# kzhai/PyLDA

Hardware: AMD Instinct MI355X
Metric: documents/sec per VB iteration (higher is better)
Workload: dtype f64

## Files before the change

### include/pylda_hip.h

```cpp
#ifndef PYLDA_HIP_H
#define PYLDA_HIP_H

#include <stdint.h>

#ifdef __cplusplus
extern "C" {
#endif

typedef struct pylda_ctx pylda_ctx;
typedef struct pylda_corpus pylda_corpus;

typedef enum pylda_status {
    PYLDA_OK = 0,
    PYLDA_ERR_INVALID = -1,
    PYLDA_ERR_HIP = -2,
    PYLDA_ERR_OOM = -3,
    PYLDA_ERR_STATE = -4
} pylda_status;

#define PYLDA_ABI_VERSION 10
int pylda_abi_version(void);

const char* pylda_version(void);

// ... 72 lines not shown
int pylda_elapsed_ms(pylda_ctx* ctx, int slot_from, int slot_to, double* ms);

int pylda_set_profiling(pylda_ctx* ctx, int enabled);
int pylda_kernel_time(pylda_ctx* ctx, double* doc_kernel_ms, double* sstats_kernel_ms,
                      int64_t* estep_calls);
int pylda_work_counters(pylda_ctx* ctx, double* inner_iterations, double* inner_iteration_terms);
int pylda_executed_work(pylda_ctx* ctx, double* tile_entries, double* handed_over);
int pylda_clock_counters(pylda_ctx* ctx, double* shader_ticks, double* wall_ticks, double* wall_hz);

int pylda_corpus_plan(pylda_corpus* corpus, int32_t capacity, int32_t* variant, int32_t* geometry,
                      int64_t* documents, int64_t* terms, double* kernel_ms);

int64_t pylda_corpus_layout(pylda_corpus* corpus, const char* name);

int pylda_set_option(pylda_ctx* ctx, const char* name, int64_t value);

int pylda_test_special(pylda_ctx* ctx, int64_t n, const double* x, double* digamma_out,
                       double* lgamma_out);

int pylda_parse_corpus(const char* text, int64_t text_bytes, int doc_separator, const char* vocab,
                       int64_t vocab_bytes, int lowercase, int64_t* n_docs, int64_t* nnz,
                       int64_t* doc_ptr, int32_t* term_id, int32_t* term_ct, int64_t* dropped_docs);

int pylda_test_alpha_update(pylda_ctx* ctx, const double* alpha_k, const double* alpha_ss_k, double number_of_documents,
                            int hyper_parameter_iteration, double hyper_parameter_decay_factor,
                            int hyper_parameter_maximum_decay, double hyper_parameter_converge_threshold,
                            double* alpha_out_k);

int pylda_hybrid_estep(pylda_ctx* ctx, pylda_corpus* corpus, int number_of_samples, int burn_in_samples, uint64_t seed,
                       uint64_t stream, int64_t first_document, int heldout);
int pylda_hybrid_scale_sstats(pylda_ctx* ctx, double divisor);

int pylda_test_philox(pylda_ctx* ctx, int64_t n, const uint32_t* counter_key, uint32_t* out);

int pylda_gibbs_init(pylda_ctx* ctx, pylda_corpus* corpus, uint64_t seed, int64_t first_document);
int pylda_gibbs_sweep(pylda_ctx* ctx, pylda_corpus* corpus, const double* alpha_k, const double* beta_v, double beta_sum,
                      int64_t blocks, uint64_t seed, uint64_t stream, int64_t first_document);
int pylda_gibbs_log_posterior(pylda_ctx* ctx, pylda_corpus* corpus, const double* alpha_k, const double* beta_v, double* out);
int pylda_gibbs_get_counts(pylda_ctx* ctx, pylda_corpus* corpus, int32_t* n_kv, int32_t* n_k, int32_t* topics);
int pylda_gibbs_set_state(pylda_ctx* ctx, pylda_corpus* corpus, const int32_t* n_kv, const int32_t* n_k, const int32_t* topics);

int pylda_gibbs_round_tokens(pylda_ctx* ctx, pylda_corpus* corpus, int64_t blocks, int64_t first_document, int64_t* tokens);
int pylda_gibbs_exchange_prepare(pylda_ctx* ctx, pylda_corpus* corpus, int64_t blocks, int64_t first_document, int world, int rank,
                                 const int64_t* capacity, void** send, void** recv);
int pylda_gibbs_round_sample(pylda_ctx* ctx, pylda_corpus* corpus, const double* alpha_k, const double* beta_v, double beta_sum,
                             int64_t blocks, int64_t round, uint64_t seed, uint64_t stream, int64_t first_document);
int pylda_gibbs_round_apply(pylda_ctx* ctx, pylda_corpus* corpus, int64_t round);
int pylda_gibbs_table_device(pylda_ctx* ctx, pylda_corpus* corpus, void** table, int64_t* table_elements, void** n_k);
int pylda_gibbs_log_posterior_parts(pylda_ctx* ctx, pylda_corpus* corpus, const double* alpha_k, const double* beta_v, double* out);

int pylda_foldin_set_model(pylda_ctx* ctx, pylda_corpus* trained, const int32_t* n_kv, const int32_t* n_k,
                           const double* beta_v, double beta_sum);
int pylda_foldin(pylda_ctx* ctx, pylda_corpus* heldout, const double* alpha_k, int number_of_samples, int burn_in_samples,
                 uint64_t seed, uint64_t stream, int64_t first_document, double* words_log_likelihood);

int pylda_completion_set_model(pylda_ctx* ctx);
int pylda_completion_score(pylda_ctx* ctx, pylda_corpus* observed, pylda_corpus* held, const double* gamma_dk,
                           double* held_log_likelihood, int64_t* held_tokens);

int pylda_left_to_right(pylda_ctx* ctx, pylda_corpus* heldout, const double* alpha_k, int particles, int resample,
                        uint64_t seed, uint64_t stream, int64_t first_document, int64_t step_budget,
                        double* log_likelihood, int64_t* tokens);
int pylda_test_left_to_right_state(pylda_ctx* ctx, pylda_corpus* heldout, int particles, uint16_t* z_out, double* p_out);

int pylda_top_words(pylda_ctx* ctx, const double* table_kv ,
                    int M, int32_t* ids_km, double* values_km);
int pylda_codocument_counts(pylda_ctx* ctx, pylda_corpus* reference, int M, const int32_t* ids_km ,
                            int64_t* doc_freq_km, int64_t* co_kmm);

int pylda_similarity_set_base(pylda_ctx* ctx, int64_t D, const double* rows_dk , int transform);
int pylda_similar_documents(pylda_ctx* ctx, int64_t Q, const double* rows_qk , int transform, int N,
                            const int32_t* self_ids , int32_t* ids_qn, double* scores_qn);

int pylda_topic_distances(pylda_ctx* ctx, const double* a_kv , int Ka,
                          const double* b_kv , int Kb, int metric, double* out_ab);

int pylda_test_expdigamma(pylda_ctx* ctx, int64_t n, const double* x, double c, double* out);

int pylda_test_special_forms(pylda_ctx* ctx, int64_t n, const double* x, double c, int form, double* out);

int pylda_test_tables(pylda_ctx* ctx, double* psi_rowsum_k, double* elog_vldk, double* expElog_vldk,
                      double* expElog_elog_vldk, double* shift_v, double* topic_lse_k, double* alpha_sgn_k, int* path_out);

int pylda_test_statistics(pylda_ctx* ctx, pylda_corpus* corpus, const double* t_dldk, const double* r_nnz,
                          const int32_t* live_n_d, const uint16_t* live_topic_d60, const double* live_t_d60,
                          double* entropy_out);

int pylda_test_gibbs_posterior_terms(pylda_ctx* ctx, pylda_corpus* corpus, const double* alpha_k, const double* beta_v,
                                     double* doc_terms, double* word_terms, double* sums);

#ifdef __cplusplus
}
#endif
#endif
```

### pylda_amd/_capi.py

```python
import collections
import ctypes
import os
import threading

import numpy as np

ABI_VERSION = 10
_LIB_PATH = os.path.join(os.path.dirname(os.path.abspath(__file__)), "lib", "libpylda_hip.so")
_lib = None

_c_double_p = ctypes.POINTER(ctypes.c_double)
_c_int32_p = ctypes.POINTER(ctypes.c_int32)
_c_int64_p = ctypes.POINTER(ctypes.c_int64)
_vp = ctypes.c_void_p

SIGNATURES = {
    "pylda_version": (ctypes.c_char_p, []),
    "pylda_abi_version": (ctypes.c_int, []),
    "pylda_device_count": (ctypes.c_int, [ctypes.POINTER(ctypes.c_int)]),
    "pylda_create": (ctypes.c_int, [ctypes.c_int, ctypes.c_int, ctypes.c_int, ctypes.POINTER(_vp)]),
    "pylda_destroy": (None, [_vp]),
    "pylda_last_error": (ctypes.c_char_p, [_vp]),
    "pylda_set_stream": (ctypes.c_int, [_vp, _vp]),
    "pylda_use_own_stream": (ctypes.c_int, [_vp]),
    "pylda_synchronize": (ctypes.c_int, [_vp]),
    "pylda_corpus_create": (ctypes.c_int, [_vp, ctypes.c_int64, _c_int64_p, _c_int32_p, _c_int32_p,
                                           ctypes.POINTER(_vp)]),
    "pylda_corpus_destroy": (None, [_vp]),
    "pylda_corpus_info": (ctypes.c_int, [_vp, _c_int64_p, _c_int64_p, _c_int64_p, _c_int32_p]),
    "pylda_set_eta": (ctypes.c_int, [_vp, _c_double_p]),
    "pylda_get_eta": (ctypes.c_int, [_vp, _c_double_p]),
    "pylda_set_alpha": (ctypes.c_int, [_vp, _c_double_p]),
    "pylda_estep": (ctypes.c_int, [_vp, _vp, ctypes.c_int, ctypes.c_double, ctypes.c_int]),
    "pylda_estep_results": (ctypes.c_int, [_vp, _vp, _c_double_p, _c_double_p, _c_int64_p]),
    "pylda_get_sstats": (ctypes.c_int, [_vp, _c_double_p]),
    "pylda_set_sstats": (ctypes.c_int, [_vp, _c_double_p]),
    "pylda_get_gamma": (ctypes.c_int, [_vp, _vp, _c_double_p]),
    "pylda_get_doc_values": (ctypes.c_int, [_vp, _vp, _c_double_p, _c_double_p, _c_int32_p]),
    "pylda_estep_host": (ctypes.c_int, [_vp, _vp, _c_double_p, _c_double_p, ctypes.c_int,
                                        ctypes.c_double, ctypes.c_int, _c_double_p, _c_double_p,
                                        _c_double_p, _c_double_p, _c_int32_p, _c_double_p]),
    "pylda_table_stride": (ctypes.c_int, [_vp]),
    "pylda_compute_units": (ctypes.c_int, [_vp]),
    "pylda_sstats_device": (_vp, [_vp]),
    "pylda_eta_device": (_vp, [_vp]),
    "pylda_gamma_device": (_vp, [_vp]),
    "pylda_mark_device_state": (ctypes.c_int, [_vp, ctypes.c_int, ctypes.c_int]),
    "pylda_comm_unique_id": (ctypes.c_int, [_vp]),
    "pylda_comm_init": (ctypes.c_int, [_vp, _vp, ctypes.c_int, ctypes.c_int]),
    "pylda_comm_destroy": (ctypes.c_int, [_vp]),
    "pylda_allreduce_sstats": (ctypes.c_int, [_vp]),
    "pylda_allreduce_doubles": (ctypes.c_int, [_vp, _c_double_p, ctypes.c_int64]),
    "pylda_mstep": (ctypes.c_int, [_vp, _vp, _c_double_p, _c_double_p, _c_double_p]),
    "pylda_mstep_enqueue": (ctypes.c_int, [_vp, _vp, _c_double_p, ctypes.c_int, ctypes.c_double, ctypes.c_int,
                                           ctypes.c_double]),
    "pylda_mstep_online": (ctypes.c_int, [_vp, _vp, _c_double_p, ctypes.c_double, ctypes.c_double, _c_double_p, _c_double_p]),
    "pylda_mstep_online_enqueue": (ctypes.c_int, [_vp, _vp, _c_double_p, ctypes.c_double, ctypes.c_double]),
    "pylda_outer_device": (_vp, [_vp, _c_int64_p]),
    "pylda_allreduce_outer": (ctypes.c_int, [_vp]),
    "pylda_outer_fetch": (ctypes.c_int, [_vp, _c_double_p, _c_double_p, _c_int64_p, _c_double_p, _c_double_p,
                                         _c_double_p]),
    "pylda_host_alloc": (ctypes.c_int, [ctypes.c_int64, ctypes.POINTER(_vp)]),
    "pylda_host_free": (ctypes.c_int, [_vp]),
    "pylda_model_checkpoint": (ctypes.c_int, [_vp, ctypes.c_int]),
    "pylda_mark_time": (ctypes.c_int, [_vp, ctypes.c_int]),
    "pylda_elapsed_ms": (ctypes.c_int, [_vp, ctypes.c_int, ctypes.c_int, _c_double_p]),
    "pylda_work_counters": (ctypes.c_int, [_vp, _c_double_p, _c_double_p]),
    "pylda_executed_work": (ctypes.c_int, [_vp, _c_double_p, _c_double_p]),
    "pylda_clock_counters": (ctypes.c_int, [_vp, _c_double_p, _c_double_p, _c_double_p]),
    "pylda_set_profiling": (ctypes.c_int, [_vp, ctypes.c_int]),
    "pylda_kernel_time": (ctypes.c_int, [_vp, _c_double_p, _c_double_p, _c_int64_p]),
    "pylda_corpus_layout": (ctypes.c_int64, [_vp, ctypes.c_char_p]),
    "pylda_corpus_plan": (ctypes.c_int, [_vp, ctypes.c_int32, _c_int32_p, _c_int32_p, _c_int64_p, _c_int64_p,
                                         _c_double_p]),
    "pylda_set_option": (ctypes.c_int, [_vp, ctypes.c_char_p, ctypes.c_int64]),
    "pylda_parse_corpus": (ctypes.c_int, [ctypes.c_char_p, ctypes.c_int64, ctypes.c_int, ctypes.c_char_p,
                                          ctypes.c_int64, ctypes.c_int, _c_int64_p, _c_int64_p, _c_int64_p,
                                          _c_int32_p, _c_int32_p, _c_int64_p]),
    "pylda_test_alpha_update": (ctypes.c_int, [_vp, _c_double_p, _c_double_p, ctypes.c_double, ctypes.c_int, ctypes.c_double,
                                               ctypes.c_int, ctypes.c_double, _c_double_p]),
    "pylda_test_expdigamma": (ctypes.c_int, [_vp, ctypes.c_int64, _c_double_p, ctypes.c_double, _c_double_p]),
    "pylda_test_special_forms": (ctypes.c_int, [_vp, ctypes.c_int64, _c_double_p, ctypes.c_double, ctypes.c_int, _c_double_p]),
    "pylda_test_tables": (ctypes.c_int, [_vp, _c_double_p, _c_double_p, _c_double_p, _c_double_p, _c_double_p, _c_double_p,
                                         _c_double_p, ctypes.POINTER(ctypes.c_int)]),
    "pylda_test_statistics": (ctypes.c_int, [_vp, _vp, _c_double_p, _c_double_p, _c_int32_p, ctypes.POINTER(ctypes.c_uint16),
                                             _c_double_p, _c_double_p]),
    "pylda_test_special": (ctypes.c_int, [_vp, ctypes.c_int64, _c_double_p, _c_double_p, _c_double_p]),
    "pylda_test_gibbs_posterior_terms": (ctypes.c_int, [_vp, _vp, _c_double_p, _c_double_p, _c_double_p, _c_double_p, _c_double_p]),
    "pylda_hybrid_estep": (ctypes.c_int, [_vp, _vp, ctypes.c_int, ctypes.c_int, ctypes.c_uint64, ctypes.c_uint64,
                                          ctypes.c_int64, ctypes.c_int]),
    "pylda_hybrid_scale_sstats": (ctypes.c_int, [_vp, ctypes.c_double]),
    "pylda_test_philox": (ctypes.c_int, [_vp, ctypes.c_int64, ctypes.POINTER(ctypes.c_uint32),
                                         ctypes.POINTER(ctypes.c_uint32)]),
    "pylda_gibbs_init": (ctypes.c_int, [_vp, _vp, ctypes.c_uint64, ctypes.c_int64]),
    "pylda_gibbs_sweep": (ctypes.c_int, [_vp, _vp, _c_double_p, _c_double_p, ctypes.c_double, ctypes.c_int64, ctypes.c_uint64,
                                         ctypes.c_uint64, ctypes.c_int64]),
    "pylda_gibbs_log_posterior": (ctypes.c_int, [_vp, _vp, _c_double_p, _c_double_p, _c_double_p]),
    "pylda_gibbs_get_counts": (ctypes.c_int, [_vp, _vp, _c_int32_p, _c_int32_p, _c_int32_p]),
    "pylda_gibbs_set_state": (ctypes.c_int, [_vp, _vp, _c_int32_p, _c_int32_p, _c_int32_p]),
    "pylda_gibbs_round_tokens": (ctypes.c_int, [_vp, _vp, ctypes.c_int64, ctypes.c_int64, _c_int64_p]),
    "pylda_gibbs_exchange_prepare": (ctypes.c_int, [_vp, _vp, ctypes.c_int64, ctypes.c_int64, ctypes.c_int, ctypes.c_int, _c_int64_p,
                                                    ctypes.POINTER(_vp), ctypes.POINTER(_vp)]),
    "pylda_gibbs_round_sample": (ctypes.c_int, [_vp, _vp, _c_double_p, _c_double_p, ctypes.c_double, ctypes.c_int64, ctypes.c_int64,
                                                ctypes.c_uint64, ctypes.c_uint64, ctypes.c_int64]),
    "pylda_gibbs_round_apply": (ctypes.c_int, [_vp, _vp, ctypes.c_int64]),
    "pylda_gibbs_table_device": (ctypes.c_int, [_vp, _vp, ctypes.POINTER(_vp), _c_int64_p, ctypes.POINTER(_vp)]),
    "pylda_gibbs_log_posterior_parts": (ctypes.c_int, [_vp, _vp, _c_double_p, _c_double_p, _c_double_p]),
    "pylda_foldin_set_model": (ctypes.c_int, [_vp, _vp, _c_int32_p, _c_int32_p, _c_double_p, ctypes.c_double]),
    "pylda_foldin": (ctypes.c_int, [_vp, _vp, _c_double_p, ctypes.c_int, ctypes.c_int, ctypes.c_uint64, ctypes.c_uint64,
                                    ctypes.c_int64, _c_double_p]),
    "pylda_completion_set_model": (ctypes.c_int, [_vp]),
    "pylda_completion_score": (ctypes.c_int, [_vp, _vp, _vp, _c_double_p, _c_double_p, _c_int64_p]),
    "pylda_left_to_right": (ctypes.c_int, [_vp, _vp, _c_double_p, ctypes.c_int, ctypes.c_int, ctypes.c_uint64, ctypes.c_uint64,
                                           ctypes.c_int64, ctypes.c_int64, _c_double_p, _c_int64_p]),
    "pylda_test_left_to_right_state": (ctypes.c_int, [_vp, _vp, ctypes.c_int, ctypes.POINTER(ctypes.c_uint16), _c_double_p]),
    "pylda_top_words": (ctypes.c_int, [_vp, _c_double_p, ctypes.c_int, _c_int32_p, _c_double_p]),
    "pylda_codocument_counts": (ctypes.c_int, [_vp, _vp, ctypes.c_int, _c_int32_p, _c_int64_p, _c_int64_p]),
    "pylda_similarity_set_base": (ctypes.c_int, [_vp, ctypes.c_int64, _c_double_p, ctypes.c_int]),
    "pylda_similar_documents": (ctypes.c_int, [_vp, ctypes.c_int64, _c_double_p, ctypes.c_int, ctypes.c_int, _c_int32_p, _c_int32_p,
                                               _c_double_p]),
    "pylda_topic_distances": (ctypes.c_int, [_vp, _c_double_p, ctypes.c_int, _c_double_p, ctypes.c_int, ctypes.c_int, _c_double_p]),
}


def library_path():
    return _LIB_PATH


def _preload_torch_hip_runtime():
    if os.environ.get("PYLDA_HIP_RUNTIME", "") == "system":
        return
    try:
        import importlib.util
        spec = importlib.util.find_spec("torch")
        if spec is None or not spec.submodule_search_locations:
            return
        bundled = os.path.join(list(spec.submodule_search_locations)[0], "lib", "libamdhip64.so")
        if os.path.exists(bundled):
            ctypes.CDLL(bundled, mode=ctypes.RTLD_GLOBAL)
    except Exception:
        pass


def _bind(lib, path=_LIB_PATH):
    for name, (restype, argtypes) in SIGNATURES.items():
        try:
            fn = getattr(lib, name)
        except AttributeError:
            raise RuntimeError("pylda_amd: %s does not export %s, which this binding declares: it was built from older "
                               "sources - rebuild it (python -m pylda_amd.build --force)" % (path, name))
        fn.restype = restype
        fn.argtypes = argtypes
    return lib


def load():
    global _lib
    if _lib is not None:
        return _lib
    if not os.path.exists(_LIB_PATH):
        raise RuntimeError(
            "pylda_amd: %s is missing - build it with `python -m pylda_amd.build` "
            "(or __graft_entry__.build()).  pylda_amd has no CPU fallback." % _LIB_PATH)
    _preload_torch_hip_runtime()
    lib = _bind(ctypes.CDLL(_LIB_PATH))
    if lib.pylda_abi_version() != ABI_VERSION:
        raise RuntimeError("pylda_amd: %s implements ABI %d, this binding was written for ABI %d - rebuild it "
# ... 470 lines not shown
        self._check(self._lib.pylda_elapsed_ms(self._h, int(slot_from), int(slot_to), ctypes.byref(ms)))
        return ms.value

    def work_counters(self):
        a, b = ctypes.c_double(0), ctypes.c_double(0)
        self._check(self._lib.pylda_work_counters(self._h, ctypes.byref(a), ctypes.byref(b)))
        return a.value, b.value

    def executed_work(self):
        a, b = ctypes.c_double(0), ctypes.c_double(0)
        self._check(self._lib.pylda_executed_work(self._h, ctypes.byref(a), ctypes.byref(b)))
        return a.value, b.value

    def shader_clock_mhz(self):
        a, b, hz = ctypes.c_double(0), ctypes.c_double(0), ctypes.c_double(0)
        self._check(self._lib.pylda_clock_counters(self._h, ctypes.byref(a), ctypes.byref(b), ctypes.byref(hz)))
        return a.value / b.value * hz.value / 1e6 if b.value > 0 else None

    def sstats_elements(self):
        return self.V * int(self._lib.pylda_table_stride(self._h))

    def compute_units(self):
        return int(self._lib.pylda_compute_units(self._h))

    def sstats_device_ptr(self):
        return int(self._lib.pylda_sstats_device(self._h) or 0)

    def eta_device_ptr(self):
        return int(self._lib.pylda_eta_device(self._h) or 0)

    def mark_device_state(self, have_eta=-1, have_sstats=-1):
        self._check(self._lib.pylda_mark_device_state(self._h, int(have_eta), int(have_sstats)))

    def comm_init(self, unique_id, rank, world_size):
        buf = ctypes.create_string_buffer(bytes(unique_id), 128)
        self._check(self._lib.pylda_comm_init(self._h, ctypes.cast(buf, _vp), int(rank), int(world_size)))

    def comm_destroy(self):
        self._check(self._lib.pylda_comm_destroy(self._h))

    def allreduce_sstats(self):
        self._check(self._lib.pylda_allreduce_sstats(self._h))

    def allreduce_doubles(self, values):
        values = np.ascontiguousarray(values, dtype=np.float64).copy()
        self._check(self._lib.pylda_allreduce_doubles(self._h, _dp(values), values.size))
        return values

    def set_profiling(self, enabled):
        self._check(self._lib.pylda_set_profiling(self._h, 1 if enabled else 0))

    def kernel_time(self):
        ms, ss, calls = ctypes.c_double(0), ctypes.c_double(0), ctypes.c_int64(0)
        self._check(self._lib.pylda_kernel_time(self._h, ctypes.byref(ms), ctypes.byref(ss), ctypes.byref(calls)))
        return ms.value, ss.value, calls.value

    def test_alpha_update(self, alpha, alpha_ss, number_of_documents, iterations=100, decay_factor=0.9, maximum_decay=10,
                          threshold=1e-6):
        alpha, alpha_ss = _f64(alpha, (self.K,), "alpha"), _f64(alpha_ss, (self.K,), "alpha_ss")
        out = np.empty(self.K, dtype=np.float64)
        self._check(self._lib.pylda_test_alpha_update(self._h, _dp(alpha), _dp(alpha_ss), float(number_of_documents),
                                                      int(iterations), float(decay_factor), int(maximum_decay),
                                                      float(threshold), _dp(out)))
        return out

    def test_expdigamma(self, x, c):
        x = _f64(x)
        out = np.empty_like(x)
        self._check(self._lib.pylda_test_expdigamma(self._h, x.size, _dp(x), float(c), _dp(out)))
        return out

    def test_special_forms(self, x, form, c=0.0):
        x = _f64(x)
        out = np.empty_like(x)
        self._check(self._lib.pylda_test_special_forms(self._h, x.size, _dp(x), float(c), int(form), _dp(out)))
        return out

    def test_special(self, x):
        x = _f64(x)
        dg, lg = np.empty_like(x), np.empty_like(x)
        self._check(self._lib.pylda_test_special(self._h, x.size, _dp(x), _dp(dg), _dp(lg)))
        return dg, lg

    def test_tables(self, alpha_sgn=False, tables=True, only=None):
        ldk = int(self._lib.pylda_table_stride(self._h))
        out = {}
        if tables:
            out = {"psi_rowsum": (self.K,), "elog": (self.V, ldk), "expElog": (self.V, ldk),
                   "expElog_elog": (self.V, ldk), "shift": (self.V,), "topic_lse": (self.K,)}
            out = {name: np.empty(shape) for name, shape in out.items() if only is None or name in only}
        if alpha_sgn:
            out["alpha_sgn"] = np.empty(self.K)
        path = ctypes.c_int(0)
        self._check(self._lib.pylda_test_tables(self._h, *[_dp(out.get(name)) for name in (
            "psi_rowsum", "elog", "expElog", "expElog_elog", "shift", "topic_lse", "alpha_sgn")], ctypes.byref(path)))
        out["path"] = path.value
        return out

    def test_statistics(self, corpus, t, r, live_n=None, live_topic=None, live_t=None):
        ldk = int(self._lib.pylda_table_stride(self._h))
        t, r = _f64(t, (corpus.D, ldk), "t"), _f64(r, (corpus.nnz,), "r")
        topic_p = None
        if live_n is not None:
            live_n = np.ascontiguousarray(live_n, dtype=np.int32)
            live_topic = np.ascontiguousarray(live_topic, dtype=np.uint16)
            live_t = _f64(live_t, (corpus.D, 60), "live_t")
            if live_n.shape != (corpus.D,) or live_topic.shape != (corpus.D, 60):
                raise ValueError("live_n, live_topic have shapes %s, %s, expected %s, %s"
                                 % (live_n.shape, live_topic.shape, (corpus.D,), (corpus.D, 60)))
            topic_p = live_topic.ctypes.data_as(ctypes.POINTER(ctypes.c_uint16))
        entropy = ctypes.c_double(0)
        self._check(self._lib.pylda_test_statistics(self._h, corpus._h, _dp(t), _dp(r), _ip(live_n), topic_p, _dp(live_t),
                                                    ctypes.byref(entropy)))
        return entropy.value

    def test_gibbs_posterior_terms(self, corpus, alpha, beta):
        alpha, beta = _f64(alpha, (self.K,), "alpha"), _f64(beta, (self.V,), "beta")
        docs, words, sums = np.zeros(corpus.D), np.zeros(self.V), np.zeros(3)
        self._check(self._lib.pylda_test_gibbs_posterior_terms(self._h, corpus._h, _dp(alpha), _dp(beta), _dp(docs), _dp(words),
                                                               _dp(sums)))
        return docs, words, sums


class Corpus(object):

    def __init__(self, ctx, doc_ptr, term_id, term_ct):
        doc_ptr = np.ascontiguousarray(doc_ptr, dtype=np.int64)
        term_id = np.ascontiguousarray(term_id, dtype=np.int32)
        term_ct = np.ascontiguousarray(term_ct, dtype=np.int32)
        if doc_ptr.ndim != 1 or doc_ptr.size < 1:
            raise ValueError("doc_ptr must hold D+1 offsets")
        if term_id.shape != term_ct.shape or term_id.ndim != 1 or term_id.size != doc_ptr[-1]:
            raise ValueError("term_id/term_ct must be 1-D of length doc_ptr[-1]")
        handle = _vp()
        rc = ctx._lib.pylda_corpus_create(
            ctx._h, doc_ptr.size - 1, doc_ptr.ctypes.data_as(_c_int64_p),
            term_id.ctypes.data_as(_c_int32_p), term_ct.ctypes.data_as(_c_int32_p),
            ctypes.byref(handle))
        ctx._check(rc)
        self._ctx = ctx
        self._h = handle
        self.D = int(doc_ptr.size - 1)
        self.nnz = int(term_id.size)
        tokens = ctypes.c_int64(0)
        ctx._lib.pylda_corpus_info(handle, None, None, ctypes.byref(tokens), None)
        self.tokens = int(tokens.value)

    def gamma_device_ptr(self):
        return int(self._ctx._lib.pylda_gamma_device(self._h) or 0)

    VARIANT_NAMES = {0: "generic64", 1: "generic256", 2: "generic512", 3: "generic_global", 4: "slab",
                     6: "quilt", 9: "qgroup", 10: "quad", 11: "qfuse", 12: "generic_huge", 13: "qfusek"}

    def plan(self):
        lib = self._ctx._lib
        n = lib.pylda_corpus_plan(self._h, 0, None, None, None, None, None)
        if n < 0:
            self._ctx._check(n)
        variant, geometry = np.zeros(n, np.int32), np.zeros(n, np.int32)
        documents, terms, ms = np.zeros(n, np.int64), np.zeros(n, np.int64), np.zeros(n, np.float64)
        rc = lib.pylda_corpus_plan(self._h, n, _ip(variant), _ip(geometry), documents.ctypes.data_as(_c_int64_p),
                                   terms.ctypes.data_as(_c_int64_p), _dp(ms))
        if rc < 0:
            self._ctx._check(rc)
        return [{"kernel": self.VARIANT_NAMES.get(int(variant[i]), str(int(variant[i]))), "geometry": int(geometry[i]),
                 "documents": int(documents[i]), "terms": int(terms[i]), "kernel_ms": float(ms[i])}
# ... 19 lines not shown
```

### pylda_amd/csrc/context.hip

```cpp
#include "host_internal.h"
#include "transpose_kernel.h"
#include "special_device.h"

namespace pylda_host {

std::string g_create_error;

int fail(pylda_ctx* ctx, int code, const char* fmt, ...)
{
    char buf[512];
    va_list ap;
    va_start(ap, fmt);
    vsnprintf(buf, sizeof buf, fmt, ap);
    va_end(ap);
    if (ctx) ctx->err = buf; else g_create_error = buf;
    return code;
}

static hipEvent_t take_event(pylda_ctx* ctx)
{
    if (!ctx->event_pool.empty()) {
        hipEvent_t e = ctx->event_pool.back();
        ctx->event_pool.pop_back();
        return e;
// ... 76 lines not shown
const char* pylda_version(void) { return "pylda_hip 0.9 (gfx950, abi 10)"; }
int pylda_abi_version(void) { return PYLDA_ABI_VERSION; }

int pylda_device_count(int* count)
{
    if (!count) return PYLDA_ERR_INVALID;
    int n = 0;
    if (hipGetDeviceCount(&n) != hipSuccess) n = 0;
    *count = n;
    return PYLDA_OK;
}

const char* pylda_last_error(const pylda_ctx* ctx)
{
    return ctx ? ctx->err.c_str() : g_create_error.c_str();
}

int pylda_create(int device, int K, int V, pylda_ctx** out)
{
    if (!out) return fail(nullptr, PYLDA_ERR_INVALID, "pylda_create: out is NULL");
    *out = nullptr;
    if (K < 1 || V < 1) return fail(nullptr, PYLDA_ERR_INVALID, "pylda_create: K=%d V=%d", K, V);
    if ((int64_t)K * V > ((int64_t)1 << 40))
        return fail(nullptr, PYLDA_ERR_INVALID, "pylda_create: K*V too large");
    int ndev = 0;
    if (hipGetDeviceCount(&ndev) != hipSuccess || ndev == 0)
        return fail(nullptr, PYLDA_ERR_HIP,
                    "pylda_create: no HIP device visible; this library has no CPU fallback");
    if (device < 0 || device >= ndev)
        return fail(nullptr, PYLDA_ERR_INVALID, "pylda_create: device %d of %d", device, ndev);
    pylda_ctx* ctx = new (std::nothrow) pylda_ctx;
    if (!ctx) return fail(nullptr, PYLDA_ERR_OOM, "pylda_create: host allocation failed");
    ctx->device = device;
    ctx->K = K;
    ctx->V = V;
    ctx->ldk = table_stride_for(K);
    auto bail = [&](int code) {
        g_create_error = ctx->err;
        pylda_destroy(ctx);
        return code;
    };
#define CREATE_TRY(expr)                     \
    do {                                     \
        int rc_ = (expr);                    \
        if (rc_ != PYLDA_OK) return bail(rc_); \
    } while (0)
    auto hip_ok = [&](hipError_t e, const char* what) {
        if (e == hipSuccess) return (int)PYLDA_OK;
        return fail(ctx, e == hipErrorOutOfMemory ? PYLDA_ERR_OOM : PYLDA_ERR_HIP, "%s: %s", what,
                    hipGetErrorString(e));
    };
    CREATE_TRY(hip_ok(hipSetDevice(device), "hipSetDevice"));
    hipDeviceProp_t prop;
    CREATE_TRY(hip_ok(hipGetDeviceProperties(&prop, device), "hipGetDeviceProperties"));
    ctx->num_cu = prop.multiProcessorCount > 0 ? prop.multiProcessorCount : 256;
    size_t lds = prop.maxSharedMemoryPerMultiProcessor;
    if (lds < 64 * 1024) lds = 64 * 1024;
    if (lds > 160 * 1024) lds = 160 * 1024;
    ctx->lds_limit = lds;
    CREATE_TRY(hip_ok(hipStreamCreateWithFlags(&ctx->own_stream, hipStreamNonBlocking),
                      "hipStreamCreate"));
    ctx->stream = ctx->own_stream;
    for (int i = 0; i < pylda_ctx::kAux; ++i) {
        CREATE_TRY(hip_ok(hipStreamCreateWithFlags(&ctx->aux_stream[i], hipStreamNonBlocking), "hipStreamCreate"));
        CREATE_TRY(hip_ok(hipEventCreateWithFlags(&ctx->join_event[i], hipEventDisableTiming), "hipEventCreate"));
    }
    CREATE_TRY(hip_ok(hipEventCreateWithFlags(&ctx->fork_event, hipEventDisableTiming), "hipEventCreate"));
    const size_t kv = (size_t)K * V, wk = (size_t)V * ctx->ldk;
    CREATE_TRY(dev_alloc(ctx, &ctx->d_eta, kv));
    CREATE_TRY(dev_alloc(ctx, &ctx->d_elog, wk));
    CREATE_TRY(dev_alloc(ctx, &ctx->d_expElog, wk));
    CREATE_TRY(dev_alloc(ctx, &ctx->d_expElog_elog, wk));
    CREATE_TRY(dev_alloc(ctx, &ctx->d_sstats, wk));
    CREATE_TRY(dev_alloc(ctx, &ctx->d_kv_scratch, kv));
    CREATE_TRY(dev_alloc(ctx, &ctx->d_shift, (size_t)V));
    CREATE_TRY(dev_alloc(ctx, &ctx->d_beta, (size_t)V));
    CREATE_TRY(dev_alloc(ctx, &ctx->d_psi_rowsum, (size_t)K));
    CREATE_TRY(dev_alloc(ctx, &ctx->d_topic_lse, (size_t)K));
    CREATE_TRY(dev_alloc(ctx, &ctx->d_alpha, (size_t)K));
    CREATE_TRY(dev_alloc(ctx, &ctx->d_alpha_sgn, (size_t)K));
    CREATE_TRY(dev_alloc(ctx, &ctx->d_alpha_wsum, (size_t)1));
    CREATE_TRY(dev_alloc(ctx, &ctx->d_small, (size_t)(4 * K + 16)));
    CREATE_TRY(dev_alloc(ctx, &ctx->d_partial, (size_t)1024 * K));
    CREATE_TRY(dev_alloc(ctx, &ctx->d_outer, (size_t)(3 * K + 8)));
    CREATE_TRY(dev_alloc(ctx, &ctx->d_newton_work, (size_t)4 * K));
    CREATE_TRY(dev_alloc(ctx, &ctx->d_work, (size_t)6));
    CREATE_TRY(hip_ok(hipMemsetAsync(ctx->d_work, 0, 6 * sizeof(double), ctx->stream), "hipMemsetAsync"));
    CREATE_TRY(hip_ok(hipHostMalloc(reinterpret_cast<void**>(&ctx->h_pin), (size_t)(5 * K + 8) * sizeof(double), hipHostMallocDefault),
                      "hipHostMalloc"));
    for (int i = 0; i < 2; ++i)
        CREATE_TRY(hip_ok(hipEventCreateWithFlags(&ctx->alpha_event[i], hipEventDisableTiming), "hipEventCreate"));
    CREATE_TRY(hip_ok(hipMemsetAsync(ctx->d_sstats, 0, wk * sizeof(double), ctx->stream),
                      "hipMemsetAsync"));
#undef CREATE_TRY
    *out = ctx;
    return PYLDA_OK;
}

void pylda_destroy(pylda_ctx* ctx)
{
    if (!ctx) return;
    (void)hipSetDevice(ctx->device);
    if (ctx->own_stream) (void)hipStreamSynchronize(ctx->own_stream);
    if (ctx->comm) pylda::comm_destroy(ctx->comm);
    dev_free(ctx->d_comm_small);
    dev_free(ctx->d_foldin_table); dev_free(ctx->d_foldin_alpha); dev_free(ctx->d_completion_rowsum);
    dev_free(ctx->d_similarity_base);
    dev_free(ctx->d_ltr_z); dev_free(ctx->d_ltr_p);
    drain_events(ctx);
    for (hipEvent_t e : ctx->event_pool) (void)hipEventDestroy(e);
    dev_free(ctx->d_eta); dev_free(ctx->d_elog); dev_free(ctx->d_expElog); dev_free(ctx->d_expElog_elog); dev_free(ctx->d_sstats);
    dev_free(ctx->d_kv_scratch); dev_free(ctx->d_shift); dev_free(ctx->d_beta);
    dev_free(ctx->d_psi_rowsum); dev_free(ctx->d_topic_lse); dev_free(ctx->d_alpha); dev_free(ctx->d_alpha_sgn); dev_free(ctx->d_alpha_wsum);
    dev_free(ctx->d_small); dev_free(ctx->d_partial); dev_free(ctx->d_outer); dev_free(ctx->d_newton_work); dev_free(ctx->d_work); dev_free(ctx->d_eta_ckpt);
    if (ctx->h_pin) (void)hipHostFree(ctx->h_pin);
    for (int i = 0; i < 2; ++i)
        if (ctx->alpha_event[i]) (void)hipEventDestroy(ctx->alpha_event[i]);
    for (hipEvent_t e : ctx->mark_event)
        if (e) (void)hipEventDestroy(e);
    for (int i = 0; i < pylda_ctx::kAux; ++i) {
        if (ctx->aux_stream[i]) { (void)hipStreamSynchronize(ctx->aux_stream[i]); (void)hipStreamDestroy(ctx->aux_stream[i]); }
        if (ctx->join_event[i]) (void)hipEventDestroy(ctx->join_event[i]);
    }
    if (ctx->fork_event) (void)hipEventDestroy(ctx->fork_event);
    if (ctx->own_stream) (void)hipStreamDestroy(ctx->own_stream);
    delete ctx;
}

int pylda_set_stream(pylda_ctx* ctx, void* hip_stream)
{
    if (!ctx) return PYLDA_ERR_INVALID;
    HIP_TRY(ctx, hipSetDevice(ctx->device));
    HIP_TRY(ctx, hipStreamSynchronize(ctx->stream));
    ctx->stream = reinterpret_cast<hipStream_t>(hip_stream);
    return PYLDA_OK;
}

int pylda_use_own_stream(pylda_ctx* ctx)
{
    if (!ctx) return PYLDA_ERR_INVALID;
    HIP_TRY(ctx, hipSetDevice(ctx->device));
    HIP_TRY(ctx, hipStreamSynchronize(ctx->stream));
    ctx->stream = ctx->own_stream;
    return PYLDA_OK;
}

int pylda_synchronize(pylda_ctx* ctx)
{
    if (!ctx) return PYLDA_ERR_INVALID;
    HIP_TRY(ctx, hipSetDevice(ctx->device));
    HIP_TRY(ctx, hipStreamSynchronize(ctx->stream));
    return PYLDA_OK;
}

int pylda_set_option(pylda_ctx* ctx, const char* name, int64_t value)
{
    if (!ctx || !name) return PYLDA_ERR_INVALID;
    if (!strcmp(name, "force_logspace")) ctx->force_logspace = value != 0;
    else if (!strcmp(name, "force_variant")) {
        if (value < -1 || value > kVariantLast || value == kRetired5 || value == kRetired7 || value == kRetired8)
            return fail(ctx, PYLDA_ERR_INVALID, "force_variant %lld is not a kernel variant", (long long)value);
        ctx->force_variant = (int)value;
        ctx->plan_epoch += 1;
    } else if (!strcmp(name, "gather_rows")) {
        ctx->gather_rows = (int)value;
    } else if (!strcmp(name, "gather_blocks")) {
        if (value > 1 && value % 8) return fail(ctx, PYLDA_ERR_INVALID, "gather_blocks=%lld: a multiple of 8, or -1 / 0 / 1", (long long)value);
        ctx->gather_blocks = (int)value;
    } else if (!strcmp(name, "quilt_odd")) {
        ctx->quilt_odd = value != 0;
        ctx->plan_epoch += 1;
    } else if (!strcmp(name, "sweep_xcd")) {
        ctx->sweep_xcd = value != 0;
    } else if (!strcmp(name, "sweep_sub")) {
        ctx->sweep_sub = (int)std::min<int64_t>(64, std::max<int64_t>(1, value));
    } else if (!strcmp(name, "sweep_spin")) {
        ctx->sweep_spin = (int)std::max<int64_t>(0, value);
    } else if (!strcmp(name, "gather_sweep")) {
        ctx->gather_sweep = (int)std::min<int64_t>(2, std::max<int64_t>(0, value));
    } else if (!strcmp(name, "gather_round_mb")) {
        ctx->gather_round_mb = (int)std::max<int64_t>(0, value);
    } else if (!strcmp(name, "launch_order")) {
        ctx->launch_order = (int)value;
    } else if (!strcmp(name, "terms_overlap")) {
        ctx->terms_overlap = value != 0;
    } else if (!strcmp(name, "slab_uber")) {
        ctx->slab_uber = value != 0;
    } else if (!strcmp(name, "wide_postings")) {
        ctx->wide_postings = value != 0;
    } else if (!strcmp(name, "lds_pad")) {
        ctx->lds_pad = (int)value;
    } else if (!strcmp(name, "quad")) {
        ctx->quad = value != 0;
        ctx->plan_epoch += 1;
    } else if (!strcmp(name, "quad_stream")) {
        ctx->quad_stream = value != 0;
        ctx->plan_epoch += 1;
    } else if (!strcmp(name, "quad_packed")) {
        ctx->quad_packed = value != 0;
    } else if (!strcmp(name, "prepare_path")) {
        if (value < 0 || value > 2 || (value == 1 && ctx->K > 64))
            return fail(ctx, PYLDA_ERR_INVALID, "prepare_path=%lld at K=%d: 0 (by size), 1 (one kernel, K <= 64) or 2 (two passes)",
                        (long long)value, ctx->K);
        ctx->prepare_path = (int)value;
    } else if (!strcmp(name, "quilt12")) {
        ctx->quilt12 = value != 0;
        ctx->plan_epoch += 1;
    } else if (!strcmp(name, "doc_values")) {
        ctx->doc_values = value != 0;
    } else if (!strcmp(name, "gather_live")) {
        ctx->gather_live = value != 0;
    } else if (!strcmp(name, "compact")) {
        ctx->compact = value != 0;
    } else if (!strcmp(name, "compact_pair")) {
        ctx->compact_pair = value < 0 ? -1 : value != 0;
    } else if (!strcmp(name, "compact_stream")) {
        ctx->compact_stream = value != 0;
    } else if (!strcmp(name, "compact_phase")) {
        ctx->compact_phase = value != 0;
    } else if (!strcmp(name, "compact_cap")) {
        if (value < 0 || value > kLiveStride) return fail(ctx, PYLDA_ERR_INVALID, "compact_cap=%lld: 0 .. %d", (long long)value, kLiveStride);
        ctx->compact_cap = (int)value;
    } else if (!strcmp(name, "compact_guard_fail")) {
        ctx->compact_guard_fail = value != 0;
    } else if (!strcmp(name, "coherence_chunk_docs")) {
        if (value < 0 || value % 64) return fail(ctx, PYLDA_ERR_INVALID, "coherence_chunk_docs=%lld: a multiple of 64, or 0", (long long)value);
        ctx->coherence_chunk_docs = value;
    } else if (!strcmp(name, "similarity_doc_slices")) {
        if (value < 0 || value > 1024) return fail(ctx, PYLDA_ERR_INVALID, "similarity_doc_slices=%lld: 1 .. 1024, or 0", (long long)value);
        ctx->similarity_doc_slices = (int)value;
    } else if (!strcmp(name, "topic_distance_segment_groups")) {
        if (value < 0 || value > 65535)
            return fail(ctx, PYLDA_ERR_INVALID, "topic_distance_segment_groups=%lld: 1 .. 65535, or 0", (long long)value);
        ctx->topic_distance_segment_groups = (int)value;
    } else if (!strcmp(name, "ltr_chunk_tokens")) {
        if (value < 0) return fail(ctx, PYLDA_ERR_INVALID, "ltr_chunk_tokens=%lld: a number of tokens, or 0", (long long)value);
        ctx->ltr_chunk_tokens = value;
    } else
        return fail(ctx, PYLDA_ERR_INVALID, "unknown option '%s'", name);
    return PYLDA_OK;
}

int pylda_set_eta(pylda_ctx* ctx, const double* eta_kv)
{
    if (!ctx) return PYLDA_ERR_INVALID;
    if (!eta_kv) return fail(ctx, PYLDA_ERR_INVALID, "set_eta: NULL");
    HIP_TRY(ctx, hipSetDevice(ctx->device));
    HIP_TRY(ctx, hipMemcpyAsync(ctx->d_eta, eta_kv, (size_t)ctx->K * ctx->V * sizeof(double),
                                hipMemcpyHostToDevice, ctx->stream));
    HIP_TRY(ctx, hipStreamSynchronize(ctx->stream));
    ctx->have_eta = true;
    return PYLDA_OK;
}

int pylda_get_eta(pylda_ctx* ctx, double* eta_kv)
{
    if (!ctx) return PYLDA_ERR_INVALID;
    if (!eta_kv) return fail(ctx, PYLDA_ERR_INVALID, "get_eta: NULL");
    if (!ctx->have_eta) return fail(ctx, PYLDA_ERR_STATE, "get_eta: eta was never set");
    HIP_TRY(ctx, hipSetDevice(ctx->device));
    HIP_TRY(ctx, hipMemcpyAsync(eta_kv, ctx->d_eta, (size_t)ctx->K * ctx->V * sizeof(double),
                                hipMemcpyDeviceToHost, ctx->stream));
    HIP_TRY(ctx, hipStreamSynchronize(ctx->stream));
    return PYLDA_OK;
}

int pylda_set_alpha(pylda_ctx* ctx, const double* alpha_k)
{
    if (!ctx) return PYLDA_ERR_INVALID;
    if (!alpha_k) return fail(ctx, PYLDA_ERR_INVALID, "set_alpha: NULL");
    for (int k = 0; k < ctx->K; ++k)
        if (!(alpha_k[k] > 0.0) || !std::isfinite(alpha_k[k]))
            return fail(ctx, PYLDA_ERR_INVALID, "set_alpha: alpha[%d]=%g is not positive", k, alpha_k[k]);
    if (ctx->have_alpha && ctx->h_alpha.size() == (size_t)ctx->K &&
        memcmp(ctx->h_alpha.data(), alpha_k, (size_t)ctx->K * sizeof(double)) == 0)
        return PYLDA_OK;
    ctx->h_alpha.assign(alpha_k, alpha_k + ctx->K);
    HIP_TRY(ctx, hipSetDevice(ctx->device));
    const int slot = ctx->alpha_slot;
    ctx->alpha_slot ^= 1;
    if (ctx->alpha_event_used[slot]) HIP_TRY(ctx, hipEventSynchronize(ctx->alpha_event[slot]));
    double* pin = ctx->h_pin + (size_t)slot * ctx->K;
    memcpy(pin, alpha_k, (size_t)ctx->K * sizeof(double));
    HIP_TRY(ctx, hipMemcpyAsync(ctx->d_alpha, pin, (size_t)ctx->K * sizeof(double), hipMemcpyHostToDevice, ctx->stream));
    HIP_TRY(ctx, hipEventRecord(ctx->alpha_event[slot], ctx->stream));
    ctx->alpha_event_used[slot] = true;
    ctx->have_alpha = true;
    return PYLDA_OK;
}

int pylda_get_sstats(pylda_ctx* ctx, double* sstats_kv)
{
    if (!ctx) return PYLDA_ERR_INVALID;
    if (!sstats_kv) return fail(ctx, PYLDA_ERR_INVALID, "get_sstats: NULL");
    if (!ctx->have_sstats) return fail(ctx, PYLDA_ERR_STATE, "get_sstats: no training-mode E-step has run");
    HIP_TRY(ctx, hipSetDevice(ctx->device));
    const int K = ctx->K, V = ctx->V;
    hipLaunchKernelGGL(transpose_kernel, dim3((K + 31) / 32, (V + 31) / 32), dim3(256), 0, ctx->stream,
                       ctx->d_sstats, V, K, ctx->ldk, V, ctx->d_kv_scratch);
    HIP_TRY(ctx, hipGetLastError());
    HIP_TRY(ctx, hipMemcpyAsync(sstats_kv, ctx->d_kv_scratch, (size_t)K * V * sizeof(double),
                                hipMemcpyDeviceToHost, ctx->stream));
    HIP_TRY(ctx, hipStreamSynchronize(ctx->stream));
    return PYLDA_OK;
}

int pylda_set_sstats(pylda_ctx* ctx, const double* sstats_kv)
{
    if (!ctx) return PYLDA_ERR_INVALID;
    if (!sstats_kv) return fail(ctx, PYLDA_ERR_INVALID, "set_sstats: NULL");
    HIP_TRY(ctx, hipSetDevice(ctx->device));
    const int K = ctx->K, V = ctx->V;
    HIP_TRY(ctx, hipMemcpyAsync(ctx->d_kv_scratch, sstats_kv, (size_t)K * V * sizeof(double),
                                hipMemcpyHostToDevice, ctx->stream));
    HIP_TRY(ctx, hipMemsetAsync(ctx->d_sstats, 0, (size_t)V * ctx->ldk * sizeof(double), ctx->stream));
    hipLaunchKernelGGL(transpose_kernel, dim3((V + 31) / 32, (K + 31) / 32), dim3(256), 0, ctx->stream,
                       ctx->d_kv_scratch, K, V, V, ctx->ldk, ctx->d_sstats);
    HIP_TRY(ctx, hipGetLastError());
    HIP_TRY(ctx, hipStreamSynchronize(ctx->stream));
    ctx->have_sstats = true;
    return PYLDA_OK;
}

int pylda_table_stride(const pylda_ctx* ctx) { return ctx ? ctx->ldk : 0; }
int pylda_compute_units(const pylda_ctx* ctx) { return ctx ? ctx->num_cu : 0; }
void* pylda_sstats_device(pylda_ctx* ctx) { return ctx ? ctx->d_sstats : nullptr; }
void* pylda_eta_device(pylda_ctx* ctx) { return ctx ? ctx->d_eta : nullptr; }
void* pylda_gamma_device(pylda_corpus* c) { return c ? c->d_gamma : nullptr; }

int pylda_mark_device_state(pylda_ctx* ctx, int have_eta, int have_sstats)
{
    if (!ctx) return PYLDA_ERR_INVALID;
    if (have_eta >= 0) ctx->have_eta = have_eta != 0;
    if (have_sstats >= 0) ctx->have_sstats = have_sstats != 0;
    return PYLDA_OK;
}

int pylda_host_alloc(int64_t bytes, void** out)
{
    if (!out || bytes < 0) return PYLDA_ERR_INVALID;
    *out = nullptr;
    const hipError_t e = hipHostMalloc(out, (size_t)std::max<int64_t>(bytes, 1), hipHostMallocDefault);
    if (e != hipSuccess) {
        *out = nullptr;
        return fail(nullptr, e == hipErrorOutOfMemory ? PYLDA_ERR_OOM : PYLDA_ERR_HIP, "host_alloc: %s", hipGetErrorString(e));
    }
    return PYLDA_OK;
}

int pylda_host_free(void* p)
{
    if (p && hipHostFree(p) != hipSuccess) return fail(nullptr, PYLDA_ERR_HIP, "host_free: not a pylda_host_alloc pointer");
    return PYLDA_OK;
}

int pylda_model_checkpoint(pylda_ctx* ctx, int restore)
{
    if (!ctx) return PYLDA_ERR_INVALID;
    HIP_TRY(ctx, hipSetDevice(ctx->device));
    const size_t bytes = (size_t)ctx->K * ctx->V * sizeof(double);
    if (!restore) {
        if (!ctx->have_eta) return fail(ctx, PYLDA_ERR_STATE, "model_checkpoint: eta was never set");
        if (!ctx->d_eta_ckpt) {
            const int rc = dev_alloc(ctx, &ctx->d_eta_ckpt, (size_t)ctx->K * ctx->V);
            if (rc != PYLDA_OK) return rc;
        }
        HIP_TRY(ctx, hipMemcpyAsync(ctx->d_eta_ckpt, ctx->d_eta, bytes, hipMemcpyDeviceToDevice, ctx->stream));
    } else {
        if (!ctx->d_eta_ckpt) return fail(ctx, PYLDA_ERR_STATE, "model_checkpoint: nothing was saved");
        HIP_TRY(ctx, hipMemcpyAsync(ctx->d_eta, ctx->d_eta_ckpt, bytes, hipMemcpyDeviceToDevice, ctx->stream));
        ctx->have_eta = true;
    }
    return PYLDA_OK;
}

int pylda_mark_time(pylda_ctx* ctx, int slot)
{
    if (!ctx) return PYLDA_ERR_INVALID;
    if (slot < 0 || slot >= 4) return fail(ctx, PYLDA_ERR_INVALID, "mark_time: slot %d", slot);
    HIP_TRY(ctx, hipSetDevice(ctx->device));
    if (!ctx->mark_event[slot]) HIP_TRY(ctx, hipEventCreate(&ctx->mark_event[slot]));
    HIP_TRY(ctx, hipEventRecord(ctx->mark_event[slot], ctx->stream));
    return PYLDA_OK;
}

int pylda_elapsed_ms(pylda_ctx* ctx, int slot_from, int slot_to, double* ms)
{
    if (!ctx) return PYLDA_ERR_INVALID;
    if (slot_from < 0 || slot_from >= 4 || slot_to < 0 || slot_to >= 4 || !ms || !ctx->mark_event[slot_from] || !ctx->mark_event[slot_to])
        return fail(ctx, PYLDA_ERR_INVALID, "elapsed_ms: slots %d, %d", slot_from, slot_to);
    HIP_TRY(ctx, hipSetDevice(ctx->device));
    HIP_TRY(ctx, hipEventSynchronize(ctx->mark_event[slot_to]));
    float f = 0.f;
    HIP_TRY(ctx, hipEventElapsedTime(&f, ctx->mark_event[slot_from], ctx->mark_event[slot_to]));
    *ms = f;
    return PYLDA_OK;
}

int pylda_work_counters(pylda_ctx* ctx, double* inner_iterations, double* inner_iteration_terms)
{
    if (!ctx) return PYLDA_ERR_INVALID;
    HIP_TRY(ctx, hipSetDevice(ctx->device));
    HIP_TRY(ctx, hipMemcpyAsync(ctx->work_cache, ctx->d_work, sizeof ctx->work_cache, hipMemcpyDeviceToHost, ctx->stream));
    HIP_TRY(ctx, hipMemsetAsync(ctx->d_work, 0, sizeof ctx->work_cache, ctx->stream));
    HIP_TRY(ctx, hipStreamSynchronize(ctx->stream));
    if (inner_iterations) *inner_iterations = ctx->work_cache[0];
    if (inner_iteration_terms) *inner_iteration_terms = ctx->work_cache[1];
    return PYLDA_OK;
}

int pylda_executed_work(pylda_ctx* ctx, double* tile_entries, double* handed_over)
// ... 206 lines not shown
```

### pylda_amd/csrc/estep_api.hip

```cpp
#include "host_internal.h"
#include "estep_logspace.h"
#include "doc_terms.h"
#include "prepare_kernels.h"

namespace pylda_host {

int prepare_path_of(const pylda_ctx* ctx)
{
    if (ctx->prepare_path) return ctx->prepare_path;
    return ctx->K <= 64 && (int64_t)ctx->K * ctx->V <= (1 << 21) ? 1 : 2;
}

int enqueue_prepare(pylda_ctx* ctx, bool heldout)
{
    const int K = ctx->K, V = ctx->V;
    hipLaunchKernelGGL(eta_rowsum_psi_kernel, dim3(K), dim3(256), 0, ctx->stream, ctx->d_eta, K, V,
                       ctx->d_psi_rowsum);
    if (prepare_path_of(ctx) == 1) {
        hipLaunchKernelGGL(elog_rows_small_kernel, dim3((V + 3) / 4), dim3(256), 0, ctx->stream, ctx->d_eta, ctx->d_psi_rowsum,
                           K, V, ctx->ldk, ctx->d_elog, ctx->d_expElog, ctx->d_expElog_elog, ctx->d_shift);
    } else {
        hipLaunchKernelGGL(elog_transpose_kernel, dim3((V + 31) / 32, (K + 31) / 32), dim3(256), 0,
                           ctx->stream, ctx->d_eta, ctx->d_psi_rowsum, K, V, ctx->ldk, ctx->d_elog);
        hipLaunchKernelGGL(row_shift_exp_kernel, dim3((V + 3) / 4), dim3(256), 0, ctx->stream,
// ... 43 lines not shown
        const int64_t n = doc_ptr[d + 1] - doc_ptr[d];
        if (n < 0) return fail(ctx, PYLDA_ERR_INVALID, "corpus_create: doc_ptr not monotone at %lld", (long long)d);
        *max_terms = std::max(*max_terms, n);
    }
    const int64_t nnz = doc_ptr[D];
    const size_t need = generic_lds_layout(ctx->K, 0, tile_stride_for(ctx->K), 256, true).total;
    const size_t net = logspace_launch_lds_bytes(ctx->K) + kLdsMargin;
    if (need > ctx->lds_limit || net > ctx->lds_limit)
        return fail(ctx, PYLDA_ERR_INVALID, "corpus_create: K=%d needs %zu bytes of LDS per document (limit %zu)", ctx->K,
                    std::max(need, net), ctx->lds_limit);
    if (*max_terms > INT32_MAX)
        return fail(ctx, PYLDA_ERR_INVALID, "corpus_create: a document has %lld distinct terms", (long long)*max_terms);
    if (nnz > ((int64_t)1 << 36))
        return fail(ctx, PYLDA_ERR_INVALID, "corpus_create: %lld distinct (doc, term) pairs; shard the corpus", (long long)nnz);
    if (nnz > 0 && (!term_id || !term_ct))
        return fail(ctx, PYLDA_ERR_INVALID, "corpus_create: NULL term arrays");
    const int nthreads = (int)std::max<int64_t>(1, std::min<int64_t>({(int64_t)std::thread::hardware_concurrency(), 16, nnz / 4000000 + 1}));
    std::vector<int64_t> bad_at((size_t)nthreads, -1), part((size_t)nthreads, 0);
    auto check = [&](int t) {
        const int64_t from = nnz * t / nthreads, to = nnz * (t + 1) / nthreads;
        const int V = ctx->V;
        int64_t sum = 0;
        for (int64_t i = from; i < to; ++i) {
            if ((unsigned)term_id[i] >= (unsigned)V || term_ct[i] < 1) {
                bad_at[(size_t)t] = i;
                return;
            }
            sum += term_ct[i];
        }
        part[(size_t)t] = sum;
    };
    std::vector<std::thread> workers;
    for (int t = 1; t < nthreads; ++t) workers.emplace_back(check, t);
    check(0);
    for (auto& w : workers) w.join();
    *tokens = 0;
    for (int t = 0; t < nthreads; ++t) {
        const int64_t i = bad_at[(size_t)t];
        if (i >= 0) {
            if (term_id[i] < 0 || term_id[i] >= ctx->V)
                return fail(ctx, PYLDA_ERR_INVALID, "corpus_create: term id %d at %lld outside [0,%d)",
                            term_id[i], (long long)i, ctx->V);
            return fail(ctx, PYLDA_ERR_INVALID, "corpus_create: count %d at %lld", term_ct[i], (long long)i);
        }
        *tokens += part[(size_t)t];
    }
    return PYLDA_OK;
}

void schedule_corpus(pylda_corpus* c, const int64_t* doc_ptr)
{
    const int64_t D = c->D, max_terms = c->max_terms;
    std::vector<int32_t>& order = c->h_order;
    order.resize((size_t)D);
    if (max_terms <= (int64_t)4 << 20) {
        std::vector<int64_t> at((size_t)max_terms + 2, 0);
        for (int64_t d = 0; d < D; ++d) at[(size_t)(max_terms - (doc_ptr[d + 1] - doc_ptr[d])) + 1] += 1;
        for (int64_t n = 0; n <= max_terms; ++n) at[(size_t)n + 1] += at[(size_t)n];
        for (int64_t d = 0; d < D; ++d) order[(size_t)at[(size_t)(max_terms - (doc_ptr[d + 1] - doc_ptr[d]))]++] = (int32_t)d;
    } else {
        std::iota(order.begin(), order.end(), 0);
        std::stable_sort(order.begin(), order.end(), [&](int32_t a, int32_t b) {
            return doc_ptr[a + 1] - doc_ptr[a] > doc_ptr[b + 1] - doc_ptr[b];
        });
    }
    c->h_terms_sorted.resize((size_t)D);
    for (int64_t i = 0; i < D; ++i)
        c->h_terms_sorted[i] = (int32_t)(doc_ptr[order[i] + 1] - doc_ptr[order[i]]);
    build_plan(c);
}

int upload_corpus(pylda_ctx* ctx, pylda_corpus* c, const int64_t* doc_ptr, const int32_t* term_id, const int32_t* term_ct)
{
    const size_t D = (size_t)c->D, nnz = (size_t)c->nnz;
    FirstError A{ctx, "corpus_create"};
    A(dev_alloc(ctx, &c->d_doc_ptr, D + 1));
    A(dev_alloc(ctx, &c->d_term_id, nnz));
    A(dev_alloc(ctx, &c->d_term_ct, nnz));
    A(dev_alloc(ctx, &c->d_order, D));
    A(dev_alloc(ctx, &c->d_gamma, D * ctx->K));
    A(dev_alloc(ctx, &c->d_doc_ll, D));
    A(dev_alloc(ctx, &c->d_doc_wll, D));
    A(dev_alloc(ctx, &c->d_iters, D));
    A(dev_alloc(ctx, &c->d_status, D));
    A(dev_alloc(ctx, &c->d_scalars, (size_t)4));
    c->d_flag_count = c->d_scalars ? reinterpret_cast<int32_t*>(c->d_scalars + 3) : nullptr;
    A(dev_alloc(ctx, &c->d_entropy_partial, (size_t)(((int64_t)ctx->V * ctx->ldk + 255) / 256)));
    A(dev_alloc(ctx, &c->d_tfinal, D * ctx->ldk));
    A(dev_alloc(ctx, &c->d_rfinal, nnz));
    if (A.rc != PYLDA_OK) return A.rc;
    A.h2d(c->d_doc_ptr, doc_ptr, (D + 1) * sizeof(int64_t));
    A.h2d(c->d_term_id, term_id, nnz * sizeof(int32_t));
    A.h2d(c->d_term_ct, term_ct, nnz * sizeof(int32_t));
    A.h2d(c->d_order, c->h_order.data(), D * sizeof(int32_t));
    return A.rc;
}

int pack_quad_slots(pylda_ctx* ctx, pylda_corpus* c)
{
    if (c->quad_slots_serial == c->plan_serial) return PYLDA_OK;
    c->quad_slots_serial = c->plan_serial;
    HIP_TRY(ctx, hipStreamSynchronize(ctx->stream));
    dev_free(c->d_quad_rec);
    dev_free(c->d_quad_ids);
    c->quad_slots = quad_slot_layout(c->plan);
    if (c->quad_slots.records == 0) return PYLDA_OK;
    if (hipMalloc(reinterpret_cast<void**>(&c->d_quad_rec), (size_t)c->quad_slots.records * sizeof(QuadSlot)) != hipSuccess ||
        hipMalloc(reinterpret_cast<void**>(&c->d_quad_ids), (size_t)c->quad_slots.ids * sizeof(int32_t)) != hipSuccess) {
        (void)hipGetLastError();
        dev_free(c->d_quad_rec);
        dev_free(c->d_quad_ids);
        return PYLDA_OK;
    }
    for (size_t j = 0; j < c->plan.size(); ++j) {
        const Launch& L = c->plan[j];
        if (c->quad_slots.rec_first[j] < 0 || L.count <= 0) continue;
        hipLaunchKernelGGL(quad_pack_kernel, dim3((unsigned)L.count), dim3(256), 0, ctx->stream, c->d_doc_ptr, c->d_term_id, c->d_term_ct,
                           c->d_order + L.first, quad_wpr_of(L.rn), quad_wpg_of(L.rn), c->quad_slots.ids_stride[j],
                           c->d_quad_rec + c->quad_slots.rec_first[j], c->d_quad_ids + c->quad_slots.ids_first[j]);
    }
    HIP_TRY(ctx, hipGetLastError());
    return PYLDA_OK;
}

int plan_handover(pylda_ctx* ctx, pylda_corpus* c)
{
    if (c->plan_epoch != ctx->plan_epoch || c->plan_exact != ctx->exact_stop) build_plan(c);
    const bool off = !alpha_allows_live(ctx, c->live_off_by_alpha);
    if (off != c->live_off_by_alpha) {
        c->live_off_by_alpha = off;
        if (c->have_postings && (c->live_stats || !off)) release_postings(c);
    }
    const int rc = pack_quad_slots(ctx, c);
    return rc == PYLDA_OK ? prepare_compact(ctx, c) : rc;
}

int estep_plan(pylda_ctx* ctx, pylda_corpus* c, double tol, bool heldout)
{
    const double span = tol * ctx->K;
    ctx->exact_stop = !(span >= 3.725290298461914e-09  && span < 1024.0);
    int rc = plan_handover(ctx, c);
    if (rc == PYLDA_OK && !heldout) rc = build_postings(c);
    if (rc != PYLDA_OK || c->d_term_scratch) return rc;
    for (const Launch& L : c->plan)
        if (L.variant == kGenericHuge) return dev_alloc(ctx, &c->d_term_scratch, (size_t)c->nnz);
    return PYLDA_OK;
}

EstepParams estep_params(const pylda_ctx* ctx, const pylda_corpus* c, int max_iter, double tol, int heldout)
{
    EstepParams p{};
    p.K = ctx->K;
    p.V = ctx->V;
    p.ldk = ctx->ldk;
    p.expElog = ctx->d_expElog;
    p.expElog_elog = ctx->d_expElog_elog;
    p.shift = ctx->d_shift;
    p.topic_lse = ctx->d_topic_lse;
    p.alpha = ctx->d_alpha;
    p.alpha_sgn = ctx->d_alpha;
    p.alpha_wsum = ctx->d_alpha_wsum;
    const AlphaSums a = alpha_sums(ctx);
    p.alpha_term = a.term;
    p.alpha_sum = a.sum;
    p.alpha_lgamma_sum = a.lgamma_sum;
    p.doc_ptr = c->d_doc_ptr;
// ... 85 lines not shown
    }
    if (debug_sync)
        fprintf(stderr, "[pylda debug] class %d variant %d geometry %d documents %lld handoff %d: %s\n", slot, L.variant, L.rn,
                (long long)L.count, p.handoff_on, hipGetErrorString(hipStreamSynchronize(st)));
    if (compact_behind)
        for (const pylda_corpus::CompactRange& r : c->compact_ranges)
            if (rc == PYLDA_OK && r.plan_index == slot) rc = launch_compact(ctx, st, c, p, r.slots, r.from_table, r.first, r.count);
    if (debug_sync && compact_behind)
        fprintf(stderr, "[pylda debug] class %d live-topic kernel: %s\n", slot, hipGetErrorString(hipStreamSynchronize(st)));
    close_bracket(ctx, class_bracket, st);
    return rc;
}

int enqueue_dense_classes(pylda_ctx* ctx, const pylda_corpus* c, EstepParams& p)
{
    const int uber_from = slab_uber_from(ctx, c);
    const size_t separate = uber_from >= 0 ? (size_t)uber_from : c->plan.size();
    const bool fan_out = separate > (uber_from >= 0 ? 0u : 1u);
    AuxFork aux{ctx};
    int rc = fan_out ? aux.fork((int)std::min<size_t>(pylda_ctx::kAux, separate)) : PYLDA_OK;
    if (rc != PYLDA_OK) return rc;
    std::vector<size_t> launch_seq(separate);
    std::iota(launch_seq.begin(), launch_seq.end(), (size_t)0);
    if (ctx->launch_order == 1)
        std::stable_sort(launch_seq.begin(), launch_seq.end(), [&](size_t a, size_t b) { return c->plan[a].count < c->plan[b].count; });
    for (size_t i = 0; i < separate; ++i) {
        hipStream_t st = fan_out ? ctx->aux_stream[i % pylda_ctx::kAux] : ctx->stream;
        if ((rc = launch_class(ctx, st, c, p, (int)launch_seq[i])) != PYLDA_OK) return rc;
    }
    p.handoff_on = 0;
    p.handoff_live = 0;
    if (uber_from < 0) return PYLDA_OK;
    const Launch& L = c->plan[(size_t)uber_from];
    p.order = c->d_order + L.first;
    p.n_cap = L.n_cap;
    p.tile_stride = L.tile_stride;
    const int class_bracket = open_bracket(ctx, uber_from, ctx->stream);
    rc = launch_slab_uber_any(ctx, ctx->stream, p, c, uber_from);
    close_bracket(ctx, class_bracket, ctx->stream);
    return rc;
}

int enqueue_live_phase(pylda_ctx* ctx, const pylda_corpus* c, const EstepParams& p)
{
    if (!c->compact_ready || !ctx->compact_phase) return PYLDA_OK;
    for (size_t a = 0; a < c->compact_ranges.size();) {
        const pylda_corpus::CompactRange& r = c->compact_ranges[a];
        int64_t count = r.count;
        size_t b = a + 1;
        while (b < c->compact_ranges.size() && c->compact_ranges[b].slots == r.slots && c->compact_ranges[b].from_table == r.from_table &&
               c->compact_ranges[b].first == r.first + count) {
            count += c->compact_ranges[b].count;
            ++b;
        }
        const int rc = launch_compact(ctx, ctx->stream, c, p, r.slots, r.from_table, r.first, count);
        if (rc != PYLDA_OK) return rc;
        a = b;
    }
    return PYLDA_OK;
}

bool plan_leaves_terms(const pylda_corpus* c)
{
    for (const Launch& L : c->plan)
        if (L.variant == kQuad || L.variant == kQuilt || L.variant == kQgroup || L.variant == kQfuse || L.variant == kQfusek) return true;
    return false;
}

bool enqueue_doc_terms(pylda_ctx* ctx, const pylda_corpus* c, EstepParams& p)
{
    if (p.heldout || p.want_doc_ll || c->D <= 0 || ctx->force_logspace || !plan_leaves_terms(c)) return false;
    p.order = nullptr;
    hipStream_t st = ctx->stream;
    if (c->have_postings && !c->sweep && ctx->terms_overlap && hipEventRecord(ctx->fork_event, ctx->stream) == hipSuccess &&
        hipStreamWaitEvent(ctx->aux_stream[0], ctx->fork_event, 0) == hipSuccess)
        st = ctx->aux_stream[0];
    hipLaunchKernelGGL(doc_terms_kernel, dim3((unsigned)((c->D + 3) / 4)), dim3(256), 0, st, p, c->D);
    if (st == ctx->stream) return false;
    if (hipEventRecord(ctx->join_event[0], st) == hipSuccess) return true;
    (void)hipStreamSynchronize(st);
    return false;
}

int enqueue_statistics(pylda_ctx* ctx, pylda_corpus* c, bool terms_forked)
{
    if (ctx->force_logspace) {
        HIP_TRY(ctx, hipMemsetAsync(c->d_rfinal, 0, (size_t)c->nnz * sizeof(double), ctx->stream));
        HIP_TRY(ctx, hipMemsetAsync(c->d_tfinal, 0, (size_t)c->D * ctx->ldk * sizeof(double), ctx->stream));
    }
    const int ss_bracket = open_bracket(ctx, -2, ctx->stream);
    const int rc = enqueue_sstats_gather(ctx, c);
    if (terms_forked) (void)hipStreamWaitEvent(ctx->stream, ctx->join_event[0], 0);
    close_bracket(ctx, ss_bracket, ctx->stream);
    return rc;
}

int enqueue_logspace_net(pylda_ctx* ctx, const pylda_corpus* c, EstepParams& p)
{
    if (c->D <= 0) return PYLDA_OK;
    p.order = nullptr;
    const int64_t slots = 4 * (int64_t)ctx->num_cu;
    const int chunk = (int)std::min<int64_t>(256, std::max<int64_t>(1, (c->D + slots - 1) / slots));
    const unsigned grid = (unsigned)std::min<int64_t>((c->D + chunk - 1) / chunk, slots);
    const size_t list_offset = logspace_list_offset(ctx->K), lds = logspace_launch_lds_bytes(ctx->K);
    HIP_TRY(ctx, launch_kernel(estep_logspace_kernel, dim3(grid), dim3(256), lds, ctx->stream, p, ctx->d_elog, ctx->d_sstats, c->d_status,
                               c->D, list_offset, chunk));
    return PYLDA_OK;
}


}

}

extern "C" {

int pylda_corpus_create(pylda_ctx* ctx, int64_t D, const int64_t* doc_ptr, const int32_t* term_id,
                        const int32_t* term_ct, pylda_corpus** out)
{
    if (!ctx) return PYLDA_ERR_INVALID;
    if (!out) return fail(ctx, PYLDA_ERR_INVALID, "corpus_create: out is NULL");
    *out = nullptr;
    PhaseTimer timer;
    int64_t max_terms = 0, tokens = 0;
    int rc = check_corpus(ctx, D, doc_ptr, term_id, term_ct, &max_terms, &tokens);
    if (rc != PYLDA_OK) return rc;
    timer.lap("corpus validation");
    HIP_TRY(ctx, hipSetDevice(ctx->device));
    pylda_corpus* c = new (std::nothrow) pylda_corpus;
    if (!c) return fail(ctx, PYLDA_ERR_OOM, "corpus_create: host allocation failed");
    c->ctx = ctx;
    c->D = D;
    c->nnz = doc_ptr[D];
    c->tokens = tokens;
    c->max_terms = (int32_t)max_terms;
    schedule_corpus(c, doc_ptr);
    timer.lap("schedule (sort + launch plan)");
    if ((rc = upload_corpus(ctx, c, doc_ptr, term_id, term_ct)) != PYLDA_OK) {
        pylda_corpus_destroy(c);
        return rc;
    }
    timer.lap("allocations + corpus H2D");
    if ((rc = pack_quad_slots(ctx, c)) != PYLDA_OK) {
        pylda_corpus_destroy(c);
        return rc;
    }
    timer.lap("packed quad launch slots");
    *out = c;
    return PYLDA_OK;
}

void pylda_corpus_destroy(pylda_corpus* c)
{
    if (!c) return;
    if (c->ctx) {
        (void)hipSetDevice(c->ctx->device);
        (void)hipStreamSynchronize(c->ctx->stream);
    }
    dev_free(c->d_doc_ptr); dev_free(c->d_term_id); dev_free(c->d_term_ct); dev_free(c->d_order);
    dev_free(c->d_gamma); dev_free(c->d_doc_ll); dev_free(c->d_doc_wll); dev_free(c->d_iters);
    dev_free(c->d_status); c->d_flag_count = nullptr; dev_free(c->d_scalars); dev_free(c->d_entropy_partial);
    dev_free(c->d_tfinal); dev_free(c->d_rfinal); dev_free(c->d_term_scratch); dev_free(c->d_post_doc);
    if (c->d_post_pos) (void)hipFree(c->d_post_pos);
    c->d_post_pos = nullptr;
    dev_free(c->d_seg_begin); dev_free(c->d_seg_end); dev_free(c->d_word_seg_ptr); dev_free(c->d_partial); dev_free(c->d_exec_order);
    dev_free(c->d_seg_block); dev_free(c->d_term_of); dev_free(c->d_rendezvous);
    dev_free(c->d_live_n); dev_free(c->d_live_list); dev_free(c->d_tile_ptr); dev_free(c->d_live_tile);
    dev_free(c->d_handoff_it); dev_free(c->d_col_iters); dev_free(c->d_quad_rec); dev_free(c->d_quad_ids);
    dev_free(c->d_tok_off); dev_free(c->d_hyb_state); dev_free(c->d_hyb_col_ptr); dev_free(c->d_hyb_post_pos);
    dev_free(c->d_gibbs_table); dev_free(c->d_gibbs_nk); dev_free(c->d_gibbs_alpha); dev_free(c->d_gibbs_beta); dev_free(c->d_gibbs_words);
    dev_free(c->d_gibbs_send); dev_free(c->d_gibbs_recv); dev_free(c->d_gibbs_rec_off);
    dev_free(c->d_ltr_tok_off);
    if (c->ctx && c->ctx->ltr_last_corpus == c) c->ctx->ltr_last_corpus = nullptr;
    delete c;
}

int pylda_corpus_info(const pylda_corpus* c, int64_t* D, int64_t* nnz, int64_t* tokens,
                      int32_t* max_terms)
{
    if (!c) return PYLDA_ERR_INVALID;
    if (D) *D = c->D;
    if (nnz) *nnz = c->nnz;
    if (tokens) *tokens = c->tokens;
    if (max_terms) *max_terms = c->max_terms;
    return PYLDA_OK;
}

int pylda_estep(pylda_ctx* ctx, pylda_corpus* c, int max_iter, double tol, int heldout)
{
    if (!ctx) return PYLDA_ERR_INVALID;
    if (!c || c->ctx != ctx) return fail(ctx, PYLDA_ERR_INVALID, "estep: corpus does not belong to this context");
    if (max_iter < 1) return fail(ctx, PYLDA_ERR_INVALID, "estep: local_parameter_iteration=%d (must be >= 1)", max_iter);
    if (!(tol >= 0.0) && !(tol < 0.0)) return fail(ctx, PYLDA_ERR_INVALID, "estep: threshold is NaN");
    if (!ctx->have_eta || !ctx->have_alpha)
        return fail(ctx, PYLDA_ERR_STATE, "estep: set_eta and set_alpha must be called first");
    HIP_TRY(ctx, hipSetDevice(ctx->device));
    heldout = heldout ? 1 : 0;
    int rc = enqueue_prepare(ctx, heldout != 0);
    if (rc != PYLDA_OK) return rc;
    if ((rc = estep_plan(ctx, c, tol, heldout != 0)) != PYLDA_OK) return rc;
    EstepParams p = estep_params(ctx, c, max_iter, tol, heldout);
    if ((rc = reset_handoff(ctx, c, p)) != PYLDA_OK) return rc;
    if (ctx->profiling && ctx->class_ms.size() != c->plan.size()) ctx->class_ms.assign(c->plan.size(), 0.0);
    const int doc_bracket = open_bracket(ctx, -1, ctx->stream);
    if (ctx->force_logspace) {
        HIP_TRY(ctx, hipMemsetD32Async(reinterpret_cast<hipDeviceptr_t>(c->d_status), 1, (size_t)c->D, ctx->stream));
    } else {
        if ((rc = enqueue_dense_classes(ctx, c, p)) != PYLDA_OK) return rc;
        if ((rc = enqueue_live_phase(ctx, c, p)) != PYLDA_OK) return rc;
    }
    const bool terms_forked = enqueue_doc_terms(ctx, c, p);
    close_bracket(ctx, doc_bracket, ctx->stream);
    if (ctx->profiling) ctx->estep_calls += 1;
    if (!heldout && (rc = enqueue_statistics(ctx, c, terms_forked)) != PYLDA_OK) return rc;
    if ((rc = enqueue_logspace_net(ctx, c, p)) != PYLDA_OK) return rc;
    if (ctx->profiling && c->D > 0)
        hipLaunchKernelGGL(work_count_kernel, dim3(1), dim3(1024), 0, ctx->stream, c->d_iters, c->d_doc_ptr, c->D, ctx->d_work,
                           c->compact_ready ? c->d_handoff_it : nullptr, c->d_col_iters, ctx->K);
    return finish_estep(ctx, c, heldout, !heldout, p.want_doc_ll != 0);
}

int pylda_estep_results(pylda_ctx* ctx, pylda_corpus* c, double* document_log_likelihood,
                        double* words_log_likelihood, int64_t* logspace_documents)
{
    if (!ctx) return PYLDA_ERR_INVALID;
    if (!c || c->ctx != ctx) return fail(ctx, PYLDA_ERR_INVALID, "estep_results: bad corpus");
    if (!c->estep_done) return fail(ctx, PYLDA_ERR_STATE, "estep_results: no E-step has run on this corpus");
    HIP_TRY(ctx, hipSetDevice(ctx->device));
    double* sc = ctx->h_pin + (size_t)5 * ctx->K + 4;
    int32_t* nflag_pin = reinterpret_cast<int32_t*>(sc + 3);
    HIP_TRY(ctx, hipMemcpyAsync(sc, c->d_scalars, 4 * sizeof(double), hipMemcpyDeviceToHost, ctx->stream));
    HIP_TRY(ctx, hipStreamSynchronize(ctx->stream));
    const int32_t nflag = *nflag_pin;
    if (!c->last_doc_values) sc[0] -= sc[2];
    if (document_log_likelihood) *document_log_likelihood = sc[0];
    if (words_log_likelihood) *words_log_likelihood = sc[1];
    if (logspace_documents) *logspace_documents = nflag;
    return PYLDA_OK;
}

int pylda_get_gamma(pylda_ctx* ctx, pylda_corpus* c, double* gamma_dk)
{
    if (!ctx) return PYLDA_ERR_INVALID;
    if (!c || c->ctx != ctx || !gamma_dk) return fail(ctx, PYLDA_ERR_INVALID, "get_gamma: bad argument");
    if (!c->estep_done) return fail(ctx, PYLDA_ERR_STATE, "get_gamma: no E-step has run on this corpus");
    HIP_TRY(ctx, hipSetDevice(ctx->device));
    HIP_TRY(ctx, hipMemcpyAsync(gamma_dk, c->d_gamma, (size_t)c->D * ctx->K * sizeof(double),
                                hipMemcpyDeviceToHost, ctx->stream));
    HIP_TRY(ctx, hipStreamSynchronize(ctx->stream));
    return PYLDA_OK;
}

int pylda_get_doc_values(pylda_ctx* ctx, pylda_corpus* c, double* doc_ll, double* doc_words_ll,
                         int32_t* iters)
{
    if (!ctx) return PYLDA_ERR_INVALID;
    if (!c || c->ctx != ctx) return fail(ctx, PYLDA_ERR_INVALID, "get_doc_values: bad corpus");
    if (!c->estep_done) return fail(ctx, PYLDA_ERR_STATE, "get_doc_values: no E-step has run on this corpus");
    if (doc_ll && !c->last_doc_values)
        return fail(ctx, PYLDA_ERR_STATE, "get_doc_values: the last E-step ran with option doc_values=0 (corpus-level likelihood only)");
    HIP_TRY(ctx, hipSetDevice(ctx->device));
    if (doc_ll)
        HIP_TRY(ctx, hipMemcpyAsync(doc_ll, c->d_doc_ll, (size_t)c->D * sizeof(double), hipMemcpyDeviceToHost, ctx->stream));
    if (doc_words_ll)
        HIP_TRY(ctx, hipMemcpyAsync(doc_words_ll, c->d_doc_wll, (size_t)c->D * sizeof(double), hipMemcpyDeviceToHost, ctx->stream));
    if (iters)
        HIP_TRY(ctx, hipMemcpyAsync(iters, c->d_iters, (size_t)c->D * sizeof(int32_t), hipMemcpyDeviceToHost, ctx->stream));
    HIP_TRY(ctx, hipStreamSynchronize(ctx->stream));
    return PYLDA_OK;
}

int pylda_test_tables(pylda_ctx* ctx, double* psi_rowsum_k, double* elog_vldk, double* expElog_vldk, double* expElog_elog_vldk,
                      double* shift_v, double* topic_lse_k, double* alpha_sgn_k, int* path_out)
{
    if (!ctx) return PYLDA_ERR_INVALID;
    if (!ctx->have_eta) return fail(ctx, PYLDA_ERR_STATE, "test_tables: set_eta must be called first");
    if (alpha_sgn_k && !ctx->have_alpha) return fail(ctx, PYLDA_ERR_STATE, "test_tables: alpha_sgn needs set_alpha first");
    HIP_TRY(ctx, hipSetDevice(ctx->device));
    const int rc = enqueue_prepare(ctx, true);
    if (rc != PYLDA_OK) return rc;
    if (alpha_sgn_k) {
        hipLaunchKernelGGL(alpha_mortality_kernel, dim3(1), dim3(256), 0, ctx->stream, ctx->d_alpha, ctx->K, ctx->d_alpha_sgn);
        HIP_TRY(ctx, hipGetLastError());
    }
    const size_t K = (size_t)ctx->K, V = (size_t)ctx->V, wk = V * (size_t)ctx->ldk;
    const struct { double* host; const double* dev; size_t n; } out[] = {
        {psi_rowsum_k, ctx->d_psi_rowsum, K}, {elog_vldk, ctx->d_elog, wk},   {expElog_vldk, ctx->d_expElog, wk},
        {expElog_elog_vldk, ctx->d_expElog_elog, wk}, {shift_v, ctx->d_shift, V}, {topic_lse_k, ctx->d_topic_lse, K},
        {alpha_sgn_k, ctx->d_alpha_sgn, K}};
    for (const auto& o : out)
        if (o.host) HIP_TRY(ctx, hipMemcpyAsync(o.host, o.dev, o.n * sizeof(double), hipMemcpyDeviceToHost, ctx->stream));
    HIP_TRY(ctx, hipStreamSynchronize(ctx->stream));
    if (path_out) *path_out = prepare_path_of(ctx);
    return PYLDA_OK;
}

int pylda_test_statistics(pylda_ctx* ctx, pylda_corpus* c, const double* t_dldk, const double* r_nnz, const int32_t* live_n_d,
                          const uint16_t* live_topic_d60, const double* live_t_d60, double* entropy_out)
{
    if (!ctx) return PYLDA_ERR_INVALID;
    if (!c || c->ctx != ctx) return fail(ctx, PYLDA_ERR_INVALID, "test_statistics: corpus does not belong to this context");
    if (!t_dldk || (c->nnz > 0 && !r_nnz)) return fail(ctx, PYLDA_ERR_INVALID, "test_statistics: t or r is NULL");
    if (live_n_d && (!live_topic_d60 || !live_t_d60)) return fail(ctx, PYLDA_ERR_INVALID, "test_statistics: live_n without the lists");
    if (!ctx->have_eta) return fail(ctx, PYLDA_ERR_STATE, "test_statistics: set_eta must be called first");
    HIP_TRY(ctx, hipSetDevice(ctx->device));
    const size_t D = (size_t)c->D;
    std::vector<char> lists;
    bool any_listed = false;
    if (live_n_d) {
        lists.assign(D * kLiveListBytes, 0);
        for (size_t d = 0; d < D; ++d) {
            const int n = live_n_d[d];
            if (n < -1 || n > kLiveStride) return fail(ctx, PYLDA_ERR_INVALID, "test_statistics: live_n[%zu]=%d outside -1 .. %d", d, n, kLiveStride);
            any_listed = any_listed || n >= 0;
            for (int j = 0; j < n; ++j) {
                const uint16_t topic = live_topic_d60[d * kLiveStride + j];
                if (topic >= ctx->K) return fail(ctx, PYLDA_ERR_INVALID, "test_statistics: document %zu lists topic %d of %d", d, (int)topic, ctx->K);
                char* line = lists.data() + d * kLiveListBytes + 128 * (j / kLiveHead);
                memcpy(line + 8 * (j % kLiveHead), &live_t_d60[d * kLiveStride + j], sizeof(double));
                memcpy(line + 96 + 2 * (j % kLiveHead), &topic, sizeof(uint16_t));
            }
        }
    }
    int rc = enqueue_prepare(ctx, false);
    if (rc != PYLDA_OK) return rc;
    if ((rc = plan_handover(ctx, c)) != PYLDA_OK) return rc;
    const bool forced = live_n_d && !c->compact_ready && !c->have_postings;
    if (forced && !c->d_live_n) {
        FirstError A{ctx, "test_statistics"};
        A(dev_alloc(ctx, &c->d_live_n, D));
        A(dev_alloc(ctx, &c->d_live_list, D * kLiveListBytes));
        A(dev_alloc(ctx, &c->d_tile_ptr, D));
        A(dev_alloc(ctx, &c->d_handoff_it, D));
        A(dev_alloc(ctx, &c->d_col_iters, D));
        if (A.rc != PYLDA_OK) return A.rc;
    }
    if (forced) c->compact_ready = true;
    rc = build_postings(c);
    if (forced) c->compact_ready = false;
    if (rc != PYLDA_OK) return rc;
    if (any_listed && !c->live_stats)
        return fail(ctx, PYLDA_ERR_STATE, "test_statistics: documents are listed, but the statistics pass of this corpus reads rows (layout gather_live = 0)");
    HIP_TRY(ctx, hipMemcpyAsync(c->d_tfinal, t_dldk, D * ctx->ldk * sizeof(double), hipMemcpyHostToDevice, ctx->stream));
    if (c->nnz > 0) HIP_TRY(ctx, hipMemcpyAsync(c->d_rfinal, r_nnz, (size_t)c->nnz * sizeof(double), hipMemcpyHostToDevice, ctx->stream));
    if (c->live_stats && live_n_d) {
        HIP_TRY(ctx, hipMemcpyAsync(c->d_live_n, live_n_d, D * sizeof(int32_t), hipMemcpyHostToDevice, ctx->stream));
        HIP_TRY(ctx, hipMemcpyAsync(c->d_live_list, lists.data(), lists.size(), hipMemcpyHostToDevice, ctx->stream));
    } else if (c->live_stats) {
        HIP_TRY(ctx, hipMemsetAsync(c->d_live_n, 0xff, D * sizeof(int32_t), ctx->stream));
    }
// ... 40 lines not shown
```

### pylda_amd/csrc/host_internal.h

```cpp
#pragma once
#include "../../include/pylda_hip.h"

#include <hip/hip_runtime.h>

#include <algorithm>
#include <chrono>
#include <cmath>
#include <cstdarg>
#include <cstdio>
#include <cstdlib>
#include <cstring>
#include <new>
#include <numeric>
#include <string>
#include <thread>
#include <vector>

#include "comm.h"
#include "estep_common.h"
#include "estep_limits.h"
#include "host_plan.h"
#include "postings.h"

using namespace pylda;

namespace pylda_host __attribute__((visibility("hidden"))) {
using namespace pylda_plan;
}

using namespace pylda_host;

struct pylda_corpus;

struct pylda_ctx {
    int device = 0;
    int K = 0, V = 0;
    int ldk = 0;
    hipStream_t own_stream = nullptr;
    static constexpr int kAux = 4;
    hipStream_t aux_stream[kAux] = {nullptr, nullptr, nullptr, nullptr};
    hipEvent_t fork_event = nullptr;
    hipEvent_t join_event[kAux] = {nullptr, nullptr, nullptr, nullptr};
    hipStream_t stream = nullptr;
    size_t lds_limit = 64 * 1024;
    int num_cu = 256;

    double* d_eta = nullptr;
    double* d_elog = nullptr;
    double* d_expElog = nullptr;
    double* d_expElog_elog = nullptr;
    double* d_shift = nullptr;
    double* d_psi_rowsum = nullptr;
    double* d_topic_lse = nullptr;
    double* d_alpha = nullptr;
    double* d_alpha_wsum = nullptr;
    double* d_alpha_sgn = nullptr;
    double* d_sstats = nullptr;
    double* d_kv_scratch = nullptr;
    double* d_beta = nullptr;
    double* d_small = nullptr;
    double* d_partial = nullptr;
    std::vector<double> h_beta;
    double beta_sum = 0.0, beta_lgamma_sum = 0.0;

    std::vector<double> h_alpha;
    double* h_pin = nullptr;
    hipEvent_t alpha_event[2] = {nullptr, nullptr};
    bool alpha_event_used[2] = {false, false};
    int alpha_slot = 0;
    double* d_outer = nullptr;
    bool outer_ready = false;
    bool newton_pending = false;
    NewtonParams newton;
    double* d_newton_work = nullptr;
    double* d_eta_ckpt = nullptr;
    double* d_work = nullptr;
    double work_cache[6] = {0.0, 0.0, 0.0, 0.0, 0.0, 0.0};
    hipEvent_t mark_event[4] = {nullptr, nullptr, nullptr, nullptr};
    void* comm = nullptr;
    int comm_world = 1;
    double* d_comm_small = nullptr;
    double* d_foldin_table = nullptr;
    double* d_foldin_alpha = nullptr;
    bool foldin_ready = false;
    double* d_completion_rowsum = nullptr;
    bool completion_ready = false;
    uint16_t* d_ltr_z = nullptr;
    double* d_ltr_p = nullptr;
    size_t ltr_capacity = 0;
    int64_t ltr_chunk_tokens = 0;
    const pylda_corpus* ltr_last_corpus = nullptr;
    int ltr_last_particles = 0, ltr_last_chunks = 0;
    size_t comm_small_cap = 0;
    bool have_eta = false, have_alpha = false, have_sstats = false;
    int force_logspace = 0;
    int force_variant = -1;
    int quilt12 = 0;
    int gather_rows = 2;
    int gather_blocks = -1;
    int sweep_xcd = 1;
    int sweep_sub = 4;
    int sweep_spin = 4000;
    int gather_sweep = 1;
    int gather_round_mb = 0;
    int launch_order = 1;
    int terms_overlap = 1;
    int slab_uber = 1;
    int wide_postings = 0;
    int lds_pad = 0;
    int quad = 1;
    int quad_stream = 1;
    int prepare_path = 0;
    int quad_packed = 1;
    int quilt_odd = 1;
    int doc_values = 1;
    int compact = 1;
    int gather_live = 1;
    int compact_phase = 1;
    int compact_stream = 1;
    int compact_pair = -1;
    int compact_cap = 0;
    int compact_guard_fail = 0;
    int64_t coherence_chunk_docs = 0;
    int similarity_doc_slices = 0;
    double* d_similarity_base = nullptr;
    int64_t similarity_D = 0;
    int topic_distance_segment_groups = 0;
    int plan_epoch = 0;
    bool exact_stop = false;

    struct Bracket { hipEvent_t a, b; int slot; };
    bool profiling = false;
    std::vector<Bracket> pending_events;
    std::vector<hipEvent_t> event_pool;
    double doc_kernel_ms = 0.0, sstats_kernel_ms = 0.0;
    std::vector<double> class_ms;
    int64_t estep_calls = 0;

    std::string err;
};

struct pylda_corpus {
    pylda_ctx* ctx = nullptr;
    int64_t D = 0, nnz = 0, tokens = 0;
    int32_t max_terms = 0;
    int64_t* d_doc_ptr = nullptr;
    int32_t* d_term_id = nullptr;
    int32_t* d_term_ct = nullptr;
    int32_t* d_order = nullptr;
    double* d_gamma = nullptr;
    double* d_doc_ll = nullptr;
    double* d_doc_wll = nullptr;
    int32_t* d_iters = nullptr;
    int32_t* d_status = nullptr;
    int32_t* d_flag_count = nullptr;
    double* d_scalars = nullptr;
    double* d_entropy_partial = nullptr;
    bool last_doc_values = true;
    double* d_tfinal = nullptr;
    double* d_rfinal = nullptr;
    double* d_term_scratch = nullptr;
    bool have_postings = false;
    int32_t* d_post_doc = nullptr;
    void* d_post_pos = nullptr;
    bool wide_pos = false;
    int64_t* d_seg_begin = nullptr;
    int64_t* d_seg_end = nullptr;
    int32_t* d_exec_order = nullptr;
    int64_t exec_slots = 0;
    using Round = pylda_plan::Round;
    std::vector<Round> rounds;
    int64_t partial_rows = 0, ent_blocks = 0;
    bool sweep = false;
    int sweep_passes = 0, sweep_terms = 0, sweep_wpb = 0;
    int32_t* d_seg_block = nullptr;
    int32_t* d_term_of = nullptr;
    unsigned* d_rendezvous = nullptr;
    int gather_blocks = 1;
    int gather_rows = 2;
    int64_t* d_word_seg_ptr = nullptr;
    double* d_partial = nullptr;
    int64_t nseg = 0;
    std::vector<int32_t> h_terms_sorted;
    std::vector<int32_t> h_order;
    int32_t* d_live_n = nullptr;
    char* d_live_list = nullptr;
    bool live_stats = false;
    int64_t* d_tile_ptr = nullptr;
    double* d_live_tile = nullptr;
    int32_t* d_handoff_it = nullptr;
    int32_t* d_col_iters = nullptr;
    bool compact_ready = false;
    bool compact_failed = false;
    bool live_off_by_alpha = false;
    int compact_plan_epoch = -1, compact_cap_used = -1, compact_stream_used = -1, compact_pair_used = -2;
    struct CompactRange { int plan_index, slots; bool from_table; int64_t first, count; };
    std::vector<CompactRange> compact_ranges;
    std::vector<Launch> plan;
    int plan_epoch = 0;
    int plan_serial = 0;
    pylda::QuadSlot* d_quad_rec = nullptr;
    int32_t* d_quad_ids = nullptr;
    pylda_plan::QuadSlotLayout quad_slots;
    int quad_slots_serial = -1;
    bool plan_exact = false;
    bool estep_done = false;
    int last_heldout = 0;
    int64_t* d_tok_off = nullptr;
    uint64_t* d_hyb_state = nullptr;
    int64_t* d_hyb_col_ptr = nullptr;
    int64_t* d_hyb_post_pos = nullptr;
    int32_t* d_gibbs_table = nullptr;
    int32_t* d_gibbs_nk = nullptr;
    double* d_gibbs_alpha = nullptr;
    double* d_gibbs_beta = nullptr;
    double* d_gibbs_words = nullptr;
    std::vector<double> h_gibbs_alpha, h_gibbs_beta;
    bool gibbs_ready = false;
    uint64_t* d_gibbs_send = nullptr;
    uint64_t* d_gibbs_recv = nullptr;
    int64_t* d_gibbs_rec_off = nullptr;
    std::vector<int64_t> h_gibbs_capacity, h_gibbs_round_tokens;
    int64_t gibbs_exchange_blocks = 0, gibbs_exchange_first = 0;
    int gibbs_exchange_world = 0;
    int64_t* d_ltr_tok_off = nullptr;
    std::vector<int64_t> h_ltr_doc_tok;
};

namespace pylda_host __attribute__((visibility("hidden"))) {

extern std::string g_create_error;
int fail(pylda_ctx* ctx, int code, const char* fmt, ...);

#define HIP_TRY(ctx, expr)                                                              \
    do {                                                                                \
        hipError_t e_ = (expr);                                                         \
        if (e_ != hipSuccess)                                                           \
            return fail((ctx), e_ == hipErrorOutOfMemory ? PYLDA_ERR_OOM : PYLDA_ERR_HIP, \
                        "%s failed: %s (%s:%d)", #expr, hipGetErrorString(e_), __FILE__,  \
                        __LINE__);                                                      \
    } while (0)

template <typename T>
int dev_alloc(pylda_ctx* ctx, T** p, size_t n)
{
    *p = nullptr;
    if (n == 0) n = 1;
    HIP_TRY(ctx, hipMalloc(reinterpret_cast<void**>(p), n * sizeof(T)));
    return PYLDA_OK;
}

template <typename T>
void dev_free(T*& p)
{
    if (p) (void)hipFree(p);
    p = nullptr;
}

struct FirstError {
    pylda_ctx* ctx;
    const char* what;
    int rc = PYLDA_OK;
    void operator()(int r) { if (rc == PYLDA_OK) rc = r; }
    void h2d(void* dst, const void* src, size_t bytes)
    {
        if (rc == PYLDA_OK && bytes && hipMemcpy(dst, src, bytes, hipMemcpyHostToDevice) != hipSuccess)
            rc = fail(ctx, PYLDA_ERR_HIP, "%s: H2D copy failed", what);
    }
};

template <typename... Params, typename... Args>
hipError_t launch_kernel(void (*kern)(Params...), dim3 grid, dim3 block, size_t lds, hipStream_t st, const Args&... args)
{
    if (lds > 64 * 1024) {
        const hipError_t e = hipFuncSetAttribute(reinterpret_cast<const void*>(kern), hipFuncAttributeMaxDynamicSharedMemorySize, (int)lds);
        if (e != hipSuccess) return e;
    }
    hipLaunchKernelGGL(kern, grid, block, lds, st, args...);
    return hipGetLastError();
}

struct PhaseTimer {
    bool on = getenv("PYLDA_TIMING") != nullptr;
    std::chrono::steady_clock::time_point t0 = std::chrono::steady_clock::now();
    void lap(const char* what)
    {
        if (!on) return;
        const auto now = std::chrono::steady_clock::now();
        fprintf(stderr, "[pylda timing] %-34s %8.1f ms\n", what, std::chrono::duration<double, std::milli>(now - t0).count());
        t0 = now;
    }
};

PlanConfig plan_config(const pylda_ctx* ctx);
void build_plan(pylda_corpus* c);
int slab_uber_from(const pylda_ctx* ctx, const pylda_corpus* c);

int launch_generic_any(pylda_ctx* ctx, hipStream_t st, const EstepParams& p, const Launch& L);
int launch_slab_any(pylda_ctx* ctx, hipStream_t st, const EstepParams& p, const Launch& L);
int launch_slab_uber_any(pylda_ctx* ctx, hipStream_t st, const EstepParams& p, const pylda_corpus* c, int from);
int launch_quilt_any(pylda_ctx* ctx, hipStream_t st, const EstepParams& p, const Launch& L);
int launch_quad_any(pylda_ctx* ctx, hipStream_t st, const EstepParams& p, const Launch& L);
int launch_quad_dense_any(pylda_ctx* ctx, hipStream_t st, const EstepParams& p, const Launch& L);
int launch_qfuse(pylda_ctx* ctx, hipStream_t st, const EstepParams& p, const Launch& L);
int launch_qfusek(pylda_ctx* ctx, hipStream_t st, const EstepParams& p, const Launch& L);
int launch_qgroup(pylda_ctx* ctx, hipStream_t st, const EstepParams& p, const Launch& L);

int compact_handoff_for(const pylda_ctx* ctx, const Launch& L);
void compact_caps(const pylda_ctx* ctx, int (&caps)[9]);
int prepare_compact(pylda_ctx* ctx, pylda_corpus* c);
int immortal_topics(const pylda_ctx* ctx);
bool alpha_allows_live(const pylda_ctx* ctx, bool was_off);
void release_postings(pylda_corpus* c);
int launch_compact(pylda_ctx* ctx, hipStream_t st, const pylda_corpus* c, EstepParams p, int slots, bool from_table, int64_t first, int64_t count);

int enqueue_prepare(pylda_ctx* ctx, bool heldout);
struct AlphaSums { double sum, lgamma_sum, term; };
AlphaSums alpha_sums(const pylda_ctx* ctx);
int finish_estep(pylda_ctx* ctx, pylda_corpus* c, int heldout, bool entropy, bool doc_values);

int build_postings(pylda_corpus* c);
int enqueue_sstats_gather(pylda_ctx* ctx, pylda_corpus* c);

int open_bracket(pylda_ctx* ctx, int slot, hipStream_t st);
void close_bracket(pylda_ctx* ctx, int at, hipStream_t st);
void drain_events(pylda_ctx* ctx);

}
```

### pylda_amd/csrc/launch_completion.hip

```cpp
#include "host_internal.h"
#include "completion_score.h"

namespace {

template <int S>
hipError_t launch_score(const CompletionParams& p, hipStream_t st)
{
    return launch_kernel(completion_score_kernel<S>, dim3((unsigned)((p.D + 3) / 4)), dim3(256), 0, st, p);
}

}

extern "C" {

int pylda_completion_set_model(pylda_ctx* ctx)
{
    if (!ctx) return PYLDA_ERR_INVALID;
    const int K = ctx->K, V = ctx->V, ldk = ctx->ldk;
    if (K > 64 * 16) return fail(ctx, PYLDA_ERR_INVALID, "completion_set_model: %d topics (at most 1024: 16 per lane)", K);
    if (!ctx->have_eta) return fail(ctx, PYLDA_ERR_STATE, "completion_set_model: eta was never set");
    HIP_TRY(ctx, hipSetDevice(ctx->device));
    const size_t cells = (size_t)V * ldk;
    if (!ctx->d_foldin_table) {
        const size_t need = cells * sizeof(double);
        size_t free_bytes = 0, total_bytes = 0;
        HIP_TRY(ctx, hipMemGetInfo(&free_bytes, &total_bytes));
        if (need + ((size_t)256 << 20) > free_bytes)
            return fail(ctx, PYLDA_ERR_OOM, "completion_set_model: the predictive table needs %zu MiB, %zu MiB of device memory are free",
                        need >> 20, free_bytes >> 20);
        FirstError A{ctx, "completion_set_model"};
        A(dev_alloc(ctx, &ctx->d_foldin_table, cells));
        A(dev_alloc(ctx, &ctx->d_foldin_alpha, (size_t)K));
        if (A.rc != PYLDA_OK) {
            dev_free(ctx->d_foldin_table); dev_free(ctx->d_foldin_alpha);
            return A.rc;
        }
    }
    if (!ctx->d_completion_rowsum) {
        const int rc = dev_alloc(ctx, &ctx->d_completion_rowsum, (size_t)K);
        if (rc != PYLDA_OK) return rc;
    }
    ctx->foldin_ready = false;
    ctx->completion_ready = false;
    HIP_TRY(ctx, launch_kernel(completion_rowsum_kernel, dim3((unsigned)K), dim3(256), 0, ctx->stream, ctx->d_eta, K, V,
                               ctx->d_completion_rowsum));
    HIP_TRY(ctx, launch_kernel(completion_table_kernel, dim3((unsigned)((V + 31) / 32), (unsigned)((ldk + 31) / 32)), dim3(256), 0,
                               ctx->stream, ctx->d_eta, ctx->d_completion_rowsum, K, V, ldk, ctx->d_foldin_table));
    ctx->completion_ready = true;
    return PYLDA_OK;
}

int pylda_completion_score(pylda_ctx* ctx, pylda_corpus* observed, pylda_corpus* held, const double* gamma_dk,
                           double* held_log_likelihood, int64_t* held_tokens)
{
    if (!ctx) return PYLDA_ERR_INVALID;
    if (!held || held->ctx != ctx) return fail(ctx, PYLDA_ERR_INVALID, "completion_score: the held corpus does not belong to this context");
    if (observed && observed->ctx != ctx)
        return fail(ctx, PYLDA_ERR_INVALID, "completion_score: the observed corpus does not belong to this context");
    if (ctx->K > 64 * 16) return fail(ctx, PYLDA_ERR_INVALID, "completion_score: %d topics (at most 1024: 16 per lane)", ctx->K);
    if ((observed != nullptr) == (gamma_dk != nullptr))
        return fail(ctx, PYLDA_ERR_INVALID, "completion_score: gamma comes from the observed corpus OR from gamma_dk (%s given)",
                    observed ? "both" : "neither");
    if (observed && observed->D != held->D)
        return fail(ctx, PYLDA_ERR_INVALID, "completion_score: the observed corpus has %lld documents, the held corpus %lld",
                    (long long)observed->D, (long long)held->D);
    if (!ctx->completion_ready && !ctx->foldin_ready)
        return fail(ctx, PYLDA_ERR_STATE, "completion_score: no predictive table (completion_set_model or foldin_set_model first)");
    if (held->gibbs_ready || (observed && observed->gibbs_ready))
        return fail(ctx, PYLDA_ERR_STATE, "completion_score: the %s corpus holds a Gibbs training state; score corpora of their own",
                    held->gibbs_ready ? "held" : "observed");
    if (observed && !observed->estep_done)
        return fail(ctx, PYLDA_ERR_STATE, "completion_score: no E-step or fold-in has run on the observed corpus");
    HIP_TRY(ctx, hipSetDevice(ctx->device));
    if (gamma_dk && held->D > 0)
        HIP_TRY(ctx, hipMemcpyAsync(held->d_gamma, gamma_dk, (size_t)held->D * ctx->K * sizeof(double), hipMemcpyHostToDevice, ctx->stream));

    CompletionParams p{};
    p.K = ctx->K;
    p.ldk = ctx->ldk;
    p.doc_ptr = held->d_doc_ptr;
    p.term_id = held->d_term_id;
    p.term_ct = held->d_term_ct;
    p.P = ctx->d_foldin_table;
    p.gamma = observed ? observed->d_gamma : held->d_gamma;
    p.doc_ll = held->d_doc_ll;
    p.doc_wll = held->d_doc_wll;
    p.iters = held->d_iters;
    p.status = held->d_status;
    p.D = held->D;

    const int bracket = open_bracket(ctx, -1, ctx->stream);
    if (held->D > 0) {
        hipError_t e;
        switch (gibbs_slots(ctx->K)) {
        case 1: e = launch_score<1>(p, ctx->stream); break;
        case 2: e = launch_score<2>(p, ctx->stream); break;
        case 4: e = launch_score<4>(p, ctx->stream); break;
        case 8: e = launch_score<8>(p, ctx->stream); break;
        default: e = launch_score<16>(p, ctx->stream); break;
        }
        HIP_TRY(ctx, e);
    }
    close_bracket(ctx, bracket, ctx->stream);
    HIP_TRY(ctx, launch_kernel(completion_sum_kernel, dim3(1), dim3(1024), 0, ctx->stream, held->d_doc_wll, held->d_status, held->D,
                               held->d_doc_ll, held->d_scalars, held->d_flag_count));
    double* sc = ctx->h_pin + (size_t)5 * ctx->K + 4;
    HIP_TRY(ctx, hipMemcpyAsync(sc, held->d_scalars, 4 * sizeof(double), hipMemcpyDeviceToHost, ctx->stream));
    HIP_TRY(ctx, hipStreamSynchronize(ctx->stream));
    const int32_t flagged = *reinterpret_cast<const int32_t*>(sc + 3);
    if (flagged) {
        held->estep_done = false;
        return fail(ctx, PYLDA_ERR_INVALID, "completion_score: %d gamma rows whose sum is not positive and finite", (int)flagged);
    }
    held->estep_done = true;
    held->last_heldout = 1;
    held->last_doc_values = true;
    if (held_log_likelihood) *held_log_likelihood = sc[1];
    if (held_tokens) *held_tokens = (int64_t)sc[2];
    return PYLDA_OK;
}

}
```

### pylda_amd/csrc/launch_foldin.hip

```cpp
#include "host_internal.h"
#include "estep_foldin.h"

namespace {

int prepare_tokens(pylda_ctx* ctx, pylda_corpus* c)
{
    if (c->d_tok_off) return PYLDA_OK;
    const int64_t nnz = c->nnz;
    const size_t need = ((size_t)nnz + 1 + (size_t)c->tokens) * sizeof(int64_t);
    size_t free_bytes = 0, total_bytes = 0;
    HIP_TRY(ctx, hipMemGetInfo(&free_bytes, &total_bytes));
    if (need + ((size_t)256 << 20) > free_bytes)
        return fail(ctx, PYLDA_ERR_OOM, "foldin: the token offsets and states need %zu MiB, %zu MiB of device memory are free",
                    need >> 20, free_bytes >> 20);
    std::vector<int32_t> cts((size_t)nnz);
    HIP_TRY(ctx, hipStreamSynchronize(ctx->stream));
    if (nnz) HIP_TRY(ctx, hipMemcpy(cts.data(), c->d_term_ct, (size_t)nnz * sizeof(int32_t), hipMemcpyDeviceToHost));
    std::vector<int64_t> tok_off((size_t)nnz + 1, 0);
    for (int64_t q = 0; q < nnz; ++q) tok_off[(size_t)q + 1] = tok_off[(size_t)q] + cts[(size_t)q];
    FirstError A{ctx, "foldin"};
    A(dev_alloc(ctx, &c->d_tok_off, (size_t)nnz + 1));
    A(dev_alloc(ctx, &c->d_hyb_state, (size_t)c->tokens));
    A.h2d(c->d_tok_off, tok_off.data(), tok_off.size() * sizeof(int64_t));
    if (A.rc != PYLDA_OK) {
// ... 7 lines not shown
{
    return launch_kernel(foldin_sample_kernel<S>, dim3((unsigned)((p.D + 3) / 4)), dim3(256), 0, st, p);
}

}

extern "C" {

int pylda_foldin_set_model(pylda_ctx* ctx, pylda_corpus* trained, const int32_t* n_kv, const int32_t* n_k, const double* beta_v,
                           double beta_sum)
{
    if (!ctx) return PYLDA_ERR_INVALID;
    const int K = ctx->K, V = ctx->V, ldk = ctx->ldk;
    if (K > 64 * 16) return fail(ctx, PYLDA_ERR_INVALID, "foldin_set_model: %d topics (at most 1024: 16 per lane)", K);
    if (!beta_v || !(beta_sum > 0.0)) return fail(ctx, PYLDA_ERR_INVALID, "foldin_set_model: beta or beta_sum missing");
    if (trained && trained->ctx != ctx) return fail(ctx, PYLDA_ERR_INVALID, "foldin_set_model: corpus does not belong to this context");
    if (trained && !trained->gibbs_ready) return fail(ctx, PYLDA_ERR_STATE, "foldin_set_model: the corpus holds no Gibbs state");
    if (!trained && (!n_kv || !n_k)) return fail(ctx, PYLDA_ERR_INVALID, "foldin_set_model: neither a trained corpus nor n_kv and n_k");
    HIP_TRY(ctx, hipSetDevice(ctx->device));
    const size_t cells = (size_t)V * ldk;
    if (!ctx->d_foldin_table) {
        const size_t need = cells * (sizeof(double) + sizeof(int32_t)) + (size_t)V * sizeof(double);
        size_t free_bytes = 0, total_bytes = 0;
        HIP_TRY(ctx, hipMemGetInfo(&free_bytes, &total_bytes));
        if (need + ((size_t)256 << 20) > free_bytes)
            return fail(ctx, PYLDA_ERR_OOM, "foldin_set_model: the predictive table needs %zu MiB, %zu MiB of device memory are free",
                        need >> 20, free_bytes >> 20);
        FirstError A{ctx, "foldin_set_model"};
        A(dev_alloc(ctx, &ctx->d_foldin_table, cells));
        A(dev_alloc(ctx, &ctx->d_foldin_alpha, (size_t)K));
        if (A.rc != PYLDA_OK) {
            dev_free(ctx->d_foldin_table); dev_free(ctx->d_foldin_alpha);
            return A.rc;
        }
    }
    ctx->foldin_ready = false;
    ctx->completion_ready = false;
    double* d_beta = nullptr;
    int32_t *d_counts = nullptr, *d_nk = nullptr;
    FirstError A{ctx, "foldin_set_model"};
    A(dev_alloc(ctx, &d_beta, (size_t)V));
    A.h2d(d_beta, beta_v, (size_t)V * sizeof(double));
    if (!trained) {
        std::vector<int32_t> table(cells, 0);
        for (int k = 0; k < K; ++k)
            for (int v = 0; v < V; ++v) table[(size_t)v * ldk + k] = n_kv[(size_t)k * V + v];
        A(dev_alloc(ctx, &d_counts, cells));
        A(dev_alloc(ctx, &d_nk, (size_t)K));
        A.h2d(d_counts, table.data(), cells * sizeof(int32_t));
        A.h2d(d_nk, n_k, (size_t)K * sizeof(int32_t));
    }
    hipError_t e = hipSuccess;
    if (A.rc == PYLDA_OK) {
        e = launch_kernel(foldin_table_kernel, dim3((unsigned)((cells + 255) / 256)), dim3(256), 0, ctx->stream,
                          trained ? trained->d_gibbs_table : d_counts, trained ? trained->d_gibbs_nk : d_nk, d_beta, beta_sum, K, V, ldk,
                          ctx->d_foldin_table);
        if (e == hipSuccess) e = hipStreamSynchronize(ctx->stream);
    }
    dev_free(d_beta); dev_free(d_counts); dev_free(d_nk);
    if (A.rc != PYLDA_OK) return A.rc;
    HIP_TRY(ctx, e);
    ctx->foldin_ready = true;
    return PYLDA_OK;
}

int pylda_foldin(pylda_ctx* ctx, pylda_corpus* c, const double* alpha_k, int number_of_samples, int burn_in_samples, uint64_t seed,
                 uint64_t stream, int64_t first_document, double* words_log_likelihood)
{
    if (!ctx) return PYLDA_ERR_INVALID;
    if (!c || c->ctx != ctx) return fail(ctx, PYLDA_ERR_INVALID, "foldin: corpus does not belong to this context");
    if (ctx->K > 64 * 16) return fail(ctx, PYLDA_ERR_INVALID, "foldin: %d topics (at most 1024: 16 per lane)", ctx->K);
    if (!alpha_k) return fail(ctx, PYLDA_ERR_INVALID, "foldin: alpha is NULL");
    if (number_of_samples < 1 || number_of_samples > 65534)
        return fail(ctx, PYLDA_ERR_INVALID, "foldin: number_of_samples=%d (1 to 65534: the sweep is 16 bits of a draw's name)", number_of_samples);
    if (burn_in_samples < 0 || burn_in_samples >= number_of_samples)
        return fail(ctx, PYLDA_ERR_INVALID, "foldin: number_of_samples=%d, burn_in_samples=%d (need 0 <= burn-in < samples)",
                    number_of_samples, burn_in_samples);
    if (stream > 0xffffffffull) return fail(ctx, PYLDA_ERR_INVALID, "foldin: stream %llu >= 2^32", (unsigned long long)stream);
    if (first_document < 0 || first_document + c->D > ((int64_t)1 << 32))
        return fail(ctx, PYLDA_ERR_INVALID, "foldin: first_document=%lld (global indices must stay below 2^32)", (long long)first_document);
    if (!ctx->foldin_ready) return fail(ctx, PYLDA_ERR_STATE, "foldin: foldin_set_model must be called first");
    if (c->gibbs_ready) return fail(ctx, PYLDA_ERR_STATE, "foldin: the corpus holds a Gibbs training state; fold in a corpus of its own");
    HIP_TRY(ctx, hipSetDevice(ctx->device));
    int rc = prepare_tokens(ctx, c);
    if (rc != PYLDA_OK) return rc;
    HIP_TRY(ctx, hipMemcpyAsync(ctx->d_foldin_alpha, alpha_k, (size_t)ctx->K * sizeof(double), hipMemcpyHostToDevice, ctx->stream));

    FoldinParams p{};
    p.K = ctx->K;
    p.V = ctx->V;
    p.ldk = ctx->ldk;
    p.doc_ptr = c->d_doc_ptr;
    p.term_id = c->d_term_id;
    p.term_ct = c->d_term_ct;
    p.tok_off = c->d_tok_off;
    p.state = c->d_hyb_state;
    p.P = ctx->d_foldin_table;
    p.alpha = ctx->d_foldin_alpha;
    p.gamma = c->d_gamma;
    p.doc_ll = c->d_doc_ll;
    p.doc_wll = c->d_doc_wll;
    p.iters = c->d_iters;
    p.D = c->D;
    p.samples = number_of_samples;
    p.burn_in = burn_in_samples;
    p.first_document = (uint32_t)first_document;
    p.stream = (uint32_t)stream;
    p.seed_lo = (uint32_t)seed;
    p.seed_hi = (uint32_t)(seed >> 32);

    const int bracket = open_bracket(ctx, -1, ctx->stream);
    if (c->D > 0) {
        hipError_t e;
        switch (gibbs_slots(ctx->K)) {
        case 1: e = launch_sampler<1>(p, ctx->stream); break;
        case 2: e = launch_sampler<2>(p, ctx->stream); break;
        case 4: e = launch_sampler<4>(p, ctx->stream); break;
        case 8: e = launch_sampler<8>(p, ctx->stream); break;
        default: e = launch_sampler<16>(p, ctx->stream); break;
        }
        HIP_TRY(ctx, e);
    }
    close_bracket(ctx, bracket, ctx->stream);
    HIP_TRY(ctx, launch_kernel(foldin_sum_kernel, dim3(1), dim3(256), 0, ctx->stream, c->d_doc_wll, c->D, c->d_scalars));
    c->estep_done = true;
    c->last_heldout = 1;
    c->last_doc_values = true;
    double* sc = ctx->h_pin + (size_t)5 * ctx->K + 4;
    HIP_TRY(ctx, hipMemcpyAsync(sc, c->d_scalars + 1, sizeof(double), hipMemcpyDeviceToHost, ctx->stream));
    HIP_TRY(ctx, hipStreamSynchronize(ctx->stream));
    if (words_log_likelihood) *words_log_likelihood = sc[0];
    return PYLDA_OK;
}

}
```

### pylda_amd/csrc/launch_gibbs.hip

```cpp
#include "host_internal.h"
#include "estep_gibbs.h"
#include "gibbs_exchange.h"

namespace {

int prepare_gibbs(pylda_ctx* ctx, pylda_corpus* c)
{
    if (c->d_gibbs_table) return PYLDA_OK;
    if (c->tokens >= ((int64_t)1 << 31))
        return fail(ctx, PYLDA_ERR_INVALID, "gibbs: %lld tokens (the count tables are int32: fewer than 2^31)", (long long)c->tokens);
    const int64_t nnz = c->nnz;
    const bool need_tokens = !c->d_tok_off;
    size_t need = (size_t)ctx->V * ctx->ldk * sizeof(int32_t) + (size_t)ctx->K * (sizeof(int32_t) + sizeof(double)) +
                  ((size_t)ctx->V * 2 + 2) * sizeof(double);
    if (need_tokens) need += ((size_t)nnz + 1 + (size_t)c->tokens) * sizeof(int64_t);
    size_t free_bytes = 0, total_bytes = 0;
    HIP_TRY(ctx, hipMemGetInfo(&free_bytes, &total_bytes));
    if (need + ((size_t)256 << 20) > free_bytes)
        return fail(ctx, PYLDA_ERR_OOM, "gibbs: the count table and the token states need %zu MiB, %zu MiB of device memory are free",
                    need >> 20, free_bytes >> 20);
    FirstError A{ctx, "gibbs"};
    if (need_tokens) {
        std::vector<int32_t> cts((size_t)nnz);
        HIP_TRY(ctx, hipStreamSynchronize(ctx->stream));
// ... 66 lines not shown

template <int S>
hipError_t launch_sampler(const GibbsParams& p, hipStream_t st)
{
    return launch_kernel(gibbs_sample_kernel<S>, dim3((unsigned)((p.count + 3) / 4)), dim3(256), 0, st, p);
}

hipError_t launch_sampler_for(const GibbsParams& p, hipStream_t st)
{
    switch (gibbs_slots(p.K)) {
    case 1: return launch_sampler<1>(p, st);
    case 2: return launch_sampler<2>(p, st);
    case 4: return launch_sampler<4>(p, st);
    case 8: return launch_sampler<8>(p, st);
    default: return launch_sampler<16>(p, st);
    }
}

hipError_t launch_round(const GibbsParams& p, hipStream_t st)
{
    const hipError_t e = launch_sampler_for(p, st);
    if (e != hipSuccess) return e;
    return launch_kernel(gibbs_apply_kernel, dim3((unsigned)((p.count + 3) / 4)), dim3(256), (size_t)p.K * sizeof(int), st, p);
}

void round_block(const pylda_corpus* c, int64_t blocks, int64_t first_document, int64_t g, int64_t* first, int64_t* count)
{
    *first = ((g - first_document) % blocks + blocks) % blocks;
    *count = *first < c->D ? (c->D - *first + blocks - 1) / blocks : 0;
}

int document_tokens(pylda_ctx* ctx, const pylda_corpus* c, std::vector<int64_t>* tokens)
{
    std::vector<int64_t> ptr((size_t)c->D + 1, 0);
    std::vector<int32_t> cts((size_t)c->nnz);
    HIP_TRY(ctx, hipMemcpy(ptr.data(), c->d_doc_ptr, ptr.size() * sizeof(int64_t), hipMemcpyDeviceToHost));
    if (c->nnz) HIP_TRY(ctx, hipMemcpy(cts.data(), c->d_term_ct, cts.size() * sizeof(int32_t), hipMemcpyDeviceToHost));
    tokens->assign((size_t)c->D, 0);
    for (int64_t d = 0; d < c->D; ++d)
        for (int64_t q = ptr[(size_t)d]; q < ptr[(size_t)d + 1]; ++q) (*tokens)[(size_t)d] += cts[(size_t)q];
    return PYLDA_OK;
}

int check_blocks(pylda_ctx* ctx, const char* what, int64_t blocks)
{
    if (blocks < 1) return fail(ctx, PYLDA_ERR_INVALID, "%s: blocks=%lld (at least 1)", what, (long long)blocks);
    if (blocks > ((int64_t)1 << 24))
        return fail(ctx, PYLDA_ERR_INVALID, "%s: blocks=%lld (at most 2^24; above the global document count pass that count)", what, (long long)blocks);
    return PYLDA_OK;
}

struct PosteriorScalars {
    double alpha_sum = 0.0, beta_sum = 0.0, alpha_lg = 0.0, beta_lg = 0.0;
};

int posterior_terms(pylda_ctx* ctx, pylda_corpus* c, const char* what, const double* alpha_k, const double* beta_v, bool has_out,
                    PosteriorScalars* h)
{
    int rc = check_call(ctx, c, what, 0);
    if (rc != PYLDA_OK) return rc;
    if (!c->gibbs_ready) return fail(ctx, PYLDA_ERR_STATE, "%s: gibbs_init or gibbs_set_state must be called first", what);
    if (!alpha_k || !beta_v || !has_out) return fail(ctx, PYLDA_ERR_INVALID, "%s: alpha, beta or out is NULL", what);
    HIP_TRY(ctx, hipSetDevice(ctx->device));
    if ((rc = upload_priors(ctx, c, alpha_k, beta_v)) != PYLDA_OK) return rc;
    for (int k = 0; k < ctx->K; ++k) { h->alpha_sum += alpha_k[k]; h->alpha_lg += std::lgamma(alpha_k[k]); }
    for (int v = 0; v < ctx->V; ++v) { h->beta_sum += beta_v[v]; h->beta_lg += std::lgamma(beta_v[v]); }
    if (c->D > 0)
        HIP_TRY(ctx, launch_kernel(gibbs_doc_posterior_kernel, dim3((unsigned)((c->D + 3) / 4)), dim3(256), 0, ctx->stream,
                                   c->d_gamma, c->d_gibbs_alpha, h->alpha_sum, ctx->K, c->D, c->d_doc_ll));
    HIP_TRY(ctx, launch_kernel(gibbs_word_posterior_kernel, dim3((unsigned)ctx->V), dim3(256), 0, ctx->stream, c->d_gibbs_table,
                               c->d_gibbs_beta, ctx->K, ctx->ldk, c->d_gibbs_words));
    return PYLDA_OK;
}

}

extern "C" {

int pylda_gibbs_init(pylda_ctx* ctx, pylda_corpus* c, uint64_t seed, int64_t first_document)
{
    if (!ctx) return PYLDA_ERR_INVALID;
    int rc = check_call(ctx, c, "gibbs_init", first_document);
    if (rc != PYLDA_OK) return rc;
    HIP_TRY(ctx, hipSetDevice(ctx->device));
    if ((rc = prepare_gibbs(ctx, c)) != PYLDA_OK) return rc;
    GibbsParams p = gibbs_params(ctx, c);
    p.first_document = (uint32_t)first_document;
    p.seed_lo = (uint32_t)seed;
    p.seed_hi = (uint32_t)(seed >> 32);
    HIP_TRY(ctx, hipMemsetAsync(c->d_gibbs_table, 0, (size_t)ctx->V * ctx->ldk * sizeof(int32_t), ctx->stream));
    HIP_TRY(ctx, hipMemsetAsync(c->d_gibbs_nk, 0, (size_t)ctx->K * sizeof(int32_t), ctx->stream));
    if (c->D > 0)
        HIP_TRY(ctx, launch_kernel(gibbs_init_kernel, dim3((unsigned)((c->D + 3) / 4)), dim3(256), (size_t)4 * ctx->K * sizeof(int),
                                   ctx->stream, p));
    c->gibbs_ready = true;
    c->estep_done = true;
    return PYLDA_OK;
}

int pylda_gibbs_sweep(pylda_ctx* ctx, pylda_corpus* c, const double* alpha_k, const double* beta_v, double beta_sum, int64_t blocks,
                      uint64_t seed, uint64_t stream, int64_t first_document)
{
    if (!ctx) return PYLDA_ERR_INVALID;
    int rc = check_call(ctx, c, "gibbs_sweep", first_document);
    if (rc != PYLDA_OK) return rc;
    if (!c->gibbs_ready) return fail(ctx, PYLDA_ERR_STATE, "gibbs_sweep: gibbs_init or gibbs_set_state must be called first");
    if (!alpha_k || !beta_v || !(beta_sum > 0.0)) return fail(ctx, PYLDA_ERR_INVALID, "gibbs_sweep: alpha, beta or beta_sum missing");
    if (blocks < 1) return fail(ctx, PYLDA_ERR_INVALID, "gibbs_sweep: blocks=%lld (at least 1)", (long long)blocks);
    if (stream > 0xffffffffull) return fail(ctx, PYLDA_ERR_INVALID, "gibbs_sweep: stream %llu >= 2^32", (unsigned long long)stream);
    HIP_TRY(ctx, hipSetDevice(ctx->device));
    if ((rc = upload_priors(ctx, c, alpha_k, beta_v)) != PYLDA_OK) return rc;
    GibbsParams p = gibbs_params(ctx, c);
    p.beta_sum = beta_sum;
    p.first_document = (uint32_t)first_document;
    p.stream = (uint32_t)stream;
    p.seed_lo = (uint32_t)seed;
    p.seed_hi = (uint32_t)(seed >> 32);
    p.step = blocks;
    const int bracket = open_bracket(ctx, -1, ctx->stream);
    const int64_t g_begin = blocks >= first_document + c->D ? first_document : 0;
    for (int64_t g = g_begin; g < std::min<int64_t>(blocks, first_document + c->D); ++g) {
        p.first = ((g - first_document) % blocks + blocks) % blocks;
        p.count = p.first < c->D ? (c->D - p.first + blocks - 1) / blocks : 0;
        if (p.count > 0) HIP_TRY(ctx, launch_round(p, ctx->stream));
    }
    close_bracket(ctx, bracket, ctx->stream);
    return PYLDA_OK;
}

int pylda_gibbs_log_posterior(pylda_ctx* ctx, pylda_corpus* c, const double* alpha_k, const double* beta_v, double* out)
{
    if (!ctx) return PYLDA_ERR_INVALID;
    PosteriorScalars h;
    const int rc = posterior_terms(ctx, c, "gibbs_log_posterior", alpha_k, beta_v, out != nullptr, &h);
    if (rc != PYLDA_OK) return rc;
    double* d_out = c->d_gibbs_words + ctx->V;
    HIP_TRY(ctx, launch_kernel(gibbs_posterior_sum_kernel, dim3(1), dim3(256), 0, ctx->stream, c->d_doc_ll, c->D, c->d_gibbs_words,
                               ctx->V, c->d_gibbs_nk, ctx->K, h.beta_sum, d_out));
    double device_sum = 0.0;
    HIP_TRY(ctx, hipMemcpyAsync(&device_sum, d_out, sizeof(double), hipMemcpyDeviceToHost, ctx->stream));
    HIP_TRY(ctx, hipStreamSynchronize(ctx->stream));
    *out = (std::lgamma(h.alpha_sum) - h.alpha_lg) * (double)c->D + (std::lgamma(h.beta_sum) - h.beta_lg) * (double)ctx->K + device_sum;
    return PYLDA_OK;
}

int pylda_gibbs_get_counts(pylda_ctx* ctx, pylda_corpus* c, int32_t* n_kv, int32_t* n_k, int32_t* topics)
{
    if (!ctx) return PYLDA_ERR_INVALID;
    int rc = check_call(ctx, c, "gibbs_get_counts", 0);
    if (rc != PYLDA_OK) return rc;
    if (!c->gibbs_ready) return fail(ctx, PYLDA_ERR_STATE, "gibbs_get_counts: gibbs_init or gibbs_set_state must be called first");
    HIP_TRY(ctx, hipSetDevice(ctx->device));
    HIP_TRY(ctx, hipStreamSynchronize(ctx->stream));
    const int K = ctx->K, V = ctx->V, ldk = ctx->ldk;
    if (n_kv) {
        std::vector<int32_t> table((size_t)V * ldk);
        HIP_TRY(ctx, hipMemcpy(table.data(), c->d_gibbs_table, table.size() * sizeof(int32_t), hipMemcpyDeviceToHost));
        for (int v = 0; v < V; ++v)
            for (int k = 0; k < K; ++k) n_kv[(size_t)k * V + v] = table[(size_t)v * ldk + k];
    }
    if (n_k) HIP_TRY(ctx, hipMemcpy(n_k, c->d_gibbs_nk, (size_t)K * sizeof(int32_t), hipMemcpyDeviceToHost));
    if (topics && c->tokens) {
        std::vector<uint64_t> state((size_t)c->tokens);
        HIP_TRY(ctx, hipMemcpy(state.data(), c->d_hyb_state, state.size() * sizeof(uint64_t), hipMemcpyDeviceToHost));
        const uint64_t mask = ((uint64_t)1 << gibbs_bits(K)) - 1;
        for (size_t t = 0; t < state.size(); ++t) topics[t] = (int32_t)(state[t] & mask);
    }
    return PYLDA_OK;
}

int pylda_gibbs_set_state(pylda_ctx* ctx, pylda_corpus* c, const int32_t* n_kv, const int32_t* n_k, const int32_t* topics)
{
    if (!ctx) return PYLDA_ERR_INVALID;
    int rc = check_call(ctx, c, "gibbs_set_state", 0);
    if (rc != PYLDA_OK) return rc;
    HIP_TRY(ctx, hipSetDevice(ctx->device));
    const bool fresh = !c->gibbs_ready;
    if (fresh && (!n_kv || !n_k || !topics))
        return fail(ctx, PYLDA_ERR_STATE, "gibbs_set_state: a corpus without a state needs the table, n_k and the topics");
    if ((rc = prepare_gibbs(ctx, c)) != PYLDA_OK) return rc;
    const int K = ctx->K, V = ctx->V, ldk = ctx->ldk, bits = gibbs_bits(K);
    HIP_TRY(ctx, hipStreamSynchronize(ctx->stream));
    if (n_kv) {
        std::vector<int32_t> table((size_t)V * ldk, 0);
        for (int k = 0; k < K; ++k)
            for (int v = 0; v < V; ++v) table[(size_t)v * ldk + k] = n_kv[(size_t)k * V + v];
        HIP_TRY(ctx, hipMemcpy(c->d_gibbs_table, table.data(), table.size() * sizeof(int32_t), hipMemcpyHostToDevice));
    }
    if (n_k) HIP_TRY(ctx, hipMemcpy(c->d_gibbs_nk, n_k, (size_t)K * sizeof(int32_t), hipMemcpyHostToDevice));
    if (topics) {
        std::vector<uint64_t> state((size_t)c->tokens);
        for (size_t t = 0; t < state.size(); ++t) {
            if (topics[t] < 0 || topics[t] >= K) return fail(ctx, PYLDA_ERR_INVALID, "gibbs_set_state: topic %d of token %zu", topics[t], t);
            state[t] = (uint64_t)topics[t] | ((uint64_t)topics[t] << bits);
        }
        if (c->tokens)
            HIP_TRY(ctx, hipMemcpy(c->d_hyb_state, state.data(), state.size() * sizeof(uint64_t), hipMemcpyHostToDevice));
        if (c->D > 0)
            HIP_TRY(ctx, launch_kernel(gibbs_recount_kernel, dim3((unsigned)((c->D + 3) / 4)), dim3(256), (size_t)4 * K * sizeof(int),
                                       ctx->stream, gibbs_params(ctx, c)));
    }
    c->gibbs_ready = true;
    c->estep_done = true;
    return PYLDA_OK;
}

int pylda_gibbs_round_tokens(pylda_ctx* ctx, pylda_corpus* c, int64_t blocks, int64_t first_document, int64_t* tokens)
{
    if (!ctx) return PYLDA_ERR_INVALID;
    int rc = check_call(ctx, c, "gibbs_round_tokens", first_document);
    if (rc != PYLDA_OK) return rc;
    if ((rc = check_blocks(ctx, "gibbs_round_tokens", blocks)) != PYLDA_OK) return rc;
    if (!tokens) return fail(ctx, PYLDA_ERR_INVALID, "gibbs_round_tokens: tokens is NULL");
    HIP_TRY(ctx, hipSetDevice(ctx->device));
    std::vector<int64_t> doc_tokens;
    if ((rc = document_tokens(ctx, c, &doc_tokens)) != PYLDA_OK) return rc;
    for (int64_t g = 0; g < blocks; ++g) tokens[g] = 0;
    for (int64_t d = 0; d < c->D; ++d) tokens[(first_document + d) % blocks] += doc_tokens[(size_t)d];
    return PYLDA_OK;
}

int pylda_gibbs_exchange_prepare(pylda_ctx* ctx, pylda_corpus* c, int64_t blocks, int64_t first_document, int world, int rank,
                                 const int64_t* capacity, void** send, void** recv)
{
    if (!ctx) return PYLDA_ERR_INVALID;
    int rc = check_call(ctx, c, "gibbs_exchange_prepare", first_document);
    if (rc != PYLDA_OK) return rc;
    if ((rc = check_blocks(ctx, "gibbs_exchange_prepare", blocks)) != PYLDA_OK) return rc;
    if (!capacity || !send || !recv) return fail(ctx, PYLDA_ERR_INVALID, "gibbs_exchange_prepare: capacity, send or recv is NULL");
    if (world < 1 || rank < 0 || rank >= world)
        return fail(ctx, PYLDA_ERR_INVALID, "gibbs_exchange_prepare: rank %d of %d", rank, world);
    HIP_TRY(ctx, hipSetDevice(ctx->device));
    std::vector<int64_t> doc_tokens;
    if ((rc = document_tokens(ctx, c, &doc_tokens)) != PYLDA_OK) return rc;
    std::vector<int64_t> round_tokens((size_t)blocks, 0), rec_off((size_t)c->D, 0);
    for (int64_t d = 0; d < c->D; ++d) {
        int64_t& at = round_tokens[(size_t)((first_document + d) % blocks)];
        rec_off[(size_t)d] = at;
        at += doc_tokens[(size_t)d];
    }
    int64_t widest = 0;
    for (int64_t g = 0; g < blocks; ++g) {
        if (capacity[g] < round_tokens[(size_t)g])
            return fail(ctx, PYLDA_ERR_INVALID, "gibbs_exchange_prepare: capacity[%lld]=%lld, this corpus has %lld tokens in that round",
                        (long long)g, (long long)capacity[g], (long long)round_tokens[(size_t)g]);
        widest = std::max(widest, capacity[g]);
    }
    if (widest >= ((int64_t)1 << 31) / world * 256)
        return fail(ctx, PYLDA_ERR_INVALID, "gibbs_exchange_prepare: %lld records per rank and round", (long long)widest);
    const size_t need = ((size_t)widest * ((size_t)world + 1) + (size_t)c->D) * sizeof(int64_t);
    size_t held = 0;
    if (c->gibbs_exchange_world) {
        int64_t old_widest = 0;
        for (int64_t cap : c->h_gibbs_capacity) old_widest = std::max(old_widest, cap);
        held = ((size_t)old_widest * ((size_t)c->gibbs_exchange_world + 1) + (size_t)c->D) * sizeof(int64_t);
    }
    size_t free_bytes = 0, total_bytes = 0;
    HIP_TRY(ctx, hipMemGetInfo(&free_bytes, &total_bytes));
    if (need + ((size_t)256 << 20) > free_bytes + held)
        return fail(ctx, PYLDA_ERR_OOM, "gibbs_exchange_prepare: the record buffers of %d ranks need %zu MiB, %zu MiB of device memory are free",
                    world, need >> 20, (free_bytes + held) >> 20);
    HIP_TRY(ctx, hipStreamSynchronize(ctx->stream));
    dev_free(c->d_gibbs_send); dev_free(c->d_gibbs_recv); dev_free(c->d_gibbs_rec_off);
    c->gibbs_exchange_world = 0;
    FirstError A{ctx, "gibbs_exchange_prepare"};
    A(dev_alloc(ctx, &c->d_gibbs_send, (size_t)widest));
    A(dev_alloc(ctx, &c->d_gibbs_recv, (size_t)widest * (size_t)world));
    A(dev_alloc(ctx, &c->d_gibbs_rec_off, (size_t)c->D));
    A.h2d(c->d_gibbs_rec_off, rec_off.data(), rec_off.size() * sizeof(int64_t));
    if (A.rc != PYLDA_OK) {
        dev_free(c->d_gibbs_send); dev_free(c->d_gibbs_recv); dev_free(c->d_gibbs_rec_off);
        return A.rc;
    }
    c->h_gibbs_capacity.assign(capacity, capacity + blocks);
    c->h_gibbs_round_tokens.swap(round_tokens);
    c->gibbs_exchange_blocks = blocks;
    c->gibbs_exchange_first = first_document;
    c->gibbs_exchange_world = world;
    *send = c->d_gibbs_send;
    *recv = c->d_gibbs_recv;
    return PYLDA_OK;
}

int pylda_gibbs_round_sample(pylda_ctx* ctx, pylda_corpus* c, const double* alpha_k, const double* beta_v, double beta_sum, int64_t blocks,
                             int64_t round, uint64_t seed, uint64_t stream, int64_t first_document)
{
    if (!ctx) return PYLDA_ERR_INVALID;
    int rc = check_call(ctx, c, "gibbs_round_sample", first_document);
    if (rc != PYLDA_OK) return rc;
    if (!c->gibbs_ready) return fail(ctx, PYLDA_ERR_STATE, "gibbs_round_sample: gibbs_init or gibbs_set_state must be called first");
    if (!alpha_k || !beta_v || !(beta_sum > 0.0)) return fail(ctx, PYLDA_ERR_INVALID, "gibbs_round_sample: alpha, beta or beta_sum missing");
    if (blocks < 1) return fail(ctx, PYLDA_ERR_INVALID, "gibbs_round_sample: blocks=%lld (at least 1)", (long long)blocks);
    if (stream > 0xffffffffull) return fail(ctx, PYLDA_ERR_INVALID, "gibbs_round_sample: stream %llu >= 2^32", (unsigned long long)stream);
    if (!c->gibbs_exchange_world) return fail(ctx, PYLDA_ERR_STATE, "gibbs_round_sample: gibbs_exchange_prepare must be called first");
    if (blocks != c->gibbs_exchange_blocks || first_document != c->gibbs_exchange_first)
        return fail(ctx, PYLDA_ERR_STATE, "gibbs_round_sample: blocks=%lld, first_document=%lld; the exchange was prepared for %lld, %lld",
                    (long long)blocks, (long long)first_document, (long long)c->gibbs_exchange_blocks, (long long)c->gibbs_exchange_first);
    if (round < 0 || round >= blocks) return fail(ctx, PYLDA_ERR_STATE, "gibbs_round_sample: round %lld of %lld", (long long)round, (long long)blocks);
    HIP_TRY(ctx, hipSetDevice(ctx->device));
    if ((rc = upload_priors(ctx, c, alpha_k, beta_v)) != PYLDA_OK) return rc;
    GibbsParams p = gibbs_params(ctx, c);
    p.beta_sum = beta_sum;
    p.first_document = (uint32_t)first_document;
    p.stream = (uint32_t)stream;
    p.seed_lo = (uint32_t)seed;
    p.seed_hi = (uint32_t)(seed >> 32);
    p.step = blocks;
    round_block(c, blocks, first_document, round, &p.first, &p.count);
    const dim3 grid((unsigned)((p.count + 3) / 4));
    if (p.count > 0) {
        const int bracket = open_bracket(ctx, -1, ctx->stream);
        const hipError_t e = launch_sampler_for(p, ctx->stream);
        close_bracket(ctx, bracket, ctx->stream);
        HIP_TRY(ctx, e);
    }
    const int64_t mine = c->h_gibbs_round_tokens[(size_t)round], cap = c->h_gibbs_capacity[(size_t)round];
    const int bracket = open_bracket(ctx, -2, ctx->stream);
    hipError_t e = hipSuccess;
    if (cap > mine) e = hipMemsetAsync(c->d_gibbs_send + mine, 0, (size_t)(cap - mine) * sizeof(uint64_t), ctx->stream);
    if (e == hipSuccess && p.count > 0)
        e = launch_kernel(gibbs_pack_kernel, grid, dim3(256), 0, ctx->stream, p, (const int64_t*)c->d_gibbs_rec_off, c->d_gibbs_send);
    close_bracket(ctx, bracket, ctx->stream);
    HIP_TRY(ctx, e);
    return PYLDA_OK;
}

int pylda_gibbs_round_apply(pylda_ctx* ctx, pylda_corpus* c, int64_t round)
{
    if (!ctx) return PYLDA_ERR_INVALID;
    int rc = check_call(ctx, c, "gibbs_round_apply", 0);
    if (rc != PYLDA_OK) return rc;
    if (!c->gibbs_ready) return fail(ctx, PYLDA_ERR_STATE, "gibbs_round_apply: gibbs_init or gibbs_set_state must be called first");
    if (!c->gibbs_exchange_world) return fail(ctx, PYLDA_ERR_STATE, "gibbs_round_apply: gibbs_exchange_prepare must be called first");
    if (round < 0 || round >= c->gibbs_exchange_blocks)
        return fail(ctx, PYLDA_ERR_STATE, "gibbs_round_apply: round %lld of %lld", (long long)round, (long long)c->gibbs_exchange_blocks);
    HIP_TRY(ctx, hipSetDevice(ctx->device));
    const int64_t n = c->h_gibbs_capacity[(size_t)round] * c->gibbs_exchange_world;
    if (n == 0) return PYLDA_OK;
    const int bracket = open_bracket(ctx, -2, ctx->stream);
    const hipError_t e = launch_kernel(gibbs_record_apply_kernel, dim3((unsigned)((n + 255) / 256)), dim3(256), (size_t)ctx->K * sizeof(int),
                                       ctx->stream, (const uint64_t*)c->d_gibbs_recv, n, c->d_gibbs_table, c->d_gibbs_nk, ctx->K, ctx->V, ctx->ldk);
    close_bracket(ctx, bracket, ctx->stream);
    HIP_TRY(ctx, e);
    return PYLDA_OK;
}

int pylda_gibbs_table_device(pylda_ctx* ctx, pylda_corpus* c, void** table, int64_t* table_elements, void** n_k)
{
    if (!ctx) return PYLDA_ERR_INVALID;
    int rc = check_call(ctx, c, "gibbs_table_device", 0);
    if (rc != PYLDA_OK) return rc;
    if (!c->gibbs_ready) return fail(ctx, PYLDA_ERR_STATE, "gibbs_table_device: gibbs_init or gibbs_set_state must be called first");
    if (table) *table = c->d_gibbs_table;
    if (table_elements) *table_elements = (int64_t)ctx->V * ctx->ldk;
    if (n_k) *n_k = c->d_gibbs_nk;
    return PYLDA_OK;
}

int pylda_gibbs_log_posterior_parts(pylda_ctx* ctx, pylda_corpus* c, const double* alpha_k, const double* beta_v, double* out)
{
    if (!ctx) return PYLDA_ERR_INVALID;
    PosteriorScalars h;
    const int rc = posterior_terms(ctx, c, "gibbs_log_posterior_parts", alpha_k, beta_v, out != nullptr, &h);
    if (rc != PYLDA_OK) return rc;
    double* d_out = c->d_gibbs_words + ctx->V;
    HIP_TRY(ctx, launch_kernel(gibbs_posterior_parts_kernel, dim3(1), dim3(256), 0, ctx->stream, c->d_doc_ll, c->D, c->d_gibbs_words,
                               ctx->V, c->d_gibbs_nk, ctx->K, h.beta_sum, d_out));
    double device_sums[2] = {0.0, 0.0};
    HIP_TRY(ctx, hipMemcpyAsync(device_sums, d_out, sizeof(device_sums), hipMemcpyDeviceToHost, ctx->stream));
    HIP_TRY(ctx, hipStreamSynchronize(ctx->stream));
    out[0] = (std::lgamma(h.alpha_sum) - h.alpha_lg) * (double)c->D + device_sums[0];
    out[1] = (std::lgamma(h.beta_sum) - h.beta_lg) * (double)ctx->K + device_sums[1];
    return PYLDA_OK;
}

int pylda_test_gibbs_posterior_terms(pylda_ctx* ctx, pylda_corpus* c, const double* alpha_k, const double* beta_v, double* doc_terms,
                                     double* word_terms, double* sums)
{
    if (!ctx) return PYLDA_ERR_INVALID;
    PosteriorScalars h;
    const int rc = posterior_terms(ctx, c, "test_gibbs_posterior_terms", alpha_k, beta_v, doc_terms && word_terms && sums, &h);
    if (rc != PYLDA_OK) return rc;
    double* d_out = c->d_gibbs_words + ctx->V;
    HIP_TRY(ctx, launch_kernel(gibbs_posterior_sum_kernel, dim3(1), dim3(256), 0, ctx->stream, c->d_doc_ll, c->D, c->d_gibbs_words,
                               ctx->V, c->d_gibbs_nk, ctx->K, h.beta_sum, d_out));
    HIP_TRY(ctx, hipMemcpyAsync(sums, d_out, sizeof(double), hipMemcpyDeviceToHost, ctx->stream));
    HIP_TRY(ctx, hipStreamSynchronize(ctx->stream));
    HIP_TRY(ctx, launch_kernel(gibbs_posterior_parts_kernel, dim3(1), dim3(256), 0, ctx->stream, c->d_doc_ll, c->D, c->d_gibbs_words,
                               ctx->V, c->d_gibbs_nk, ctx->K, h.beta_sum, d_out));
    HIP_TRY(ctx, hipMemcpyAsync(sums + 1, d_out, 2 * sizeof(double), hipMemcpyDeviceToHost, ctx->stream));
    if (c->D > 0)
        HIP_TRY(ctx, hipMemcpyAsync(doc_terms, c->d_doc_ll, (size_t)c->D * sizeof(double), hipMemcpyDeviceToHost, ctx->stream));
    HIP_TRY(ctx, hipMemcpyAsync(word_terms, c->d_gibbs_words, (size_t)ctx->V * sizeof(double), hipMemcpyDeviceToHost, ctx->stream));
    HIP_TRY(ctx, hipStreamSynchronize(ctx->stream));
    return PYLDA_OK;
}

}
```

### pylda_amd/csrc/launch_hybrid.hip

```cpp
#include "host_internal.h"
#include "estep_hybrid.h"

namespace {

int prepare_hybrid(pylda_ctx* ctx, pylda_corpus* c, bool postings)
{
    const bool need_tokens = !c->d_tok_off, need_postings = postings && !c->d_hyb_post_pos;
    if (!need_tokens && !need_postings) return PYLDA_OK;
    const int64_t nnz = c->nnz;
    const int V = ctx->V;
    size_t need = 0;
    if (need_tokens) need += ((size_t)nnz + 1 + (size_t)c->tokens) * sizeof(int64_t);
    if (need_postings) need += ((size_t)nnz + (size_t)V + 1) * sizeof(int64_t);
    size_t free_bytes = 0, total_bytes = 0;
    HIP_TRY(ctx, hipMemGetInfo(&free_bytes, &total_bytes));
    const size_t headroom = (size_t)256 << 20;
    if (need + headroom > free_bytes)
        return fail(ctx, PYLDA_ERR_OOM, "hybrid_estep: the sample histories and offsets need %zu MiB, %zu MiB of device memory are free",
                    need >> 20, free_bytes >> 20);
    std::vector<int32_t> ids(need_postings ? (size_t)nnz : 0), cts(need_tokens ? (size_t)nnz : 0);
    HIP_TRY(ctx, hipStreamSynchronize(ctx->stream));
    if (nnz && need_postings)
        HIP_TRY(ctx, hipMemcpy(ids.data(), c->d_term_id, (size_t)nnz * sizeof(int32_t), hipMemcpyDeviceToHost));
    if (nnz && need_tokens)
// ... 4 lines not shown
        for (int64_t q = 0; q < nnz; ++q) tok_off[(size_t)q + 1] = tok_off[(size_t)q] + cts[(size_t)q];
        A(dev_alloc(ctx, &c->d_tok_off, (size_t)nnz + 1));
        A(dev_alloc(ctx, &c->d_hyb_state, (size_t)c->tokens));
        A.h2d(c->d_tok_off, tok_off.data(), tok_off.size() * sizeof(int64_t));
        if (A.rc != PYLDA_OK) {
            dev_free(c->d_tok_off); dev_free(c->d_hyb_state);
            return A.rc;
        }
    }
    if (need_postings) {
        std::vector<int64_t> col_ptr((size_t)V + 1, 0), post((size_t)nnz);
        for (int64_t q = 0; q < nnz; ++q) col_ptr[(size_t)ids[(size_t)q] + 1] += 1;
        for (int v = 0; v < V; ++v) col_ptr[(size_t)v + 1] += col_ptr[(size_t)v];
        {
            std::vector<int64_t> at(col_ptr.begin(), col_ptr.end() - 1);
            for (int64_t q = 0; q < nnz; ++q) post[(size_t)at[(size_t)ids[(size_t)q]]++] = q;
        }
        A(dev_alloc(ctx, &c->d_hyb_col_ptr, (size_t)V + 1));
        A(dev_alloc(ctx, &c->d_hyb_post_pos, (size_t)nnz));
        A.h2d(c->d_hyb_col_ptr, col_ptr.data(), col_ptr.size() * sizeof(int64_t));
        A.h2d(c->d_hyb_post_pos, post.data(), post.size() * sizeof(int64_t));
        if (A.rc != PYLDA_OK) {
            dev_free(c->d_hyb_col_ptr); dev_free(c->d_hyb_post_pos);
        }
    }
    return A.rc;
}

HybridParams hybrid_params(const pylda_ctx* ctx, const pylda_corpus* c, int heldout)
{
    HybridParams p{};
    p.K = ctx->K;
    p.V = ctx->V;
    p.ldk = ctx->ldk;
    p.B = ctx->d_expElog;
    p.alpha = ctx->d_alpha;
    p.eta = ctx->d_eta;
    p.psi_rowsum = ctx->d_psi_rowsum;
    p.doc_ptr = c->d_doc_ptr;
    p.term_id = c->d_term_id;
    p.term_ct = c->d_term_ct;
    p.tok_off = c->d_tok_off;
    p.state = c->d_hyb_state;
    p.gamma = c->d_gamma;
    p.doc_ll = c->d_doc_ll;
    p.doc_wll = c->d_doc_wll;
    p.iters = c->d_iters;
    p.status = c->d_status;
    p.D = c->D;
    p.heldout = heldout;
    p.alpha_term = alpha_sums(ctx).term;
    return p;
}

template <int S>
void launch_sampler(const HybridParams& p, hipStream_t st)
{
    hipLaunchKernelGGL(hybrid_sample_kernel<S>, dim3((unsigned)((p.D + 3) / 4)), dim3(256), 0, st, p);
}

}

extern "C" {

int pylda_hybrid_estep(pylda_ctx* ctx, pylda_corpus* c, int number_of_samples, int burn_in_samples, uint64_t seed,
                       uint64_t stream, int64_t first_document, int heldout)
{
    if (!ctx) return PYLDA_ERR_INVALID;
    if (!c || c->ctx != ctx) return fail(ctx, PYLDA_ERR_INVALID, "hybrid_estep: corpus does not belong to this context");
    const int K = ctx->K, bits = hybrid_bits(K);
    if (number_of_samples < 1 || burn_in_samples < 0 || burn_in_samples >= number_of_samples)
        return fail(ctx, PYLDA_ERR_INVALID, "hybrid_estep: number_of_samples=%d, burn_in_samples=%d (need 0 <= burn-in < samples)",
                    number_of_samples, burn_in_samples);
    if ((int64_t)(number_of_samples - burn_in_samples + 1) * bits > 64)
        return fail(ctx, PYLDA_ERR_INVALID, "hybrid_estep: %d post-burn-in samples of %d bits each do not fit a token's 64-bit history",
                    number_of_samples - burn_in_samples, bits);
    if (stream > 0xffffffffull) return fail(ctx, PYLDA_ERR_INVALID, "hybrid_estep: stream %llu >= 2^32", (unsigned long long)stream);
    if (first_document < 0 || first_document + c->D > ((int64_t)1 << 32))
        return fail(ctx, PYLDA_ERR_INVALID, "hybrid_estep: first_document=%lld (global indices must stay below 2^32)", (long long)first_document);
    if (!ctx->have_eta || !ctx->have_alpha)
        return fail(ctx, PYLDA_ERR_STATE, "hybrid_estep: set_eta and set_alpha must be called first");
    HIP_TRY(ctx, hipSetDevice(ctx->device));
    heldout = heldout ? 1 : 0;
    int rc = prepare_hybrid(ctx, c, heldout == 0);
    if (rc != PYLDA_OK) return rc;
    if ((rc = enqueue_prepare(ctx, false)) != PYLDA_OK) return rc;

    HybridParams p = hybrid_params(ctx, c, heldout);
    p.first_document = (uint32_t)first_document;
    p.stream = (uint32_t)stream;
    p.seed_lo = (uint32_t)seed;
    p.seed_hi = (uint32_t)(seed >> 32);
    p.samples = number_of_samples;
    p.burn_in = burn_in_samples;
    p.bits = bits;

    const int doc_bracket = open_bracket(ctx, -1, ctx->stream);
    if (c->D > 0) {
        switch (hybrid_slots(K)) {
        case 1: launch_sampler<1>(p, ctx->stream); break;
        case 2: launch_sampler<2>(p, ctx->stream); break;
        case 4: launch_sampler<4>(p, ctx->stream); break;
        case 8: launch_sampler<8>(p, ctx->stream); break;
        default: launch_sampler<16>(p, ctx->stream); break;
        }
        HIP_TRY(ctx, hipGetLastError());
    }
    close_bracket(ctx, doc_bracket, ctx->stream);
    const int ss_bracket = open_bracket(ctx, -2, ctx->stream);
    if (!heldout) {
        hipLaunchKernelGGL(hybrid_sstats_kernel, dim3((unsigned)ctx->V), dim3(256), (size_t)K * sizeof(unsigned), ctx->stream,
                           c->d_hyb_col_ptr, c->d_hyb_post_pos, c->d_tok_off, c->d_hyb_state, K, ctx->ldk, number_of_samples,
                           burn_in_samples, bits, ctx->d_sstats);
        HIP_TRY(ctx, hipGetLastError());
    }
    close_bracket(ctx, ss_bracket, ctx->stream);
    if (doc_bracket >= 0 && ss_bracket >= 0) ctx->estep_calls += 1;
    return finish_estep(ctx, c, heldout, false, true);
}

int pylda_hybrid_scale_sstats(pylda_ctx* ctx, double divisor)
{
    if (!ctx) return PYLDA_ERR_INVALID;
    if (!(divisor > 0.0)) return fail(ctx, PYLDA_ERR_INVALID, "hybrid_scale_sstats: divisor %g", divisor);
    if (!ctx->have_sstats) return fail(ctx, PYLDA_ERR_STATE, "hybrid_scale_sstats: no training-mode E-step has run");
    HIP_TRY(ctx, hipSetDevice(ctx->device));
    const int64_t n = (int64_t)ctx->V * ctx->ldk;
    const unsigned grid = (unsigned)std::max<int64_t>(1, std::min<int64_t>((n + 255) / 256, 4 * (int64_t)ctx->num_cu));
    hipLaunchKernelGGL(hybrid_scale_kernel, dim3(grid), dim3(256), 0, ctx->stream, ctx->d_sstats, n, divisor);
    HIP_TRY(ctx, hipGetLastError());
    return PYLDA_OK;
}

int pylda_test_philox(pylda_ctx* ctx, int64_t n, const uint32_t* counter_key, uint32_t* out)
{
    if (!ctx) return PYLDA_ERR_INVALID;
    if (n < 0 || !counter_key || !out) return fail(ctx, PYLDA_ERR_INVALID, "test_philox: bad argument");
    if (n == 0) return PYLDA_OK;
    HIP_TRY(ctx, hipSetDevice(ctx->device));
    uint32_t *din = nullptr, *dout = nullptr;
    int rc = dev_alloc(ctx, &din, (size_t)n * 6);
    if (rc == PYLDA_OK) rc = dev_alloc(ctx, &dout, (size_t)n * 4);
    if (rc == PYLDA_OK) {
        hipError_t e = hipMemcpy(din, counter_key, (size_t)n * 6 * sizeof(uint32_t), hipMemcpyHostToDevice);
        if (e == hipSuccess) {
            hipLaunchKernelGGL(philox_test_kernel, dim3((unsigned)((n + 255) / 256)), dim3(256), 0, ctx->stream, din, n, dout);
            e = hipStreamSynchronize(ctx->stream);
        }
        if (e == hipSuccess) e = hipMemcpy(out, dout, (size_t)n * 4 * sizeof(uint32_t), hipMemcpyDeviceToHost);
        if (e != hipSuccess) rc = fail(ctx, PYLDA_ERR_HIP, "test_philox: %s", hipGetErrorString(e));
    }
    dev_free(din);
    dev_free(dout);
    return rc;
}

}
```

### pylda_amd/csrc/mstep_api.hip

```cpp
#include "host_internal.h"
#include "mstep_kernels.h"

extern "C" {

namespace {
struct OnlineBlend { double rho, omr, scale; };

static int enqueue_mstep(pylda_ctx* ctx, pylda_corpus* c, const double* beta_v, bool want_alpha_ss, const char* who,
                         const OnlineBlend* blend = nullptr)
{
    if (!beta_v) return fail(ctx, PYLDA_ERR_INVALID, "%s: beta is NULL", who);
    if (!ctx->have_eta || !ctx->have_sstats)
        return fail(ctx, PYLDA_ERR_STATE, "%s: needs eta and the sufficient statistics of a training E-step", who);
    if (want_alpha_ss && (!c || c->ctx != ctx || !c->estep_done))
        return fail(ctx, PYLDA_ERR_STATE, "%s: alpha statistics need the corpus of the last E-step", who);
    HIP_TRY(ctx, hipSetDevice(ctx->device));
    const int K = ctx->K, V = ctx->V;
    if (ctx->h_beta.size() != (size_t)V || memcmp(ctx->h_beta.data(), beta_v, (size_t)V * sizeof(double)) != 0) {
        double bsum = 0.0, blg = 0.0;
        for (int v = 0; v < V; ++v) {
            if (!(beta_v[v] > 0.0)) return fail(ctx, PYLDA_ERR_INVALID, "%s: beta[%d]=%g", who, v, beta_v[v]);
            bsum += beta_v[v];
            blg += std::lgamma(beta_v[v]);
        }
        ctx->h_beta.clear();
        HIP_TRY(ctx, hipMemcpyAsync(ctx->d_beta, beta_v, (size_t)V * sizeof(double), hipMemcpyHostToDevice, ctx->stream));
        HIP_TRY(ctx, hipStreamSynchronize(ctx->stream));
        ctx->h_beta.assign(beta_v, beta_v + V);
        ctx->beta_sum = bsum;
        ctx->beta_lgamma_sum = blg;
    }
    double* d_per_topic = ctx->d_small;
    double* d_alpha_ss = ctx->d_small + K;
    hipLaunchKernelGGL(mstep_topic_ll_kernel, dim3(K, kTopicChunks), dim3(256), 0, ctx->stream, ctx->d_eta, K, V,
                       ctx->d_partial);
    hipLaunchKernelGGL(mstep_topic_ll_finish_kernel, dim3((K + 255) / 256), dim3(256), 0, ctx->stream, ctx->d_partial, K,
                       d_per_topic);
    if (blend)
        hipLaunchKernelGGL(mstep_online_eta_kernel, dim3((K + 31) / 32, (V + 31) / 32), dim3(256), 0, ctx->stream,
                           ctx->d_sstats, ctx->d_beta, K, V, ctx->ldk, blend->rho, blend->omr, blend->scale, ctx->d_eta);
    else
        hipLaunchKernelGGL(mstep_update_eta_kernel, dim3((K + 31) / 32, (V + 31) / 32), dim3(256), 0, ctx->stream,
                           ctx->d_sstats, ctx->d_beta, K, V, ctx->ldk, ctx->d_eta);
    if (want_alpha_ss) {
        const int nblocks = (int)std::min<int64_t>(1024, std::max<int64_t>(1, (c->D + 3) / 4));
        hipLaunchKernelGGL(mstep_alpha_ss_kernel, dim3(nblocks), dim3(256), (size_t)4 * K * sizeof(double),
                           ctx->stream, c->d_gamma, c->D, K, ctx->d_partial);
        hipLaunchKernelGGL(column_sum_kernel, dim3((K + 63) / 64), dim3(256), 0, ctx->stream, ctx->d_partial,
                           nblocks, K, d_alpha_ss);
    }
    HIP_TRY(ctx, hipGetLastError());
    return PYLDA_OK;
}

static double topic_ll_from(const pylda_ctx* ctx, const double* per_topic)
{
    double ll = ctx->K * (std::lgamma(ctx->beta_sum) - ctx->beta_lgamma_sum);
    for (int k = 0; k < ctx->K; ++k) ll += per_topic[k];
    return ll;
}
}

int pylda_mstep(pylda_ctx* ctx, pylda_corpus* c, const double* beta_v, double* topic_log_likelihood,
                double* alpha_ss_k)
{
    if (!ctx) return PYLDA_ERR_INVALID;
    const int rc = enqueue_mstep(ctx, c, beta_v, alpha_ss_k != nullptr, "mstep");
    if (rc != PYLDA_OK) return rc;
    const int K = ctx->K;
    std::vector<double> per_topic((size_t)K);
    HIP_TRY(ctx, hipMemcpyAsync(per_topic.data(), ctx->d_small, (size_t)K * sizeof(double), hipMemcpyDeviceToHost, ctx->stream));
    if (alpha_ss_k)
        HIP_TRY(ctx, hipMemcpyAsync(alpha_ss_k, ctx->d_small + K, (size_t)K * sizeof(double), hipMemcpyDeviceToHost, ctx->stream));
    HIP_TRY(ctx, hipStreamSynchronize(ctx->stream));
    if (topic_log_likelihood) *topic_log_likelihood = topic_ll_from(ctx, per_topic.data());
    return PYLDA_OK;
}

int pylda_mstep_enqueue(pylda_ctx* ctx, pylda_corpus* c, const double* beta_v, int hyper_parameter_iteration,
                        double hyper_parameter_decay_factor, int hyper_parameter_maximum_decay,
                        double hyper_parameter_converge_threshold)
{
    if (!ctx) return PYLDA_ERR_INVALID;
    if (!c || c->ctx != ctx || !c->estep_done || c->last_heldout)
        return fail(ctx, PYLDA_ERR_STATE, "mstep_enqueue: needs the corpus of the last training-mode E-step");
    if (hyper_parameter_iteration < 0 || hyper_parameter_maximum_decay < 0 || hyper_parameter_maximum_decay > 16)
        return fail(ctx, PYLDA_ERR_INVALID, "mstep_enqueue: hyper_parameter_iteration=%d, hyper_parameter_maximum_decay=%d (0..16)",
                    hyper_parameter_iteration, hyper_parameter_maximum_decay);
    ctx->newton_pending = hyper_parameter_iteration > 0;
    if (ctx->newton_pending) {
        ctx->newton.iterations = hyper_parameter_iteration;
        ctx->newton.maximum_decay = hyper_parameter_maximum_decay;
        ctx->newton.threshold = hyper_parameter_converge_threshold;
        for (int d = 0; d <= 16; ++d) ctx->newton.decay_power[d] = std::pow(hyper_parameter_decay_factor, (double)d);
    }
    const int rc = enqueue_mstep(ctx, c, beta_v, true, "mstep_enqueue");
    if (rc != PYLDA_OK) return rc;
    const int K = ctx->K;
    hipLaunchKernelGGL(outer_pack_kernel, dim3(1), dim3(256), 0, ctx->stream, c->d_scalars, c->d_flag_count,
                       c->last_doc_values ? 1 : 0, (double)c->D, ctx->d_small + K, ctx->d_small, ctx->d_alpha, K, ctx->d_outer);
    HIP_TRY(ctx, hipGetLastError());
    ctx->outer_ready = true;
    return PYLDA_OK;
}

namespace {
static int online_blend_from(pylda_ctx* ctx, double rho, double scale, const char* who, OnlineBlend* blend)
{
    if (!(rho > 0.0 && rho <= 1.0)) return fail(ctx, PYLDA_ERR_INVALID, "%s: rho=%g is outside (0, 1]", who, rho);
    if (!std::isfinite(scale) || !(scale > 0.0)) return fail(ctx, PYLDA_ERR_INVALID, "%s: scale=%g is not a positive number", who, scale);
    blend->rho = rho;
    blend->omr = 1.0 - rho;
    blend->scale = scale;
    return PYLDA_OK;
}
}

int pylda_mstep_online(pylda_ctx* ctx, pylda_corpus* c, const double* beta_v, double rho, double scale,
                       double* topic_log_likelihood, double* alpha_ss_k)
{
    if (!ctx) return PYLDA_ERR_INVALID;
    OnlineBlend blend;
    int rc = online_blend_from(ctx, rho, scale, "mstep_online", &blend);
    if (rc != PYLDA_OK) return rc;
    rc = enqueue_mstep(ctx, c, beta_v, alpha_ss_k != nullptr, "mstep_online", &blend);
    if (rc != PYLDA_OK) return rc;
    const int K = ctx->K;
    std::vector<double> per_topic((size_t)K);
    HIP_TRY(ctx, hipMemcpyAsync(per_topic.data(), ctx->d_small, (size_t)K * sizeof(double), hipMemcpyDeviceToHost, ctx->stream));
    if (alpha_ss_k)
        HIP_TRY(ctx, hipMemcpyAsync(alpha_ss_k, ctx->d_small + K, (size_t)K * sizeof(double), hipMemcpyDeviceToHost, ctx->stream));
    HIP_TRY(ctx, hipStreamSynchronize(ctx->stream));
    if (topic_log_likelihood) *topic_log_likelihood = topic_ll_from(ctx, per_topic.data());
    return PYLDA_OK;
// ... 101 lines not shown
```

### pylda_amd/csrc/mstep_kernels.h

```cpp
#pragma once
#include "estep_common.h"
#include "special_device.h"
#include "estep_limits.h"

namespace pylda {

constexpr int kTopicChunks = 8;
__global__ __launch_bounds__(256) void mstep_topic_ll_kernel(const double* __restrict__ eta, int K,
                                                             int V, double* __restrict__ part)
{
    __shared__ double scratch[4];
    const int k = blockIdx.x, chunk = blockIdx.y;
    const int per = (V + kTopicChunks - 1) / kTopicChunks;
    const int v0 = chunk * per, v1 = min(V, v0 + per);
    const double* row = eta + (size_t)k * V;
    double lg = 0.0, s = 0.0;
    for (int v = v0 + threadIdx.x; v < v1; v += 256) {
        const double e = row[v];
        lg += lgamma_pos(e);
        s += e;
    }
    lg = block_sum<256>(lg, scratch);
    s = block_sum<256>(s, scratch);
    if (threadIdx.x == 0) {
        part[((size_t)k * kTopicChunks + chunk) * 2] = lg;
        part[((size_t)k * kTopicChunks + chunk) * 2 + 1] = s;
    }
}

__global__ __launch_bounds__(256) void mstep_topic_ll_finish_kernel(const double* __restrict__ part, int K,
                                                                    double* __restrict__ per_topic)
{
    const int k = blockIdx.x * 256 + threadIdx.x;
    if (k >= K) return;
    double lg = 0.0, s = 0.0;
#pragma unroll
    for (int c = 0; c < kTopicChunks; ++c) {
        lg += part[((size_t)k * kTopicChunks + c) * 2];
        s += part[((size_t)k * kTopicChunks + c) * 2 + 1];
    }
    per_topic[k] = lg - lgamma_pos(s);
}

__global__ __launch_bounds__(256) void mstep_update_eta_kernel(const double* __restrict__ sstats_wk,
                                                               const double* __restrict__ beta,
                                                               int K, int V, int ldk,
                                                               double* __restrict__ eta)
{
    __shared__ double tile[32][33];
    const int tx = threadIdx.x & 31, ty = threadIdx.x >> 5;
    const int k0 = blockIdx.x * 32, v0 = blockIdx.y * 32;
#pragma unroll
    for (int j = 0; j < 4; ++j) {
        const int v = v0 + ty + j * 8, k = k0 + tx;
        if (v < V && k < K) tile[ty + j * 8][tx] = sstats_wk[(size_t)v * ldk + k];
    }
    __syncthreads();
#pragma unroll
    for (int j = 0; j < 4; ++j) {
        const int k = k0 + ty + j * 8, v = v0 + tx;
        if (v < V && k < K) eta[(size_t)k * V + v] = tile[tx][ty + j * 8] + beta[v];
    }
}

__global__ __launch_bounds__(256) void mstep_online_eta_kernel(const double* __restrict__ sstats_wk,
                                                               const double* __restrict__ beta,
                                                               int K, int V, int ldk, double rho, double omr,
                                                               double scale, double* eta)
{
    __shared__ double tile[32][33];
    const int tx = threadIdx.x & 31, ty = threadIdx.x >> 5;
    const int k0 = blockIdx.x * 32, v0 = blockIdx.y * 32;
#pragma unroll
    for (int j = 0; j < 4; ++j) {
        const int v = v0 + ty + j * 8, k = k0 + tx;
        if (v < V && k < K) tile[ty + j * 8][tx] = sstats_wk[(size_t)v * ldk + k];
    }
    __syncthreads();
#pragma unroll
    for (int j = 0; j < 4; ++j) {
        const int k = k0 + ty + j * 8, v = v0 + tx;
        if (v < V && k < K) {
            const size_t at = (size_t)k * V + v;
            const double m = scale * tile[tx][ty + j * 8];
            const double a = m + beta[v];
            const double b = rho * a;
            const double c = omr * eta[at];
            eta[at] = c + b;
        }
    }
}

__global__ __launch_bounds__(256) void mstep_alpha_ss_kernel(const double* __restrict__ gamma,
                                                             int64_t D, int K,
                                                             double* __restrict__ partial)
{
    extern __shared__ __attribute__((aligned(16))) char smem[];
    double* acc = reinterpret_cast<double*>(smem);
    const int lane = threadIdx.x & (kWave - 1), wave = threadIdx.x / kWave;
    for (int k = lane; k < K; k += kWave) acc[wave * K + k] = 0.0;
    const int64_t stride = (int64_t)gridDim.x * 4;
    for (int64_t d = (int64_t)blockIdx.x * 4 + wave; d < D; d += 2 * stride) {
        const double* g0 = gamma + (size_t)d * K;
        const bool two = d + stride < D;
        const double* g1 = two ? gamma + (size_t)(d + stride) * K : g0;
        double s0 = 0.0, s1 = 0.0;
        for (int k = lane; k < K; k += kWave) {
            s0 += g0[k];
            s1 += g1[k];
        }
        s0 = wave_sum(s0);
        s1 = wave_sum(s1);
        const double ps0 = digamma(s0), ps1 = digamma(s1);
        for (int k = lane; k < K; k += kWave) {
            double a = acc[wave * K + k] + (digamma(g0[k]) - ps0);
            if (two) a += digamma(g1[k]) - ps1;
            acc[wave * K + k] = a;
        }
    }
    __syncthreads();
    for (int k = threadIdx.x; k < K; k += 256)
        partial[(size_t)blockIdx.x * K + k] = acc[k] + acc[K + k] + acc[2 * K + k] + acc[3 * K + k];
}

__global__ __launch_bounds__(256) void column_sum_kernel(const double* __restrict__ partial,
                                                         int nblocks, int K,
                                                         double* __restrict__ out)
{
    __shared__ double part[4][64];
    const int kk = threadIdx.x & 63, grp = threadIdx.x >> 6;
    const int k = blockIdx.x * 64 + kk;
    double s = 0.0;
    if (k < K)
        for (int b = grp; b < nblocks; b += 4) s += partial[(size_t)b * K + k];
    part[grp][kk] = s;
    __syncthreads();
    if (grp == 0 && k < K) out[k] = (part[0][kk] + part[1][kk]) + (part[2][kk] + part[3][kk]);
}

__global__ __launch_bounds__(256) void outer_pack_kernel(const double* __restrict__ scalars, const int32_t* __restrict__ flag_count,
                                                         int doc_values, double n_docs, const double* __restrict__ alpha_ss,
                                                         const double* __restrict__ per_topic, const double* __restrict__ alpha,
                                                         int K, double* __restrict__ out)
{
    if (threadIdx.x == 0) {
        out[0] = doc_values ? scalars[0] : scalars[0] - scalars[2];
        out[1] = n_docs;
        out[2] = (double)flag_count[0];
        out[3] = 0.0;
    }
    for (int k = threadIdx.x; k < K; k += 256) {
        out[4 + k] = alpha_ss[k];
        out[4 + K + k] = per_topic[k];
        out[4 + 2 * K + k] = alpha[k];
    }
}

__global__ __launch_bounds__(1024) void alpha_newton_kernel(double* __restrict__ io, const double* __restrict__ stats,
                                                            const double* __restrict__ docs_ptr, int K, NewtonParams np,
                                                            double* __restrict__ work, double* __restrict__ alpha_device)
{
    __shared__ double scratch[16];
    const int tid = threadIdx.x;
    const double docs = docs_ptr[0];
    double* alpha = work;
    double* update = work + K;
    double* grad = work + 2 * (size_t)K;
    double* hess = work + 3 * (size_t)K;
    for (int k = tid; k < K; k += 1024) alpha[k] = update[k] = io[k];
    __syncthreads();
    int decay = 0;
    for (int it = 0; it < np.iterations; ++it) {
        double part = 0.0;
        for (int k = tid; k < K; k += 1024) part += alpha[k];
        const double alpha_sum = block_sum<1024>(part, scratch);
        const double psi_sum = digamma(alpha_sum);
        part = 0.0;
        for (int k = tid; k < K; k += 1024) {
            const double a = alpha[k];
            const double g = docs * (psi_sum - digamma(a)) + stats[k];
            const double h = -docs * trigamma(a);
            grad[k] = g;
            hess[k] = h;
            part += g / h;
        }
        const double sum_g_h = block_sum<1024>(part, scratch);
        const double z = docs * trigamma(alpha_sum);
        bool accepted_step = false;
        for (;;) {
            const double scale = np.decay_power[decay];
            int singular = 0;
            for (int k = tid; k < K; k += 1024) {
                const double c = sum_g_h / (1.0 / z + 1.0 / hess[k]);
                const double step = scale * (grad[k] - c) / hess[k];
                if (alpha[k] <= step) singular = 1;
            }
            if (__syncthreads_or(singular)) {
                decay += 1;
                if (decay > np.maximum_decay) break;
            } else {
                accepted_step = true;
                break;
            }
        }
        part = 0.0;
        for (int k = tid; k < K; k += 1024) {
            if (accepted_step) {
                const double c = sum_g_h / (1.0 / z + 1.0 / hess[k]);
                update[k] = alpha[k] - np.decay_power[decay] * (grad[k] - c) / hess[k];
            }
            part += fabs(update[k] - alpha[k]);
            alpha[k] = update[k];
// ... 13 lines not shown
```

### pylda_amd/csrc/plan.hip

```cpp
#include "host_internal.h"

namespace pylda_host {

PlanConfig plan_config(const pylda_ctx* ctx)
{
    PlanConfig cfg;
    cfg.K = ctx->K;
    cfg.V = ctx->V;
    cfg.ldk = ctx->ldk;
    cfg.num_cu = ctx->num_cu;
    cfg.lds_limit = ctx->lds_limit;
    cfg.force_variant = ctx->force_variant;
    cfg.exact_stop = ctx->exact_stop;
    cfg.quad = ctx->quad;
    cfg.quad_stream = ctx->quad_stream;
    cfg.quilt12 = ctx->quilt12;
    cfg.quilt_odd = ctx->quilt_odd;
    cfg.slab_uber = ctx->slab_uber;
    return cfg;
}

void build_plan(pylda_corpus* c)
{
    pylda_ctx* ctx = c->ctx;
    c->plan_epoch = ctx->plan_epoch;
    c->plan_exact = ctx->exact_stop;
    c->plan = build_launch_classes(plan_config(ctx), c->h_terms_sorted.data(), c->D);
    c->plan_serial += 1;
}

int slab_uber_from(const pylda_ctx* ctx, const pylda_corpus* c) { return pylda_plan::slab_uber_from(plan_config(ctx), c->plan); }

}

extern "C" {

int64_t pylda_corpus_layout(pylda_corpus* c, const char* name)
{
    if (!c || !name) return PYLDA_ERR_INVALID;
    if (!strcmp(name, "gather_blocks")) return c->have_postings ? c->gather_blocks : 0;
    if (!strcmp(name, "gather_segments")) return c->have_postings ? c->nseg : 0;
    if (!strcmp(name, "gather_rounds")) return c->have_postings ? (int64_t)c->rounds.size() : 0;
    if (!strcmp(name, "gather_sweep_passes")) return c->have_postings && c->sweep ? c->sweep_passes : 0;
    if (!strcmp(name, "gather_sweep_terms")) return c->have_postings && c->sweep ? c->sweep_terms : 0;
    if (!strcmp(name, "gather_sweep_wpb")) return c->have_postings && c->sweep ? c->sweep_wpb : 0;
    if (!strcmp(name, "gather_partial_rows")) return c->have_postings ? c->partial_rows : 0;
    if (!strcmp(name, "gather_live")) return c->have_postings && c->live_stats ? 1 : 0;
    if (!strcmp(name, "live_off_by_alpha")) return c->live_off_by_alpha ? 1 : 0;
    if (!strcmp(name, "quad_slot_bytes")) return c->d_quad_rec && c->quad_slots_serial == c->plan_serial ? c->quad_slots.bytes() : 0;
    return fail(c->ctx, PYLDA_ERR_INVALID, "corpus_layout: unknown name '%s'", name);
}

int pylda_corpus_plan(pylda_corpus* c, int32_t capacity, int32_t* variant, int32_t* geometry, int64_t* documents,
                      int64_t* terms, double* kernel_ms)
{
    if (!c || !c->ctx || capacity < 0) return PYLDA_ERR_INVALID;
    pylda_ctx* ctx = c->ctx;
    if (c->plan_epoch != ctx->plan_epoch || c->plan_exact != ctx->exact_stop) build_plan(c);
    if (kernel_ms) {
        if (hipSetDevice(ctx->device) == hipSuccess) drain_events(ctx);
    }
    const int n = (int)std::min<size_t>(c->plan.size(), (size_t)capacity);
    for (int i = 0; i < n; ++i) {
        const Launch& L = c->plan[(size_t)i];
        if (variant) variant[i] = L.variant;
        if (geometry) geometry[i] = L.rn;
        if (documents) documents[i] = L.count;
        if (terms) {
            int64_t t = 0;
            for (int64_t j = L.first; j < L.first + L.count; ++j) t += c->h_terms_sorted[(size_t)j];
            terms[i] = t;
        }
        if (kernel_ms) {
            kernel_ms[i] = (size_t)i < ctx->class_ms.size() ? ctx->class_ms[(size_t)i] : 0.0;
            if ((size_t)i < ctx->class_ms.size()) ctx->class_ms[(size_t)i] = 0.0;
        }
    }
    return (int)c->plan.size();
}

}
```

Before: 5.008 million.

## Compute alpha sufficient statistics early on aux stream; parallelize work counting

Launches the alpha sufficient-statistics reduction over gamma on an auxiliary stream right after the document phase, so it overlaps the sstats gather. After finish_estep it re-runs the reduction only when documents were redone, signalled through the flag count. The M-step then copies the precomputed result instead of launching the reduction itself. A new multi-block work_count kernel replaces the single-block one in profiling mode. Adds invalidation hooks wherever gamma is rewritten, at the cost of extra buffers and stream synchronisation complexity.

Result: no change. 5.047 million, median of 6 (+0.8%).

```diff
diff --git a/include/pylda_hip.h b/include/pylda_hip.h
--- a/include/pylda_hip.h
+++ b/include/pylda_hip.h
@@ -178,6 +178,8 @@
 int pylda_test_tables(pylda_ctx* ctx, double* psi_rowsum_k, double* elog_vldk, double* expElog_vldk,
                       double* expElog_elog_vldk, double* shift_v, double* topic_lse_k, double* alpha_sgn_k, int* path_out);
 
+int pylda_test_handover(pylda_ctx* ctx, pylda_corpus* corpus, int32_t* handoff_it_d, int32_t* col_iters_d);
+
 int pylda_test_statistics(pylda_ctx* ctx, pylda_corpus* corpus, const double* t_dldk, const double* r_nnz,
                           const int32_t* live_n_d, const uint16_t* live_topic_d60, const double* live_t_d60,
                           double* entropy_out);
diff --git a/pylda_amd/_capi.py b/pylda_amd/_capi.py
--- a/pylda_amd/_capi.py
+++ b/pylda_amd/_capi.py
@@ -83,6 +83,7 @@
     "pylda_test_special_forms": (ctypes.c_int, [_vp, ctypes.c_int64, _c_double_p, ctypes.c_double, ctypes.c_int, _c_double_p]),
     "pylda_test_tables": (ctypes.c_int, [_vp, _c_double_p, _c_double_p, _c_double_p, _c_double_p, _c_double_p, _c_double_p,
                                          _c_double_p, ctypes.POINTER(ctypes.c_int)]),
+    "pylda_test_handover": (ctypes.c_int, [_vp, _vp, _c_int32_p, _c_int32_p]),
     "pylda_test_statistics": (ctypes.c_int, [_vp, _vp, _c_double_p, _c_double_p, _c_int32_p, ctypes.POINTER(ctypes.c_uint16),
                                              _c_double_p, _c_double_p]),
     "pylda_test_special": (ctypes.c_int, [_vp, ctypes.c_int64, _c_double_p, _c_double_p, _c_double_p]),
@@ -719,6 +720,11 @@
         self._check(self._lib.pylda_test_special(self._h, x.size, _dp(x), _dp(dg), _dp(lg)))
         return dg, lg
 
+    def test_handover(self, corpus):
+        handoff_it, col_iters = np.empty(corpus.D, dtype=np.int32), np.empty(corpus.D, dtype=np.int32)
+        self._check(self._lib.pylda_test_handover(self._h, corpus._h, _ip(handoff_it), _ip(col_iters)))
+        return handoff_it, col_iters
+
     def test_tables(self, alpha_sgn=False, tables=True, only=None):
         ldk = int(self._lib.pylda_table_stride(self._h))
         out = {}
diff --git a/pylda_amd/csrc/context.hip b/pylda_amd/csrc/context.hip
--- a/pylda_amd/csrc/context.hip
+++ b/pylda_amd/csrc/context.hip
@@ -182,6 +182,7 @@
     CREATE_TRY(dev_alloc(ctx, &ctx->d_alpha_wsum, (size_t)1));
     CREATE_TRY(dev_alloc(ctx, &ctx->d_small, (size_t)(4 * K + 16)));
     CREATE_TRY(dev_alloc(ctx, &ctx->d_partial, (size_t)1024 * K));
+    CREATE_TRY(dev_alloc(ctx, &ctx->d_early_partial, (size_t)1024 * K));
     CREATE_TRY(dev_alloc(ctx, &ctx->d_outer, (size_t)(3 * K + 8)));
     CREATE_TRY(dev_alloc(ctx, &ctx->d_newton_work, (size_t)4 * K));
     CREATE_TRY(dev_alloc(ctx, &ctx->d_work, (size_t)6));
@@ -212,7 +213,7 @@
     dev_free(ctx->d_eta); dev_free(ctx->d_elog); dev_free(ctx->d_expElog); dev_free(ctx->d_expElog_elog); dev_free(ctx->d_sstats);
     dev_free(ctx->d_kv_scratch); dev_free(ctx->d_shift); dev_free(ctx->d_beta);
     dev_free(ctx->d_psi_rowsum); dev_free(ctx->d_topic_lse); dev_free(ctx->d_alpha); dev_free(ctx->d_alpha_sgn); dev_free(ctx->d_alpha_wsum);
-    dev_free(ctx->d_small); dev_free(ctx->d_partial); dev_free(ctx->d_outer); dev_free(ctx->d_newton_work); dev_free(ctx->d_work); dev_free(ctx->d_eta_ckpt);
+    dev_free(ctx->d_small); dev_free(ctx->d_partial); dev_free(ctx->d_early_partial); dev_free(ctx->d_outer); dev_free(ctx->d_newton_work); dev_free(ctx->d_work); dev_free(ctx->d_eta_ckpt);
     if (ctx->h_pin) (void)hipHostFree(ctx->h_pin);
     for (int i = 0; i < 2; ++i)
         if (ctx->alpha_event[i]) (void)hipEventDestroy(ctx->alpha_event[i]);
@@ -284,6 +285,10 @@
         ctx->launch_order = (int)value;
     } else if (!strcmp(name, "terms_overlap")) {
         ctx->terms_overlap = value != 0;
+    } else if (!strcmp(name, "alpha_ss_early")) {
+        ctx->alpha_ss_early = value != 0;
+    } else if (!strcmp(name, "work_count_grid")) {
+        ctx->work_count_grid = value != 0;
     } else if (!strcmp(name, "slab_uber")) {
         ctx->slab_uber = value != 0;
     } else if (!strcmp(name, "wide_postings")) {
@@ -426,7 +431,13 @@
 int pylda_compute_units(const pylda_ctx* ctx) { return ctx ? ctx->num_cu : 0; }
 void* pylda_sstats_device(pylda_ctx* ctx) { return ctx ? ctx->d_sstats : nullptr; }
 void* pylda_eta_device(pylda_ctx* ctx) { return ctx ? ctx->d_eta : nullptr; }
-void* pylda_gamma_device(pylda_corpus* c) { return c ? c->d_gamma : nullptr; }
+void* pylda_gamma_device(pylda_corpus* c)
+{
+    if (!c) return nullptr;
+    c->gamma_escaped = true;
+    gamma_rewritten(c);
+    return c->d_gamma;
+}
 
 int pylda_mark_device_state(pylda_ctx* ctx, int have_eta, int have_sstats)
 {
diff --git a/pylda_amd/csrc/estep_api.hip b/pylda_amd/csrc/estep_api.hip
--- a/pylda_amd/csrc/estep_api.hip
+++ b/pylda_amd/csrc/estep_api.hip
@@ -149,6 +149,8 @@
     A(dev_alloc(ctx, &c->d_doc_ll, D));
     A(dev_alloc(ctx, &c->d_doc_wll, D));
     A(dev_alloc(ctx, &c->d_iters, D));
+    A(dev_alloc(ctx, &c->d_work_partial, work_count_partials(c->D)));
+    A(dev_alloc(ctx, &c->d_alpha_early, (size_t)ctx->K));
     A(dev_alloc(ctx, &c->d_status, D));
     A(dev_alloc(ctx, &c->d_scalars, (size_t)4));
     c->d_flag_count = c->d_scalars ? reinterpret_cast<int32_t*>(c->d_scalars + 3) : nullptr;
@@ -400,7 +402,34 @@
     return false;
 }
 
-int enqueue_statistics(pylda_ctx* ctx, pylda_corpus* c, bool terms_forked)
+struct AlphaEarly {
+    pylda_ctx* ctx;
+    bool launched = false, forked = false;
+    bool wanted(const pylda_corpus* c, const EstepParams& p) const
+    {
+        if (p.heldout || !ctx->alpha_ss_early || c->D <= 0 || c->gamma_escaped || ctx->force_logspace) return false;
+        return c->have_postings && !c->sweep;
+    }
+    void start(pylda_corpus* c)
+    {
+        if (hipEventRecord(ctx->fork_event, ctx->stream) != hipSuccess ||
+            hipStreamWaitEvent(ctx->aux_stream[1], ctx->fork_event, 0) != hipSuccess) {
+            (void)hipGetLastError();
+            return;
+        }
+        launched = enqueue_alpha_ss(ctx, c, ctx->aux_stream[1], ctx->d_early_partial, c->d_alpha_early, nullptr) == PYLDA_OK;
+        if (hipEventRecord(ctx->join_event[1], ctx->aux_stream[1]) == hipSuccess) forked = true;
+        else (void)hipStreamSynchronize(ctx->aux_stream[1]);
+    }
+    void join()
+    {
+        if (forked) (void)hipStreamWaitEvent(ctx->stream, ctx->join_event[1], 0);
+        forked = false;
+    }
+    ~AlphaEarly() { join(); }
+};
+
+int enqueue_statistics(pylda_ctx* ctx, pylda_corpus* c, bool terms_forked, AlphaEarly& alpha_early)
 {
     if (ctx->force_logspace) {
         HIP_TRY(ctx, hipMemsetAsync(c->d_rfinal, 0, (size_t)c->nnz * sizeof(double), ctx->stream));
@@ -409,6 +438,7 @@
     const int ss_bracket = open_bracket(ctx, -2, ctx->stream);
     const int rc = enqueue_sstats_gather(ctx, c);
     if (terms_forked) (void)hipStreamWaitEvent(ctx->stream, ctx->join_event[0], 0);
+    alpha_early.join();
     close_bracket(ctx, ss_bracket, ctx->stream);
     return rc;
 }
@@ -476,7 +506,7 @@
         (void)hipStreamSynchronize(c->ctx->stream);
     }
     dev_free(c->d_doc_ptr); dev_free(c->d_term_id); dev_free(c->d_term_ct); dev_free(c->d_order);
-    dev_free(c->d_gamma); dev_free(c->d_doc_ll); dev_free(c->d_doc_wll); dev_free(c->d_iters);
+    dev_free(c->d_gamma); dev_free(c->d_alpha_early); dev_free(c->d_doc_ll); dev_free(c->d_doc_wll); dev_free(c->d_iters); dev_free(c->d_work_partial);
     dev_free(c->d_status); c->d_flag_count = nullptr; dev_free(c->d_scalars); dev_free(c->d_entropy_partial);
     dev_free(c->d_tfinal); dev_free(c->d_rfinal); dev_free(c->d_term_scratch); dev_free(c->d_post_doc);
     if (c->d_post_pos) (void)hipFree(c->d_post_pos);
@@ -514,6 +544,7 @@
         return fail(ctx, PYLDA_ERR_STATE, "estep: set_eta and set_alpha must be called first");
     HIP_TRY(ctx, hipSetDevice(ctx->device));
     heldout = heldout ? 1 : 0;
+    gamma_rewritten(c);
     int rc = enqueue_prepare(ctx, heldout != 0);
     if (rc != PYLDA_OK) return rc;
     if ((rc = estep_plan(ctx, c, tol, heldout != 0)) != PYLDA_OK) return rc;
@@ -527,15 +558,27 @@
         if ((rc = enqueue_dense_classes(ctx, c, p)) != PYLDA_OK) return rc;
         if ((rc = enqueue_live_phase(ctx, c, p)) != PYLDA_OK) return rc;
     }
+    AlphaEarly alpha_early{ctx};
+    if (alpha_early.wanted(c, p)) alpha_early.start(c);
     const bool terms_forked = enqueue_doc_terms(ctx, c, p);
     close_bracket(ctx, doc_bracket, ctx->stream);
     if (ctx->profiling) ctx->estep_calls += 1;
-    if (!heldout && (rc = enqueue_statistics(ctx, c, terms_forked)) != PYLDA_OK) return rc;
+    if (!heldout && (rc = enqueue_statistics(ctx, c, terms_forked, alpha_early)) != PYLDA_OK) return rc;
+    alpha_early.join();
     if ((rc = enqueue_logspace_net(ctx, c, p)) != PYLDA_OK) return rc;
-    if (ctx->profiling && c->D > 0)
-        hipLaunchKernelGGL(work_count_kernel, dim3(1), dim3(1024), 0, ctx->stream, c->d_iters, c->d_doc_ptr, c->D, ctx->d_work,
-                           c->compact_ready ? c->d_handoff_it : nullptr, c->d_col_iters, ctx->K);
-    return finish_estep(ctx, c, heldout, !heldout, p.want_doc_ll != 0);
+    if (ctx->profiling && c->D > 0) {
+        if (ctx->work_count_grid) {
+            if ((rc = enqueue_work_count_grid(ctx, c)) != PYLDA_OK) return rc;
+        } else {
+            hipLaunchKernelGGL(work_count_kernel, dim3(1), dim3(1024), 0, ctx->stream, c->d_iters, c->d_doc_ptr, c->D, ctx->d_work,
+                               c->compact_ready ? c->d_handoff_it : nullptr, c->d_col_iters, ctx->K);
+        }
+    }
+    if ((rc = finish_estep(ctx, c, heldout, !heldout, p.want_doc_ll != 0)) != PYLDA_OK) return rc;
+    if (alpha_early.launched &&
+        enqueue_alpha_ss(ctx, c, ctx->stream, ctx->d_early_partial, c->d_alpha_early, c->d_flag_count) == PYLDA_OK)
+        c->alpha_early = true;
+    return PYLDA_OK;
 }
 
 int pylda_estep_results(pylda_ctx* ctx, pylda_corpus* c, double* document_log_likelihood,
@@ -584,6 +627,23 @@
         HIP_TRY(ctx, hipMemcpyAsync(doc_words_ll, c->d_doc_wll, (size_t)c->D * sizeof(double), hipMemcpyDeviceToHost, ctx->stream));
     if (iters)
         HIP_TRY(ctx, hipMemcpyAsync(iters, c->d_iters, (size_t)c->D * sizeof(int32_t), hipMemcpyDeviceToHost, ctx->stream));
+    HIP_TRY(ctx, hipStreamSynchronize(ctx->stream));
+    return PYLDA_OK;
+}
+
+int pylda_test_handover(pylda_ctx* ctx, pylda_corpus* c, int32_t* handoff_it_d, int32_t* col_iters_d)
+{
+    if (!ctx) return PYLDA_ERR_INVALID;
+    if (!c || c->ctx != ctx || !handoff_it_d || !col_iters_d) return fail(ctx, PYLDA_ERR_INVALID, "test_handover: bad argument");
+    if (!c->estep_done) return fail(ctx, PYLDA_ERR_STATE, "test_handover: no E-step has run on this corpus");
+    HIP_TRY(ctx, hipSetDevice(ctx->device));
+    if (!c->compact_ready) {
+        std::fill(handoff_it_d, handoff_it_d + c->D, -1);
+        std::fill(col_iters_d, col_iters_d + c->D, 0);
+        return PYLDA_OK;
+    }
+    HIP_TRY(ctx, hipMemcpyAsync(handoff_it_d, c->d_handoff_it, (size_t)c->D * sizeof(int32_t), hipMemcpyDeviceToHost, ctx->stream));
+    HIP_TRY(ctx, hipMemcpyAsync(col_iters_d, c->d_col_iters, (size_t)c->D * sizeof(int32_t), hipMemcpyDeviceToHost, ctx->stream));
     HIP_TRY(ctx, hipStreamSynchronize(ctx->stream));
     return PYLDA_OK;
 }
diff --git a/pylda_amd/csrc/host_internal.h b/pylda_amd/csrc/host_internal.h
--- a/pylda_amd/csrc/host_internal.h
+++ b/pylda_amd/csrc/host_internal.h
@@ -60,6 +60,7 @@
     double* d_beta = nullptr;
     double* d_small = nullptr;
     double* d_partial = nullptr;
+    double* d_early_partial = nullptr;
     std::vector<double> h_beta;
     double beta_sum = 0.0, beta_lgamma_sum = 0.0;
 
@@ -105,6 +106,8 @@
     int gather_round_mb = 0;
     int launch_order = 1;
     int terms_overlap = 1;
+    int alpha_ss_early = 1;
+    int work_count_grid = 1;
     int slab_uber = 1;
     int wide_postings = 0;
     int lds_pad = 0;
@@ -149,9 +152,13 @@
     int32_t* d_term_ct = nullptr;
     int32_t* d_order = nullptr;
     double* d_gamma = nullptr;
+    double* d_alpha_early = nullptr;
+    bool alpha_early = false;
+    bool gamma_escaped = false;
     double* d_doc_ll = nullptr;
     double* d_doc_wll = nullptr;
     int32_t* d_iters = nullptr;
+    double* d_work_partial = nullptr;
     int32_t* d_status = nullptr;
     int32_t* d_flag_count = nullptr;
     double* d_scalars = nullptr;
@@ -292,6 +299,8 @@
     }
 };
 
+inline void gamma_rewritten(pylda_corpus* c) { c->alpha_early = false; }
+
 PlanConfig plan_config(const pylda_ctx* ctx);
 void build_plan(pylda_corpus* c);
 int slab_uber_from(const pylda_ctx* ctx, const pylda_corpus* c);
@@ -319,6 +328,11 @@
 AlphaSums alpha_sums(const pylda_ctx* ctx);
 int finish_estep(pylda_ctx* ctx, pylda_corpus* c, int heldout, bool entropy, bool doc_values);
 
+int enqueue_alpha_ss(pylda_ctx* ctx, const pylda_corpus* c, hipStream_t st, double* partial, double* out_k, const int32_t* redo);
+
+size_t work_count_partials(int64_t D);
+int enqueue_work_count_grid(pylda_ctx* ctx, const pylda_corpus* c);
+
 int build_postings(pylda_corpus* c);
 int enqueue_sstats_gather(pylda_ctx* ctx, pylda_corpus* c);
 
diff --git a/pylda_amd/csrc/launch_completion.hip b/pylda_amd/csrc/launch_completion.hip
--- a/pylda_amd/csrc/launch_completion.hip
+++ b/pylda_amd/csrc/launch_completion.hip
@@ -72,6 +72,7 @@
     if (observed && !observed->estep_done)
         return fail(ctx, PYLDA_ERR_STATE, "completion_score: no E-step or fold-in has run on the observed corpus");
     HIP_TRY(ctx, hipSetDevice(ctx->device));
+    if (gamma_dk) gamma_rewritten(held);
     if (gamma_dk && held->D > 0)
         HIP_TRY(ctx, hipMemcpyAsync(held->d_gamma, gamma_dk, (size_t)held->D * ctx->K * sizeof(double), hipMemcpyHostToDevice, ctx->stream));
 
diff --git a/pylda_amd/csrc/launch_foldin.hip b/pylda_amd/csrc/launch_foldin.hip
--- a/pylda_amd/csrc/launch_foldin.hip
+++ b/pylda_amd/csrc/launch_foldin.hip
@@ -113,6 +113,7 @@
     if (!ctx->foldin_ready) return fail(ctx, PYLDA_ERR_STATE, "foldin: foldin_set_model must be called first");
     if (c->gibbs_ready) return fail(ctx, PYLDA_ERR_STATE, "foldin: the corpus holds a Gibbs training state; fold in a corpus of its own");
     HIP_TRY(ctx, hipSetDevice(ctx->device));
+    gamma_rewritten(c);
     int rc = prepare_tokens(ctx, c);
     if (rc != PYLDA_OK) return rc;
     HIP_TRY(ctx, hipMemcpyAsync(ctx->d_foldin_alpha, alpha_k, (size_t)ctx->K * sizeof(double), hipMemcpyHostToDevice, ctx->stream));
diff --git a/pylda_amd/csrc/launch_gibbs.hip b/pylda_amd/csrc/launch_gibbs.hip
--- a/pylda_amd/csrc/launch_gibbs.hip
+++ b/pylda_amd/csrc/launch_gibbs.hip
@@ -172,6 +172,7 @@
     if (!ctx) return PYLDA_ERR_INVALID;
     int rc = check_call(ctx, c, "gibbs_init", first_document);
     if (rc != PYLDA_OK) return rc;
+    gamma_rewritten(c);
     HIP_TRY(ctx, hipSetDevice(ctx->device));
     if ((rc = prepare_gibbs(ctx, c)) != PYLDA_OK) return rc;
     GibbsParams p = gibbs_params(ctx, c);
@@ -194,6 +195,7 @@
     if (!ctx) return PYLDA_ERR_INVALID;
     int rc = check_call(ctx, c, "gibbs_sweep", first_document);
     if (rc != PYLDA_OK) return rc;
+    gamma_rewritten(c);
     if (!c->gibbs_ready) return fail(ctx, PYLDA_ERR_STATE, "gibbs_sweep: gibbs_init or gibbs_set_state must be called first");
     if (!alpha_k || !beta_v || !(beta_sum > 0.0)) return fail(ctx, PYLDA_ERR_INVALID, "gibbs_sweep: alpha, beta or beta_sum missing");
     if (blocks < 1) return fail(ctx, PYLDA_ERR_INVALID, "gibbs_sweep: blocks=%lld (at least 1)", (long long)blocks);
@@ -264,6 +266,7 @@
     if (!ctx) return PYLDA_ERR_INVALID;
     int rc = check_call(ctx, c, "gibbs_set_state", 0);
     if (rc != PYLDA_OK) return rc;
+    gamma_rewritten(c);
     HIP_TRY(ctx, hipSetDevice(ctx->device));
     const bool fresh = !c->gibbs_ready;
     if (fresh && (!n_kv || !n_k || !topics))
@@ -378,6 +381,7 @@
     if (!ctx) return PYLDA_ERR_INVALID;
     int rc = check_call(ctx, c, "gibbs_round_sample", first_document);
     if (rc != PYLDA_OK) return rc;
+    gamma_rewritten(c);
     if (!c->gibbs_ready) return fail(ctx, PYLDA_ERR_STATE, "gibbs_round_sample: gibbs_init or gibbs_set_state must be called first");
     if (!alpha_k || !beta_v || !(beta_sum > 0.0)) return fail(ctx, PYLDA_ERR_INVALID, "gibbs_round_sample: alpha, beta or beta_sum missing");
     if (blocks < 1) return fail(ctx, PYLDA_ERR_INVALID, "gibbs_round_sample: blocks=%lld (at least 1)", (long long)blocks);
@@ -420,6 +424,7 @@
     if (!ctx) return PYLDA_ERR_INVALID;
     int rc = check_call(ctx, c, "gibbs_round_apply", 0);
     if (rc != PYLDA_OK) return rc;
+    gamma_rewritten(c);
     if (!c->gibbs_ready) return fail(ctx, PYLDA_ERR_STATE, "gibbs_round_apply: gibbs_init or gibbs_set_state must be called first");
     if (!c->gibbs_exchange_world) return fail(ctx, PYLDA_ERR_STATE, "gibbs_round_apply: gibbs_exchange_prepare must be called first");
     if (round < 0 || round >= c->gibbs_exchange_blocks)
diff --git a/pylda_amd/csrc/launch_hybrid.hip b/pylda_amd/csrc/launch_hybrid.hip
--- a/pylda_amd/csrc/launch_hybrid.hip
+++ b/pylda_amd/csrc/launch_hybrid.hip
@@ -110,6 +110,7 @@
         return fail(ctx, PYLDA_ERR_STATE, "hybrid_estep: set_eta and set_alpha must be called first");
     HIP_TRY(ctx, hipSetDevice(ctx->device));
     heldout = heldout ? 1 : 0;
+    gamma_rewritten(c);
     int rc = prepare_hybrid(ctx, c, heldout == 0);
     if (rc != PYLDA_OK) return rc;
     if ((rc = enqueue_prepare(ctx, false)) != PYLDA_OK) return rc;
diff --git a/pylda_amd/csrc/launch_work_count.hip b/pylda_amd/csrc/launch_work_count.hip
--- /dev/null
+++ b/pylda_amd/csrc/launch_work_count.hip
@@ -0,0 +1,18 @@
+#include "host_internal.h"
+#include "work_count.h"
+
+namespace pylda_host {
+
+size_t work_count_partials(int64_t D) { return (size_t)((D + kWorkCountDocs - 1) / kWorkCountDocs) * 4; }
+
+int enqueue_work_count_grid(pylda_ctx* ctx, const pylda_corpus* c)
+{
+    const int nblocks = (int)((c->D + kWorkCountDocs - 1) / kWorkCountDocs);
+    hipLaunchKernelGGL(work_count_grid_kernel, dim3(nblocks), dim3(1024), 0, ctx->stream, c->d_iters, c->d_doc_ptr, c->D,
+                       c->d_work_partial, c->compact_ready ? c->d_handoff_it : nullptr, c->d_col_iters, ctx->K);
+    hipLaunchKernelGGL(work_count_finish_kernel, dim3(1), dim3(256), 0, ctx->stream, c->d_work_partial, nblocks, ctx->d_work);
+    HIP_TRY(ctx, hipGetLastError());
+    return PYLDA_OK;
+}
+
+}
diff --git a/pylda_amd/csrc/mstep_api.hip b/pylda_amd/csrc/mstep_api.hip
--- a/pylda_amd/csrc/mstep_api.hip
+++ b/pylda_amd/csrc/mstep_api.hip
@@ -1,5 +1,20 @@
 #include "host_internal.h"
 #include "mstep_kernels.h"
+
+namespace pylda_host {
+
+int enqueue_alpha_ss(pylda_ctx* ctx, const pylda_corpus* c, hipStream_t st, double* partial, double* out_k, const int32_t* redo)
+{
+    const int K = ctx->K;
+    const int nblocks = (int)std::min<int64_t>(1024, std::max<int64_t>(1, (c->D + 3) / 4));
+    hipLaunchKernelGGL(mstep_alpha_ss_kernel, dim3(nblocks), dim3(256), (size_t)4 * K * sizeof(double), st, c->d_gamma, c->D, K,
+                       partial, redo);
+    hipLaunchKernelGGL(column_sum_kernel, dim3((K + 63) / 64), dim3(256), 0, st, partial, nblocks, K, out_k, redo);
+    HIP_TRY(ctx, hipGetLastError());
+    return PYLDA_OK;
+}
+
+}
 
 extern "C" {
 
@@ -42,14 +57,12 @@
     else
         hipLaunchKernelGGL(mstep_update_eta_kernel, dim3((K + 31) / 32, (V + 31) / 32), dim3(256), 0, ctx->stream,
                            ctx->d_sstats, ctx->d_beta, K, V, ctx->ldk, ctx->d_eta);
-    if (want_alpha_ss) {
-        const int nblocks = (int)std::min<int64_t>(1024, std::max<int64_t>(1, (c->D + 3) / 4));
-        hipLaunchKernelGGL(mstep_alpha_ss_kernel, dim3(nblocks), dim3(256), (size_t)4 * K * sizeof(double),
-                           ctx->stream, c->d_gamma, c->D, K, ctx->d_partial);
-        hipLaunchKernelGGL(column_sum_kernel, dim3((K + 63) / 64), dim3(256), 0, ctx->stream, ctx->d_partial,
-                           nblocks, K, d_alpha_ss);
-    }
-    HIP_TRY(ctx, hipGetLastError());
+    HIP_TRY(ctx, hipGetLastError());
+    if (want_alpha_ss && ctx->alpha_ss_early && c->alpha_early && c->d_alpha_early) {
+        HIP_TRY(ctx, hipMemcpyAsync(d_alpha_ss, c->d_alpha_early, (size_t)K * sizeof(double), hipMemcpyDeviceToDevice, ctx->stream));
+    } else if (want_alpha_ss) {
+        return enqueue_alpha_ss(ctx, c, ctx->stream, ctx->d_partial, d_alpha_ss, nullptr);
+    }
     return PYLDA_OK;
 }
 
diff --git a/pylda_amd/csrc/mstep_kernels.h b/pylda_amd/csrc/mstep_kernels.h
--- a/pylda_amd/csrc/mstep_kernels.h
+++ b/pylda_amd/csrc/mstep_kernels.h
@@ -93,9 +93,11 @@
 
 __global__ __launch_bounds__(256) void mstep_alpha_ss_kernel(const double* __restrict__ gamma,
                                                              int64_t D, int K,
-                                                             double* __restrict__ partial)
+                                                             double* __restrict__ partial,
+                                                             const int32_t* __restrict__ redo)
 {
     extern __shared__ __attribute__((aligned(16))) char smem[];
+    if (redo && redo[0] == 0) return;
     double* acc = reinterpret_cast<double*>(smem);
     const int lane = threadIdx.x & (kWave - 1), wave = threadIdx.x / kWave;
     for (int k = lane; k < K; k += kWave) acc[wave * K + k] = 0.0;
@@ -125,9 +127,11 @@
 
 __global__ __launch_bounds__(256) void column_sum_kernel(const double* __restrict__ partial,
                                                          int nblocks, int K,
-                                                         double* __restrict__ out)
+                                                         double* __restrict__ out,
+                                                         const int32_t* __restrict__ redo)
 {
     __shared__ double part[4][64];
+    if (redo && redo[0] == 0) return;
     const int kk = threadIdx.x & 63, grp = threadIdx.x >> 6;
     const int k = blockIdx.x * 64 + kk;
     double s = 0.0;
diff --git a/pylda_amd/csrc/plan.hip b/pylda_amd/csrc/plan.hip
--- a/pylda_amd/csrc/plan.hip
+++ b/pylda_amd/csrc/plan.hip
@@ -47,6 +47,7 @@
     if (!strcmp(name, "gather_partial_rows")) return c->have_postings ? c->partial_rows : 0;
     if (!strcmp(name, "gather_live")) return c->have_postings && c->live_stats ? 1 : 0;
     if (!strcmp(name, "live_off_by_alpha")) return c->live_off_by_alpha ? 1 : 0;
+    if (!strcmp(name, "alpha_ss_early")) return c->alpha_early ? 1 : 0;
     if (!strcmp(name, "quad_slot_bytes")) return c->d_quad_rec && c->quad_slots_serial == c->plan_serial ? c->quad_slots.bytes() : 0;
     return fail(c->ctx, PYLDA_ERR_INVALID, "corpus_layout: unknown name '%s'", name);
 }
diff --git a/pylda_amd/csrc/work_count.h b/pylda_amd/csrc/work_count.h
--- /dev/null
+++ b/pylda_amd/csrc/work_count.h
@@ -0,0 +1,59 @@
+#pragma once
+#include "estep_common.h"
+
+namespace pylda {
+
+constexpr int kWorkCountDocs = 16384;
+
+__global__ __launch_bounds__(1024) void work_count_grid_kernel(const int32_t* __restrict__ iters, const int64_t* __restrict__ doc_ptr,
+                                                               int64_t D, double* __restrict__ partial,
+                                                               const int32_t* __restrict__ handoff_it,
+                                                               const int32_t* __restrict__ col_iters, int K)
+{
+    __shared__ double scratch[16];
+    const int64_t first = (int64_t)blockIdx.x * kWorkCountDocs, last = first + kWorkCountDocs < D ? first + kWorkCountDocs : D;
+    double a = 0.0, b = 0.0, e = 0.0, h = 0.0;
+    for (int64_t d = first + threadIdx.x; d < last; d += 1024) {
+        const double it = (double)iters[d], n = (double)(doc_ptr[d + 1] - doc_ptr[d]);
+        a += it;
+        b += it * n;
+        const int at = handoff_it ? handoff_it[d] : -1;
+        if (at >= 0) {
+            e += n * ((double)K * at + (double)col_iters[d]);
+            h += 1.0;
+        } else {
+            e += n * (double)K * it;
+        }
+    }
+    a = block_sum<1024>(a, scratch);
+    b = block_sum<1024>(b, scratch);
+    e = block_sum<1024>(e, scratch);
+    h = block_sum<1024>(h, scratch);
+    if (threadIdx.x == 0) {
+        double* out = partial + (size_t)blockIdx.x * 4;
+        out[0] = a;
+        out[1] = b;
+        out[2] = e;
+        out[3] = h;
+    }
+}
+
+__global__ __launch_bounds__(256) void work_count_finish_kernel(const double* __restrict__ partial, int nblocks, double* __restrict__ work)
+{
+    __shared__ double scratch[4];
+    const long long tick0 = clock64(), wall0 = wall_clock64();
+    double s[4] = {0.0, 0.0, 0.0, 0.0};
+    for (int b = threadIdx.x; b < nblocks; b += 256)
+#pragma unroll
+        for (int j = 0; j < 4; ++j) s[j] += partial[(size_t)b * 4 + j];
+#pragma unroll
+    for (int j = 0; j < 4; ++j) s[j] = block_sum<256>(s[j], scratch);
+    if (threadIdx.x == 0) {
+#pragma unroll
+        for (int j = 0; j < 4; ++j) work[j] += s[j];
+        work[4] += (double)(clock64() - tick0);
+        work[5] += (double)(wall_clock64() - wall0);
+    }
+}
+
+}
```
